# MyrtleSoftware/myrtlespeech

Measured on AMD Instinct MI355X. Metric: audio-sec/s (RTF), DS2 5xBiLSTM-1024 encoder forward + CTC greedy, 80-feature 10 s clips @ batch 32/GPU, higher is better.
Workload: dtype f16x3 (f32 split in fp16 hi+lo, 3 fp16 MFMA passes, f32 acc: LSTM, projections, conv1/2, FC1; FC2/CTC/decode f32)

## Files before the change

include/ms_hotpath.h:

```cpp
#ifndef MS_HOTPATH_H
#define MS_HOTPATH_H

#include <stddef.h>
#include <stdint.h>

#ifdef __cplusplus
extern "C" {
#endif

#define MS_ABI_VERSION 4

enum {
  MS_OK = 0,
  MS_ERR_INVALID = 1,
  MS_ERR_HIP = 2,
  MS_ERR_WORKSPACE = 3,
  MS_ERR_TIMEOUT = 4,
  MS_ERR_UNSUPPORTED = 5
};

enum { MS_CELL_LSTM = 0, MS_CELL_GRU = 1, MS_CELL_RNN_TANH = 2, MS_CELL_HARD_LSTM = 3 };

enum { MS_ACT_NONE = 0, MS_ACT_CLAMP = 1  };

int ms_abi_version(void);
const char* ms_last_error(void);


int ms_mask_time_(float* x, const int32_t* lens, int N, int inner, int T, void* stream);

size_t ms_maskconv_packed_bytes(int Cout, int Cin_g, int KF, int KT, int groups);

int ms_maskconv_pack(const float* w, void* packed, int Cout, int Cin_g, int KF, int KT, int groups, void* stream);

int ms_maskconv_forward(const float* x, const int32_t* lens, const void* packed_w, const float* bias, float* y,
                        int N, int Cin, int Fin, int Tin, int Cout, int Fout, int Tout, int KF, int KT, int SF,
                        int ST, int DF, int DT, int pad_f_l, int pad_t_l, int groups, int act, float act_lo,
                        float act_hi, void* stream);

size_t ms_maskconv_cl_packed_bytes(int Cout, int Cin, int KF, int KT);
int ms_maskconv_cl_pack(const float* w, void* packed, int Cout, int Cin, int KF, int KT, void* stream);
size_t ms_maskconv_cl_workspace_bytes(int N, int Cin, int Fin, int Tin);
int ms_maskconv_cl_forward(const float* x, const int32_t* lens, const void* packed_w, const float* bias, float* y,
                           int N, int Cin, int Fin, int Tin, int Cout, int Fout, int Tout, int KF, int KT, int SF,
                           int ST, int DF, int DT, int pad_f_l, int pad_t_l, int act, float act_lo, float act_hi,
                           void* workspace, size_t workspace_bytes, void* stream);

size_t ms_maskconv_fwin_packed_bytes(int Cout, int KF, int KT);
int ms_maskconv_fwin_pack(const float* w, void* packed, int Cout, int KF, int KT, void* stream);
size_t ms_maskconv_fwin_workspace_bytes(int N, int Tin, int KF, int SF, int Fout);
int ms_maskconv_fwin_forward(const float* x, const int32_t* lens, const void* packed_w, const float* bias, float* y, int N,
                             int Fin, int Tin, int Cout, int Fout, int Tout, int KF, int KT, int SF, int ST, int DT,
                             int pad_f_l, int pad_t_l, int act, float act_lo, float act_hi, void* workspace,
                             size_t workspace_bytes, void* stream);

int ms_maskconv_fwin_planes_supported(int N, int Tin, int Cout, int Fout, int Tout, int KF, int KT, int SF, int ST, int DT);
int ms_maskconv_cl_supported(int N, int Cin, int Fin, int Cout, int Fout, int Tout, int KT, int ST, int DT);
int ms_maskconv_fwin_planes_forward(const float* x, const int32_t* lens, const void* packed_w, const float* bias, void* planes,
                                    size_t planes_bytes, int N, int Fin, int Tin, int Cout, int Fout, int Tout, int KF, int KT,
                                    int SF, int ST, int DT, int pad_f_l, int pad_t_l, int act, float act_lo, float act_hi,
                                    void* workspace, size_t workspace_bytes, void* stream);
int ms_maskconv_cl_planes_forward(const int32_t* lens, const void* packed_w, const float* bias, float* y, int N, int Cin,
                                  int Fin, int Tin, int Cout, int Fout, int Tout, int KF, int KT, int SF, int ST, int DF,
                                  int DT, int pad_f_l, int pad_t_l, int act, float act_lo, float act_hi, void* planes,
                                  size_t planes_bytes, void* stream);

int ms_conv_set_variant(int variant);

size_t ms_maskconv1d_gemm_packed_bytes(int Cout, int Cin, int KT);
int ms_maskconv1d_gemm_pack(const float* w, void* packed, int Cout, int Cin, int KT, void* stream);
size_t ms_maskconv1d_gemm_workspace_bytes(int N, int Cin, int Tout, int Cout, int KT);
int ms_maskconv1d_gemm_forward(const float* x, const int32_t* lens, const void* packed, const float* bias, float* y, int N,
                               int Cin, int Tin, int Cout, int Tout, int KT, int ST, int DT, int pad_l, int act,
                               float act_lo, float act_hi, void* workspace, size_t workspace_bytes, void* stream);

int ms_nct_to_tnc(const float* x, float* y, int N, int CF, int T, void* stream);

int ms_clamp(const float* x, float* y, size_t n, float lo, float hi, void* stream);


int ms_linear_forward(const float* x, const float* w, const float* bias, float* y, int M, int K, int N, int act,
                      float act_lo, float act_hi, void* stream);

#define MS_LINEAR_FEW_ROWS 1
size_t ms_linear_splitk_workspace_bytes(int M, int K, int N, int flags);
int ms_linear_splitk_forward(const float* x, const float* w, const float* bias, float* y, int M, int K, int N, int act,
                             float act_lo, float act_hi, int flags, void* workspace, size_t workspace_bytes, void* stream);

size_t ms_linear_split_workspace_bytes(int M, int K, int N);
int ms_linear_split_forward(const float* x, const float* w, const float* bias, float* y, int M, int K, int N, int act,
                            float act_lo, float act_hi, void* workspace, size_t workspace_bytes, void* stream);

size_t ms_linear_split_packed_bytes(int K, int N);
int ms_linear_split_pack(const float* w, void* packed, int K, int N, void* stream);
int ms_linear_split_forward_packed(const float* x, const void* packed_w, const float* bias, float* y, int M, int K, int N, int act,
                                   float act_lo, float act_hi, void* workspace, size_t workspace_bytes, void* stream);


int ms_lookahead_forward(const float* x, const float* w, float* y, int N, int F, int T, int ctx, long xs_n,
                         long xs_f, long xs_t, long ys_n, long ys_f, long ys_t, int act, float act_lo,
                         float act_hi, void* stream);

int ms_lookahead_window_forward(const float* x, const float* w, float* y, int N, int F, int T_in, int T_out, int ctx,
                                long xs_n, long xs_f, long xs_t, long ys_n, long ys_f, long ys_t, int act, float act_lo,
                                float act_hi, void* stream);


int ms_rnn_padded_hidden(int cell, int H, int ndir);
size_t ms_rnn_packed_bytes(int cell, int In, int H, int ndir);
int ms_rnn_pack(int cell, int In, int H, int ndir, const float* const* w_ih_host, const float* const* w_hh_host,
                const float* const* b_ih_host, const float* const* b_hh_host, void* packed, void* stream);

size_t ms_rnn_workspace_bytes(int cell, int T, int N, int In, int H, int ndir);

int ms_rnn_layer_forward(int cell, const void* packed, const float* x, const int32_t* lens, int max_len,
                         const float* h0, const float* c0, float* out, float* hn, float* cn, int T, int N, int In,
                         int H, int ndir, void* workspace, size_t workspace_bytes, void* stream);

enum { MS_RNN_X_PLANES_IN_WS = 1, MS_RNN_OUT_PLANES_TO_WS = 2, MS_RNN_PACKED_ROWS = 4, MS_RNN_HX_PREINIT = 4096,
       MS_RNN_RECURRENCE_ONLY = 8192, MS_RNN_TIMING_SKIP_PROJECTION = 8192 ,
       MS_RNN_PROJECTION_ONLY = 16384 };
int ms_rnn_layer_chains_planes(int cell, int H, int ndir);
int ms_rnn_hx_preinit(int cell, int T, int N, int In, int H, int ndir, int max_len, int nregions, void* workspace,
                      size_t workspace_bytes, void* stream);
int ms_rnn_layer_packs_rows(int cell, int T, int N, int In, int H, int ndir);
int ms_rnn_layer_forward_ex(int cell, const void* packed, const float* x, const int32_t* lens, int max_len,
                            const float* h0, const float* c0, float* out, float* hn, float* cn, int T, int N, int In,
                            int H, int ndir, int flags, void* workspace, size_t workspace_bytes, void* stream);

int ms_rnn_layer_is_wide(int cell, int H, int ndir, int N);
int ms_rnn_stack_overlap_ok(int cell, int T, int N, int In, int H, int ndir, int nl);
int ms_rnn_stack_forward(int cell, const void* const* packed_host, const float* x, const int32_t* lens, int max_len,
                         const float* h0, const float* c0, float* out, float* hn, float* cn, int T, int N, int In, int H, int ndir,
                         int nl, int segments, void* workspace, size_t workspace_bytes, void* stream);

int ms_rnn_status(const void* workspace, void* stream);

size_t ms_rnn_debug_offset(int cell, int T, int N, int In, int H, int ndir);

int ms_gemm_set_variant(int variant);

enum {
  MS_PROF_PROJECTION = 0, MS_PROF_RECURRENCE = 1, MS_PROF_GEMM_K_LARGE = 2, MS_PROF_GEMM_K_SMALL = 3, MS_PROF_CONV = 4,
  MS_PROF_LAYOUT = 5, MS_PROF_LINEAR = 6, MS_PROF_GREEDY = 7, MS_PROF_OTHER = 8
};
#define MS_PROF_KINDS 9
int ms_prof_enable(int on);
int ms_prof_read(float* out_ms_host, int* out_n_host);

int ms_clock_probe(unsigned long long* out_dev, int samples, int spacing_us, void* stream);

int ms_barrier_chain_probe(unsigned long long* out_dev, int steps, int threads, void* stream);


size_t ms_ctc_loss_workspace_bytes(int T, int N, int V, int S_max);

int ms_ctc_status(const void* workspace, void* stream);

#define MS_CTC_LOG_PROBS_IN 2
int ms_ctc_loss_forward(const float* logits, const int32_t* in_lens, const int32_t* targets,
                        const int32_t* tgt_offsets, const int32_t* tgt_lens, float* nll, float* reduced, int T,
                        int N, int V, int S_max, int blank, int reduction, int zero_infinity, void* workspace,
                        size_t workspace_bytes, void* stream);

int ms_log_softmax_axis(const float* x, float* y, int outer, int axis, int inner, void* stream);
int ms_log_softmax_axis_backward(const float* y, const float* g, float* gx, int outer, int axis, int inner, void* stream);

size_t ms_ctc_loss_backward_workspace_bytes(int T, int N, int V, int S_max);
int ms_ctc_loss_backward(const float* logits, const int32_t* in_lens, const int32_t* targets, const int32_t* tgt_offsets,
                         const int32_t* tgt_lens, const float* grad_nll, float* grad_logits, int T, int N, int V,
                         int S_max, int blank, int zero_infinity, void* workspace, size_t workspace_bytes, void* stream);


int ms_ctc_greedy_decode(const float* x, const int32_t* lens, int32_t* out_idx, int32_t* out_len, int T, int N,
                         int V, int blank, void* stream);

size_t ms_ctc_greedy_stream_state_bytes(int N);
int ms_ctc_greedy_stream_begin(void* state, int N, void* stream);
int ms_ctc_greedy_stream_step(const float* x, int rows, int n, int V, int blank, const int32_t* total_lens,
                              const int32_t* chunk_lens, int32_t* labels, int32_t* label_frames, int cap, int32_t* fresh,
                              void* state, int N, void* stream);


#define MS_CTC_ALIGN_BP_LDS_BYTES 98304
size_t ms_ctc_align_workspace_bytes(int T, int N, int V, int S_max);
int ms_ctc_align(const float* x, const int32_t* in_lens, const int32_t* targets, const int32_t* tgt_offsets,
                 const int32_t* tgt_lens, float* score, int32_t* frame_state, int32_t* token_start, int32_t* token_end,
                 float* token_logp, int T, int N, int V, int L_max, int blank, int flags, void* workspace,
                 size_t workspace_bytes, void* stream);


size_t ms_ctc_beam_workspace_bytes(int T, int N, int V, int beam_width);

int ms_ctc_beam_decode(const float* probs, const int32_t* lens, int32_t* out_idx, int32_t* out_len, int T, int N,
                       int V, int blank, int beam_width, float prune_threshold, int separator, const float* word_factor,
                       int t_begin, int t_end, const float* lm_factor, int finish, int32_t* beam_len,
                       int32_t* beam_idx, int32_t* beam_plen, void* workspace, size_t workspace_bytes,
                       void* stream);

int ms_ctc_beam_decode_rows(const float* probs, const int32_t* lens, int32_t* out_idx, int32_t* out_len, int T, int N,
                            int V, int blank, int beam_width, float prune_threshold, int separator,
                            const float* word_factor, int t_begin, int t_end, int row0, int rows_held,
                            const float* lm_factor, int finish, int32_t* beam_len, int32_t* beam_idx, int32_t* beam_plen,
                            void* workspace, size_t workspace_bytes, void* stream);


#define MS_NGRAM_MAX_ORDER 5

int ms_ngram_lm_table_check(const void* blob_host, size_t bytes);

int ms_ngram_lm_score(const void* table, const void* header_host, size_t table_bytes, const int32_t* prefixes,
                      const int32_t* prefix_lens, float* out, int P, int L, int separator, void* stream);

size_t ms_ctc_beam_lm_workspace_bytes(int T, int N, int V, int beam_width, int order);
int ms_ctc_beam_decode_lm(const float* probs, const int32_t* lens, int32_t* out_idx, int32_t* out_len, int T, int N,
                          int V, int blank, int beam_width, float prune_threshold, int separator,
                          const float* word_factor, int t_begin, int t_end, int row0, int rows_held, const void* lm_table,
                          const void* lm_header_host, size_t lm_table_bytes, int finish, int32_t* beam_len,
                          int32_t* beam_idx, int32_t* beam_plen, void* workspace, size_t workspace_bytes, void* stream);

int ms_ctc_beam_decode_ex(const float* probs, const int32_t* lens, int32_t* out_idx, int32_t* out_len, int T, int N,
                          int V, int blank, int beam_width, float prune_threshold, int separator,
                          const float* word_factor, int t_begin, int t_end, int row0, int rows_held,
                          const float* lm_factor, int finish, int32_t* beam_len, int32_t* beam_idx, int32_t* beam_plen,
                          void* workspace, size_t workspace_bytes, void* stream, const void* lm_table,
                          const void* lm_header_host, size_t lm_table_bytes, int range_safe, float* beam_score,
                          int32_t* scale_log2);


size_t ms_mfcc_workspace_bytes(int N, int T, int n_fft, int n_mels, int n_mfcc);
int ms_mfcc_forward(const float* wave, const int32_t* wave_lens, const float* window, const float* dft,
                    const float* mel_fb, const float* dct, float* out, int N, int max_samples, int T, int n_fft,
                    int hop, int n_mels, int n_mfcc, float top_db, void* workspace, size_t workspace_bytes,
                    void* stream);

int ms_mfcc_legacy_forward(const float* wave, const int32_t* wave_lens, const double* twiddle, const double* fbank,
                           const double* dct, const double* lifter, float* out, int N, int max_samples, int T,
                           int frame_len, int frame_step, int nfft, int nfilt, int numcep, double preemph,
                           void* stream);

size_t ms_standardize_workspace_bytes(int N);
int ms_standardize_forward(const float* x, const int32_t* lens, float* y, int N, int inner, int T, void* workspace,
                           size_t workspace_bytes, void* stream);

int ms_context_frames_forward(const float* x, const int32_t* lens, float* y, int N, int F, int T, int n_context,
                              void* stream);

int ms_spec_augment_(float* x, const int32_t* f_bands, const int32_t* t_bands, int N, int C, int F, int T, int n_f,
                     int n_t, void* stream);


int ms_embedding_forward(const float* table, const int32_t* idx, float* out, int R, int D, int V1, void* stream);

int ms_rnnt_joint_forward(const float* enc_p, const int32_t* enc_row, const float* pred_p, const float* w_out,
                          const float* b_out, float* logp, int R, int J, int V1, void* stream);

int ms_rnnt_topk(const float* scores, int32_t* out_idx, float* out_val, int B, int C, int k, void* stream);

size_t ms_rnnt_decode_workspace_bytes(int T, int N, int V, int D, int H, int L, int J, int beam_width, int max_symbols,
                                      int greedy);
int ms_rnnt_decode(const float* enc_p, const int32_t* lens, const float* embedding, const float* const* w_ih,
                   const float* const* w_hh, const float* const* b_ih, const float* const* b_hh, const float* w_pred,
                   const float* w_out, const float* b_out, int32_t* out_idx, int32_t* out_len, float* out_score, int T,
                   int N, int V, int D, int H, int L, int J, int beam_width, int max_symbols, int greedy, void* workspace,
                   size_t workspace_bytes, void* stream);

size_t ms_rnnt_loss_lattice_bytes(int N, int T, int U1);
size_t ms_rnnt_loss_workspace_bytes(int N, int T, int U1, int V1);
int ms_rnnt_loss_forward(const float* logits, const int32_t* in_lens, const int32_t* targets, const int32_t* tgt_lens,
                         float* nll, float* lattice, int N, int T, int U1, int V1, int blank, void* workspace,
                         size_t workspace_bytes, void* stream);
int ms_rnnt_loss_backward(const float* logits, const int32_t* in_lens, const int32_t* targets, const int32_t* tgt_lens,
                          const float* nll, const float* lattice, const float* grad_nll, float* grad, int N, int T, int U1,
                          int V1, int blank, void* stream);

size_t ms_rnnt_score_lattice_bytes(int N, int T, int U1);
size_t ms_rnnt_score_workspace_bytes(int N, int T, int U1, int J, int V1);
int ms_rnnt_score(const float* enc_p, const float* pred_p, const float* w_out, const float* b_out, const int32_t* in_lens,
                  const int32_t* targets, const int32_t* tgt_lens, float* nll, float* lattice, int N, int T, int U1, int J,
                  int V1, int blank, void* workspace, size_t workspace_bytes, void* stream);

size_t ms_rnnt_joint_loss_lattice_bytes(int N, int T, int U1);
int ms_rnnt_joint_loss_forward(const float* enc_p, const float* pred_p, const float* w_out, const float* b_out,
                               const int32_t* in_lens, const int32_t* targets, const int32_t* tgt_lens, float* nll,
                               float* lattice, int N, int T, int U1, int J, int V1, int blank, void* workspace,
                               size_t workspace_bytes, void* stream);
size_t ms_rnnt_joint_loss_backward_workspace_min_bytes(int N, int T, int U1, int J, int V1);
size_t ms_rnnt_joint_loss_backward_workspace_bytes(int N, int T, int U1, int J, int V1);
int ms_rnnt_joint_loss_backward(const float* enc_p, const float* pred_p, const float* w_out, const float* b_out,
                                const int32_t* in_lens, const int32_t* targets, const int32_t* tgt_lens, const float* nll,
                                const float* lattice, const float* grad_nll, float* d_enc_p, float* d_pred_p, float* d_w_out,
                                float* d_b_out, int N, int T, int U1, int J, int V1, int blank, void* workspace,
                                size_t workspace_bytes, void* stream);
// ... 18 lines not shown
```

myrtlespeech_amd/_lib.py:

```python
import ctypes
import os
import re
from ctypes import POINTER, c_char_p, c_double, c_float, c_int, c_int32, c_long, c_size_t, c_void_p

import torch

_HERE = os.path.dirname(os.path.abspath(__file__))
LIB_PATH = os.environ.get("MS_HOTPATH_LIB") or os.path.join(_HERE, "libms_hotpath.so")
HEADER_PATH = os.path.join(os.path.dirname(_HERE), "include", "ms_hotpath.h")

MS_OK = 0
ABI_VERSION = 4
ERR_NAMES = {1: "MS_ERR_INVALID", 2: "MS_ERR_HIP", 3: "MS_ERR_WORKSPACE", 4: "MS_ERR_TIMEOUT", 5: "MS_ERR_UNSUPPORTED"}

CELL_LSTM, CELL_GRU, CELL_RNN_TANH, CELL_HARD_LSTM = 0, 1, 2, 3
ACT_NONE, ACT_CLAMP = 0, 1
LINEAR_FEW_ROWS = 1
PROF_KINDS = 9

_P = c_void_p
_PP = POINTER(c_void_p)

SIGNATURES = {
    "ms_abi_version": (c_int, []),
    "ms_last_error": (c_char_p, []),
    "ms_mask_time_": (c_int, [_P, _P, c_int, c_int, c_int, _P]),
    "ms_maskconv_packed_bytes": (c_size_t, [c_int, c_int, c_int, c_int, c_int]),
    "ms_maskconv_pack": (c_int, [_P, _P, c_int, c_int, c_int, c_int, c_int, _P]),
    "ms_maskconv_forward": (c_int, [_P, _P, _P, _P, _P] + [c_int] * 17 + [c_float, c_float, _P]),
    "ms_maskconv_cl_packed_bytes": (c_size_t, [c_int, c_int, c_int, c_int]),
    "ms_maskconv_cl_pack": (c_int, [_P, _P, c_int, c_int, c_int, c_int, _P]),
    "ms_maskconv_cl_workspace_bytes": (c_size_t, [c_int, c_int, c_int, c_int]),
    "ms_maskconv_cl_forward": (c_int, [_P, _P, _P, _P, _P] + [c_int] * 16 + [c_float, c_float, _P, c_size_t, _P]),
    "ms_maskconv_fwin_packed_bytes": (c_size_t, [c_int, c_int, c_int]),
    "ms_maskconv_fwin_pack": (c_int, [_P, _P, c_int, c_int, c_int, _P]),
    "ms_maskconv_fwin_workspace_bytes": (c_size_t, [c_int, c_int, c_int, c_int, c_int]),
    "ms_maskconv_fwin_forward": (c_int, [_P, _P, _P, _P, _P] + [c_int] * 14 + [c_float, c_float, _P, c_size_t, _P]),
    "ms_maskconv_fwin_planes_forward": (c_int, [_P, _P, _P, _P, _P, c_size_t] + [c_int] * 14 + [c_float, c_float, _P, c_size_t, _P]),
    "ms_maskconv_cl_planes_forward": (c_int, [_P, _P, _P, _P] + [c_int] * 16 + [c_float, c_float, _P, c_size_t, _P]),
    "ms_maskconv_fwin_planes_supported": (c_int, [c_int] * 10),
    "ms_maskconv_cl_supported": (c_int, [c_int] * 9),
    "ms_conv_set_variant": (c_int, [c_int]),
    "ms_maskconv1d_gemm_packed_bytes": (c_size_t, [c_int, c_int, c_int]),
    "ms_maskconv1d_gemm_pack": (c_int, [_P, _P, c_int, c_int, c_int, _P]),
    "ms_maskconv1d_gemm_workspace_bytes": (c_size_t, [c_int] * 5),
    "ms_maskconv1d_gemm_forward": (c_int, [_P, _P, _P, _P, _P] + [c_int] * 10 + [c_float, c_float, _P, c_size_t, _P]),
    "ms_nct_to_tnc": (c_int, [_P, _P, c_int, c_int, c_int, _P]),
    "ms_clamp": (c_int, [_P, _P, c_size_t, c_float, c_float, _P]),
    "ms_linear_forward": (c_int, [_P, _P, _P, _P, c_int, c_int, c_int, c_int, c_float, c_float, _P]),
    "ms_linear_splitk_workspace_bytes": (c_size_t, [c_int, c_int, c_int, c_int]),
    "ms_linear_splitk_forward": (c_int, [_P, _P, _P, _P, c_int, c_int, c_int, c_int, c_float, c_float, c_int, _P, c_size_t, _P]),
    "ms_linear_split_workspace_bytes": (c_size_t, [c_int, c_int, c_int]),
    "ms_linear_split_forward": (c_int, [_P, _P, _P, _P, c_int, c_int, c_int, c_int, c_float, c_float, _P, c_size_t, _P]),
    "ms_linear_split_packed_bytes": (c_size_t, [c_int, c_int]),
    "ms_linear_split_pack": (c_int, [_P, _P, c_int, c_int, _P]),
    "ms_linear_split_forward_packed": (c_int, [_P, _P, _P, _P, c_int, c_int, c_int, c_int, c_float, c_float, _P, c_size_t, _P]),
    "ms_lookahead_forward": (c_int, [_P, _P, _P, c_int, c_int, c_int, c_int] + [c_long] * 6 + [c_int, c_float, c_float, _P]),
    "ms_lookahead_window_forward": (c_int, [_P, _P, _P, c_int, c_int, c_int, c_int, c_int] + [c_long] * 6 + [c_int, c_float, c_float, _P]),
    "ms_rnn_packed_bytes": (c_size_t, [c_int, c_int, c_int, c_int]),
    "ms_ctc_status": (c_int, [_P, _P]),
    "ms_rnn_padded_hidden": (c_int, [c_int, c_int, c_int]),
    "ms_rnn_hx_preinit": (c_int, [c_int] * 8 + [_P, c_size_t, _P]),
    "ms_rnn_pack": (c_int, [c_int, c_int, c_int, c_int, _PP, _PP, _PP, _PP, _P, _P]),
    "ms_rnn_workspace_bytes": (c_size_t, [c_int] * 6),
    "ms_rnn_layer_forward": (c_int, [c_int, _P, _P, _P, c_int, _P, _P, _P, _P, _P] + [c_int] * 5 + [_P, c_size_t, _P]),
    "ms_rnn_layer_forward_ex": (c_int, [c_int, _P, _P, _P, c_int, _P, _P, _P, _P, _P] + [c_int] * 6 + [_P, c_size_t, _P]),
    "ms_rnn_layer_chains_planes": (c_int, [c_int, c_int, c_int]),
    "ms_rnn_layer_is_wide": (c_int, [c_int] * 4),
    "ms_rnn_stack_overlap_ok": (c_int, [c_int] * 7),
    "ms_rnn_stack_forward": (c_int, [c_int, _P, _P, _P, c_int, _P, _P, _P, _P, _P] + [c_int] * 7 + [_P, c_size_t, _P]),
    "ms_rnn_status": (c_int, [_P, _P]),
    "ms_rnn_debug_offset": (c_size_t, [c_int] * 6),
    "ms_rnn_layer_packs_rows": (c_int, [c_int] * 6),
    "ms_gemm_set_variant": (c_int, [c_int]),
    "ms_prof_enable": (c_int, [c_int]),
    "ms_prof_read": (c_int, [POINTER(c_float), POINTER(c_int)]),
    "ms_clock_probe": (c_int, [_P, c_int, c_int, _P]),
    "ms_barrier_chain_probe": (c_int, [_P, c_int, c_int, _P]),
    "ms_ctc_loss_workspace_bytes": (c_size_t, [c_int] * 4),
    "ms_ctc_loss_forward": (c_int, [_P] * 7 + [c_int] * 7 + [_P, c_size_t, _P]),
    "ms_log_softmax_axis": (c_int, [_P, _P, c_int, c_int, c_int, _P]),
    "ms_log_softmax_axis_backward": (c_int, [_P, _P, _P, c_int, c_int, c_int, _P]),
    "ms_ctc_loss_backward_workspace_bytes": (c_size_t, [c_int] * 4),
    "ms_ctc_loss_backward": (c_int, [_P] * 7 + [c_int] * 6 + [_P, c_size_t, _P]),
    "ms_ctc_greedy_decode": (c_int, [_P, _P, _P, _P, c_int, c_int, c_int, c_int, _P]),
    "ms_ctc_align_workspace_bytes": (c_size_t, [c_int] * 4),
    "ms_ctc_align": (c_int, [_P] * 10 + [c_int] * 6 + [_P, c_size_t, _P]),
    "ms_ctc_greedy_stream_state_bytes": (c_size_t, [c_int]),
    "ms_ctc_greedy_stream_begin": (c_int, [_P, c_int, _P]),
    "ms_ctc_greedy_stream_step": (c_int, [_P, c_int, c_int, c_int, c_int, _P, _P, _P, _P, c_int, _P, _P, c_int, _P]),
    "ms_embedding_forward": (c_int, [_P, _P, _P, c_int, c_int, c_int, _P]),
    "ms_rnnt_joint_forward": (c_int, [_P, _P, _P, _P, _P, _P, c_int, c_int, c_int, _P]),
    "ms_rnnt_topk": (c_int, [_P, _P, _P, c_int, c_int, c_int, _P]),
    "ms_ctc_beam_workspace_bytes": (c_size_t, [c_int] * 4),
    "ms_ctc_beam_decode": (c_int, [_P, _P, _P, _P, c_int, c_int, c_int, c_int, c_int, c_float, c_int, _P, c_int, c_int,
                                   _P, c_int, _P, _P, _P, _P, c_size_t, _P]),
    "ms_ctc_beam_decode_rows": (c_int, [_P, _P, _P, _P, c_int, c_int, c_int, c_int, c_int, c_float, c_int, _P, c_int, c_int,
                                        c_int, c_int, _P, c_int, _P, _P, _P, _P, c_size_t, _P]),
    "ms_ngram_lm_table_check": (c_int, [_P, c_size_t]),
    "ms_ngram_lm_score": (c_int, [_P, _P, c_size_t, _P, _P, _P, c_int, c_int, c_int, _P]),
    "ms_ctc_beam_lm_workspace_bytes": (c_size_t, [c_int] * 5),
    "ms_ctc_beam_decode_lm": (c_int, [_P, _P, _P, _P, c_int, c_int, c_int, c_int, c_int, c_float, c_int, _P, c_int, c_int,
                                      c_int, c_int, _P, _P, c_size_t, c_int, _P, _P, _P, _P, c_size_t, _P]),
    "ms_ctc_beam_decode_ex": (c_int, [_P, _P, _P, _P, c_int, c_int, c_int, c_int, c_int, c_float, c_int, _P, c_int, c_int,
                                      c_int, c_int, _P, c_int, _P, _P, _P, _P, c_size_t, _P, _P, _P, c_size_t, c_int, _P, _P]),
    "ms_rnnt_decode_workspace_bytes": (c_size_t, [c_int] * 10),
    "ms_rnnt_decode": (c_int, [_P, _P, _P, _PP, _PP, _PP, _PP, _P, _P, _P, _P, _P, _P] + [c_int] * 10 + [_P, c_size_t, _P]),
    "ms_rnnt_loss_lattice_bytes": (c_size_t, [c_int] * 3),
    "ms_rnnt_loss_workspace_bytes": (c_size_t, [c_int] * 4),
    "ms_rnnt_loss_forward": (c_int, [_P] * 6 + [c_int] * 5 + [_P, c_size_t, _P]),
    "ms_rnnt_loss_backward": (c_int, [_P] * 8 + [c_int] * 5 + [_P]),
    "ms_rnnt_score_lattice_bytes": (c_size_t, [c_int] * 3),
    "ms_rnnt_score_workspace_bytes": (c_size_t, [c_int] * 5),
    "ms_rnnt_score": (c_int, [_P] * 9 + [c_int] * 6 + [_P, c_size_t, _P]),
    "ms_rnnt_joint_loss_lattice_bytes": (c_size_t, [c_int] * 3),
    "ms_rnnt_joint_loss_forward": (c_int, [_P] * 9 + [c_int] * 6 + [_P, c_size_t, _P]),
    "ms_rnnt_joint_loss_backward_workspace_min_bytes": (c_size_t, [c_int] * 5),
    "ms_rnnt_joint_loss_backward_workspace_bytes": (c_size_t, [c_int] * 5),
    "ms_rnnt_joint_loss_backward": (c_int, [_P] * 14 + [c_int] * 6 + [_P, c_size_t, _P]),
    "ms_rnnt_align_workspace_bytes": (c_size_t, [c_int] * 4),
    "ms_rnnt_align": (c_int, [_P] * 9 + [c_int] * 6 + [_P, c_size_t, _P]),
    "ms_rnnt_align_joint_workspace_bytes": (c_size_t, [c_int] * 5),
    "ms_rnnt_align_joint": (c_int, [_P] * 12 + [c_int] * 6 + [_P, c_size_t, _P]),
    "ms_mfcc_workspace_bytes": (c_size_t, [c_int] * 5),
    "ms_mfcc_forward": (c_int, [_P] * 7 + [c_int] * 7 + [c_float, _P, c_size_t, _P]),
    "ms_mfcc_legacy_forward": (c_int, [_P] * 7 + [c_int] * 8 + [c_double, _P]),
    "ms_standardize_workspace_bytes": (c_size_t, [c_int]),
    "ms_standardize_forward": (c_int, [_P, _P, _P, c_int, c_int, c_int, _P, c_size_t, _P]),
    "ms_context_frames_forward": (c_int, [_P, _P, _P, c_int, c_int, c_int, c_int, _P]),
    "ms_spec_augment_": (c_int, [_P, _P, _P] + [c_int] * 6 + [_P]),
}

_lib = None


def header_symbols():
    with open(HEADER_PATH) as f:
        text = re.sub(r"/\*.*?\*/", "", f.read(), flags=re.S)
    return sorted(set(re.findall(r"\b(ms_[a-z0-9_]+)\s*\(", text)))


def load():
    global _lib
    if _lib is None:
        if not os.path.exists(LIB_PATH):
            raise RuntimeError(
                f"{LIB_PATH} not found: build it with `python -c 'import __graft_entry__ as g; g.build()'` "
                "(or `make -C myrtlespeech_amd/csrc`). There is no CPU fallback."
            )
        lib = ctypes.CDLL(LIB_PATH)
        for name, (res, args) in SIGNATURES.items():
            fn = getattr(lib, name)
            fn.restype = res
            fn.argtypes = args
        got = lib.ms_abi_version()
        if got != ABI_VERSION:
            raise RuntimeError(f"{LIB_PATH} reports MS_ABI_VERSION {got}, this binding needs {ABI_VERSION}: rebuild the "
                               "library (`make -C myrtlespeech_amd/csrc`)")
        _lib = lib
    return _lib


def require_gpu():
    if not torch.cuda.is_available():
        raise RuntimeError("myrtlespeech_amd: a HIP device (MI355X) is required; there is no CPU fallback")


def stream_ptr():
    return c_void_p(torch.cuda.current_stream().cuda_stream)


def ptr(t, strided=False):
    if t is None:
        return c_void_p(0)
    if not isinstance(t, torch.Tensor):
        raise TypeError(f"_lib.ptr: expected a torch.Tensor or None, got {type(t).__name__}")
    if not t.is_cuda:
        raise ValueError(f"_lib.ptr: a {t.device.type} tensor (shape {tuple(t.shape)}) cannot be a device-pointer argument; "
                         "move it to the GPU first (host buffers go through _lib.host_ptr)")
    if not strided and not t.is_contiguous():
        raise ValueError(f"_lib.ptr: tensor of shape {tuple(t.shape)} and strides {tuple(t.stride())} is not contiguous; the "
                         "kernels read dense storage (call .contiguous())")
    return c_void_p(t.data_ptr())


def host_ptr(t):
    if t is None:
        return c_void_p(0)
    if not isinstance(t, torch.Tensor) or t.is_cuda or not t.is_contiguous():
        raise ValueError("_lib.host_ptr: expected a contiguous CPU tensor")
    return c_void_p(t.data_ptr())


def check(rc, what):
    if rc != MS_OK:
        msg = load().ms_last_error().decode()
        raise RuntimeError(f"{what} failed with {ERR_NAMES.get(rc, rc)}: {msg}")


def f32c(t):
    if t.dtype != torch.float32:
        t = t.float()
    if not t.is_cuda:
        t = t.cuda()
    return t.contiguous()


_ASYNC_LENS = os.environ.get("MS_ASYNC_LENS") != "0"


_const_lens = {}


def _const_tensor(shape, dtype, value, make: bool):
    key = (tuple(shape), dtype, int(value))
    rec = _const_lens.get(key)
    if rec is not None:
        t, version = rec
        if version_of(t) == version:
            return t
        _const_lens[("stale", len(_const_lens)) + key] = rec
        del _const_lens[key]
    if not make or len(_const_lens) >= 4096:
        return None
    t = torch.full(tuple(shape), int(value), dtype=dtype, device="cuda")
    _const_lens[key] = (t, version_of(t))
    return t
# ... 108 lines not shown
```

myrtlespeech_amd/csrc/common.h:

```cpp
#pragma once
#include <hip/hip_runtime.h>
#include <stdint.h>
#include <stdio.h>
#include <atomic>
#include <string>

#include "../../include/ms_hotpath.h"

namespace ms {

void set_error(const std::string& s);

#define MS_REQUIRE(cond, msg)                                              \
  do {                                                                     \
    if (!(cond)) {                                                         \
      ms::set_error(std::string(__func__) + ": " + (msg));                 \
      return MS_ERR_INVALID;                                               \
    }                                                                      \
  } while (0)

#define MS_HIP(call)                                                                        \
  do {                                                                                      \
    hipError_t e_ = (call);                                                                 \
    if (e_ != hipSuccess) {                                                                 \
      ms::set_error(std::string(__func__) + ": " #call " -> " + hipGetErrorString(e_));     \
      return MS_ERR_HIP;                                                                    \
    }                                                                                       \
  } while (0)

#define MS_LAUNCH_CHECK() MS_HIP(hipGetLastError())

static inline size_t align_up(size_t v, size_t a) { return (v + a - 1) / a * a; }
static inline int cdiv(int a, int b) { return (a + b - 1) / b; }

typedef float f32x4 __attribute__((ext_vector_type(4)));
typedef float f32x16 __attribute__((ext_vector_type(16)));

__device__ __forceinline__ int mfma32_row(int reg, int lane) { return (reg & 3) + 8 * (reg >> 2) + 4 * (lane >> 5); }

int num_cus();

struct DeviceOnce {
  std::atomic<unsigned long long> done_mask{0};
  static unsigned long long bit() {
    int d = 0;
    if (hipGetDevice(&d) != hipSuccess) d = 0;
    return 1ull << (d & 63);
  }
  bool need() const { return !(done_mask.load(std::memory_order_acquire) & bit()); }
  void done() { done_mask.fetch_or(bit(), std::memory_order_release); }
};

struct ProfScope {
  hipEvent_t a = nullptr, b = nullptr;
  int kind;
  hipStream_t stream;
  bool on;
  ProfScope(int kind, hipStream_t st);
  ~ProfScope();
  ProfScope(const ProfScope&) = delete;
  ProfScope& operator=(const ProfScope&) = delete;
};

enum { PREC_F32 = 0, PREC_BF16X3 = 1, PREC_F16 = 2, PREC_F16X3 = 3 };
int precision_mode();
int split_mode();
enum { GEMM_K_WHOLE = 0, GEMM_K_FIRST = 1, GEMM_K_SECOND = 2 };
int weight_scale_launch(const float* w, size_t n, float* scale_word, int prec, hipStream_t stream);

constexpr bool prec_one_plane(int P) { return P == PREC_F16; }
constexpr bool prec_half_planes(int P) { return P == PREC_F16X3 || P == PREC_F16; }

typedef unsigned u32x4_ __attribute__((ext_vector_type(4)));
typedef __bf16 bf16x8_ __attribute__((ext_vector_type(8)));
typedef _Float16 f16x8_ __attribute__((ext_vector_type(8)));
template <bool HM>
__device__ __forceinline__ unsigned plane_bits(float x) {
  if constexpr (HM) return (unsigned)__builtin_bit_cast(unsigned short, (_Float16)__builtin_amdgcn_fmed3f(x, -65504.f, 65504.f));
  else return (unsigned)__builtin_bit_cast(unsigned short, (__bf16)x);
}
template <bool HM>
__device__ __forceinline__ unsigned plane_bits_bounded(float x) {
  if constexpr (HM) return (unsigned)__builtin_bit_cast(unsigned short, (_Float16)x);
  else return (unsigned)__builtin_bit_cast(unsigned short, (__bf16)x);
}
template <bool HM>
__device__ __forceinline__ float plane_val(unsigned bits) {
  if constexpr (HM) return (float)__builtin_bit_cast(_Float16, (unsigned short)bits);
  else return __uint_as_float(bits << 16);
}
template <bool HM>
__device__ __forceinline__ void plane_split(float x, unsigned& hi, unsigned& lo) {
  hi = plane_bits<HM>(x);
  lo = plane_bits<HM>(x - plane_val<HM>(hi));
}
template <bool HM>
__device__ __forceinline__ void plane_split_bounded(float x, unsigned& hi, unsigned& lo) {
  hi = plane_bits_bounded<HM>(x);
  lo = plane_bits_bounded<HM>(x - plane_val<HM>(hi));
}
template <bool HM>
__device__ __forceinline__ f32x16 mfma_32x32x16(u32x4_ a, u32x4_ b, f32x16 c) {
  if constexpr (HM) return __builtin_amdgcn_mfma_f32_32x32x16_f16(__builtin_bit_cast(f16x8_, a), __builtin_bit_cast(f16x8_, b), c, 0, 0, 0);
  else return __builtin_amdgcn_mfma_f32_32x32x16_bf16(__builtin_bit_cast(bf16x8_, a), __builtin_bit_cast(bf16x8_, b), c, 0, 0, 0);
}
template <bool HM>
__device__ __forceinline__ f32x4 mfma_16x16x32(u32x4_ a, u32x4_ b, f32x4 c) {
  if constexpr (HM) return __builtin_amdgcn_mfma_f32_16x16x32_f16(__builtin_bit_cast(f16x8_, a), __builtin_bit_cast(f16x8_, b), c, 0, 0, 0);
  else return __builtin_amdgcn_mfma_f32_16x16x32_bf16(__builtin_bit_cast(bf16x8_, a), __builtin_bit_cast(bf16x8_, b), c, 0, 0, 0);
}

}
```

myrtlespeech_amd/csrc/gemm_split.hip:

```cpp
#include <algorithm>
#include <cstdlib>

#include "common.h"

namespace ms {

typedef unsigned u32x4 __attribute__((ext_vector_type(4)));
typedef unsigned u32x2 __attribute__((ext_vector_type(2)));
typedef __bf16 bf16x8 __attribute__((ext_vector_type(8)));
typedef _Float16 f16x8 __attribute__((ext_vector_type(8)));

__device__ __forceinline__ unsigned bf16_hi_bits(float x) { return (unsigned)__builtin_bit_cast(unsigned short, (__bf16)x); }

__device__ __forceinline__ unsigned f16_bits(float x) { return (unsigned)__builtin_bit_cast(unsigned short, (_Float16)x); }

__global__ void to_f16_plane_kernel(const float* __restrict__ x, unsigned short* __restrict__ hi, size_t n4) {
  for (size_t i = (size_t)blockIdx.x * blockDim.x + threadIdx.x; i < n4; i += (size_t)gridDim.x * blockDim.x) {
    const f32x4 v = reinterpret_cast<const f32x4*>(x)[i];
    u32x2 ho = {f16_bits(v[0]) | (f16_bits(v[1]) << 16), f16_bits(v[2]) | (f16_bits(v[3]) << 16)};
    reinterpret_cast<u32x2*>(hi)[i] = ho;
  }
}

template <bool HM>
// ... 267 lines not shown
  }
  constexpr int GM = 4;
  const int per_group = GM * nbn;
  const int first_m = (bid / per_group) * GM;
  const int gm = min(GM, nbm - first_m);
  const int bm = first_m + (bid % per_group) % gm;
  const int bn = (bid % per_group) / gm;
  const int m0 = bm * S2_M, n0 = bn * S2_N;

  const int tid = threadIdx.x, lane = tid & 63, wave = tid >> 6;
  const int wm = wave >> 1, wn = wave & 1;
  const int l31 = lane & 31, half = lane >> 5;
  const int kg = tid & 3, r_in = tid >> 2;

  f32x16 acc[2][4];
#pragma unroll
  for (int i = 0; i < 2; ++i)
#pragma unroll
    for (int j = 0; j < 4; ++j)
#pragma unroll
      for (int r = 0; r < 16; ++r) acc[i][j][r] = 0.f;

  u32x4 rah[2], ral[2], rbh[2], rbl[2];
  auto load_regs = [&](int k0) {
#pragma unroll
    for (int i = 0; i < 2; ++i) {
      rah[i] = ld_granule(Ah, M, lda, m0 + r_in + 128 * i, k0 + kg * 8);
      rbh[i] = ld_granule(Wh, N, ldw, n0 + r_in + 128 * i, k0 + kg * 8);
      if (!F16) {
        ral[i] = ld_granule(Al, M, lda, m0 + r_in + 128 * i, k0 + kg * 8);
        rbl[i] = ld_granule(Wl, N, ldw, n0 + r_in + 128 * i, k0 + kg * 8);
      }
    }
  };
  auto store_regs = [&](char* buf) {
#pragma unroll
    for (int i = 0; i < 2; ++i) {
      const int off = kg * S2_PLANE + (r_in + 128 * i) * 16;
      *reinterpret_cast<u32x4*>(buf + off) = rah[i];
      *reinterpret_cast<u32x4*>(buf + 2 * S2_TILE + off) = rbh[i];
      if (!F16) {
        *reinterpret_cast<u32x4*>(buf + S2_TILE + off) = ral[i];
        *reinterpret_cast<u32x4*>(buf + 3 * S2_TILE + off) = rbl[i];
      }
    }
  };

  const int nk = K / SB_K;
  load_regs(0);
  store_regs(lds);
  if (nk > 1) load_regs(SB_K);
  __syncthreads();

  u32x4 ah[2], al[2], bh[4], bl[4];
  auto read_ops = [&](const char* cur, int s) {
    const int g = 2 * s + half;
#pragma unroll
    for (int i = 0; i < 2; ++i) {
      const int off = g * S2_PLANE + (wm * 64 + i * 32 + l31) * 16;
      ah[i] = *reinterpret_cast<const u32x4*>(cur + off);
      if (!F16) al[i] = *reinterpret_cast<const u32x4*>(cur + S2_TILE + off);
    }
#pragma unroll
    for (int j = 0; j < 4; ++j) {
      const int off = g * S2_PLANE + (wn * 128 + j * 32 + l31) * 16;
      bh[j] = *reinterpret_cast<const u32x4*>(cur + 2 * S2_TILE + off);
      if (!F16) bl[j] = *reinterpret_cast<const u32x4*>(cur + 3 * S2_TILE + off);
    }
  };
  auto mfma_ops = [&]() {
    if (F16) {
#pragma unroll
      for (int i = 0; i < 2; ++i)
#pragma unroll
        for (int j = 0; j < 4; ++j)
          acc[i][j] = __builtin_amdgcn_mfma_f32_32x32x16_f16(__builtin_bit_cast(f16x8, ah[i]), __builtin_bit_cast(f16x8, bh[j]),
                                                             acc[i][j], 0, 0, 0);
    } else {
#pragma unroll
      for (int i = 0; i < 2; ++i)
#pragma unroll
        for (int j = 0; j < 4; ++j)
          acc[i][j] = mfma_32x32x16<HM>(ah[i], bh[j], acc[i][j]);
#pragma unroll
      for (int i = 0; i < 2; ++i)
#pragma unroll
        for (int j = 0; j < 4; ++j)
          acc[i][j] = mfma_32x32x16<HM>(al[i], bh[j], acc[i][j]);
#pragma unroll
      for (int i = 0; i < 2; ++i)
#pragma unroll
        for (int j = 0; j < 4; ++j)
          acc[i][j] = mfma_32x32x16<HM>(ah[i], bl[j], acc[i][j]);
    }
  };
  {
    for (int kt = 0; kt < nk; ++kt) {
      const char* cur = lds + (kt & 1) * S2_BUF;
      read_ops(cur, 0);
      store_regs(lds + ((kt + 1) & 1) * S2_BUF);
      mfma_ops();
      __builtin_amdgcn_sched_group_barrier(0x100, F16 ? 6 : 12, 0);
#pragma unroll
      for (int i = 0; i < (F16 ? 4 : 8); ++i) {
        __builtin_amdgcn_sched_group_barrier(0x008, F16 ? 2 : 3, 0);
        __builtin_amdgcn_sched_group_barrier(0x200, 1, 0);
      }
      __builtin_amdgcn_sched_barrier(0);
      read_ops(cur, 1);
      load_regs(min(kt + 2, nk - 1) * SB_K);
      mfma_ops();
      __builtin_amdgcn_sched_group_barrier(0x100, F16 ? 6 : 12, 0);
#pragma unroll
      for (int i = 0; i < (F16 ? 4 : 8); ++i) {
        __builtin_amdgcn_sched_group_barrier(0x008, F16 ? 2 : 3, 0);
        __builtin_amdgcn_sched_group_barrier(0x020, 1, 0);
      }
      __builtin_amdgcn_sched_barrier(0);
      __syncthreads();
    }
  }

#pragma unroll
  for (int j = 0; j < 4; ++j) {
    const int n = n0 + wn * 128 + j * 32 + l31;
    const float bv = (bias != nullptr && n < N) ? bias[n] : 0.f;
#pragma unroll
    for (int i = 0; i < 2; ++i)
#pragma unroll
      for (int r = 0; r < 16; ++r) {
        const int m = m0 + wm * 64 + i * 32 + mfma32_row(r, lane);
        if (m < M && n < N) {
          float v = acc[i][j][r] + bv;
          if (act == MS_ACT_CLAMP) v = fminf(fmaxf(v, lo), hi);
          Y[(size_t)m * N + n] = v;
        }
      }
  }
}

constexpr int G4_PLANE = 256 * 64;
constexpr int G4_STAGE = 4 * G4_PLANE;
constexpr int G4_LDS = 2 * G4_STAGE;
typedef __attribute__((address_space(3))) void* lds_ptr_t;

__device__ __forceinline__ void lds_dma_16(__amdgpu_buffer_rsrc_t rsrc, char* dst, int voff, int soff) {
  __builtin_amdgcn_raw_ptr_buffer_load_lds(rsrc, (lds_ptr_t)dst, 16, voff, soff, 0, 0);
}

template <int P, int WN, int PER_STEP_ = 3, bool SPACED = false, int NJ = 4, int TM = 256>
__device__ __forceinline__ void gemm4_body(const unsigned short* __restrict__ Ah, const unsigned short* __restrict__ Al,
                                           const unsigned short* __restrict__ Wh, const unsigned short* __restrict__ Wl,
                                           const float* __restrict__ bias, float* __restrict__ Y, int M, int K, int N, int act,
                                           float lo, float hi, const int* __restrict__ m_eff, int lda, int ldw, int kmode) {
  constexpr bool F16 = prec_one_plane(P), HM = P == PREC_F16X3;
  extern __shared__ __attribute__((aligned(16))) char lds[];
  constexpr int TN = 32 * NJ * WN;
  static_assert(NJ == 4 || (NJ == 2 && WN == 2), "the narrow form is the 8-wave kernel");
  static_assert(TM == 256 || (TM == 128 && NJ == 2 && WN == 2), "128-row tiles: the four-wave 128 x 128 form");
  if (m_eff != nullptr) {
    M = __builtin_amdgcn_readfirstlane(*m_eff);
    if ((int)blockIdx.x >= ((N + TN - 1) / TN) * ((M + TM - 1) / TM)) return;
  }
  const int nbn = (N + TN - 1) / TN, nbm = (M + TM - 1) / TM;
  const int nwg = nbn * nbm;
  int bid = blockIdx.x;
  {
    const int q = nwg / 8, r = nwg % 8, xcd = bid % 8;
    bid = (xcd < r ? xcd * (q + 1) : r * (q + 1) + (xcd - r) * q) + bid / 8;
  }
  constexpr int GM = 4;
  const int per_group = GM * nbn;
  const int first_m = (bid / per_group) * GM;
  const int gm = min(GM, nbm - first_m);
  const int bm = first_m + (bid % per_group) % gm;
  const int bn = (bid % per_group) / gm;
  const int m0 = bm * TM, n0 = bn * TN;

  const int tid = threadIdx.x, lane = tid & 63;
  const int wave = __builtin_amdgcn_readfirstlane(tid >> 6);
  const int wm = WN == 2 ? wave >> 1 : wave, wn = WN == 2 ? wave & 1 : 0;
  const int l31 = lane & 31, half = lane >> 5;

  constexpr int NPA = NJ == 2 ? (F16 ? 2 : 4) : WN == 2 ? (F16 ? 4 : 8) : (F16 ? 4 : 8);
  constexpr int NPB = TM == 128 ? NPA : NJ == 2 ? (F16 ? 1 : 2) : WN == 2 ? 0 : (F16 ? 2 : 4);
  constexpr int NP = NPA + NPB;
  int PA, RA, PB = 2, RB = 0;
  if (TM == 128) {
    if (F16) { PA = 0; RA = wave * 32; PB = 2; RB = wave * 32; }
    else { PA = wave >> 1; RA = (wave & 1) * 64; PB = 2 + (wave >> 1); RB = (wave & 1) * 64; }
  } else if (NJ == 2) {
    if (F16) { PA = 0; RA = wave * 32; PB = 2; RB = wave * 16; }
    else { PA = wave >> 2; RA = (wave & 3) * 64; PB = 2 + (wave >> 2); RB = (wave & 3) * 32; }
  } else if (WN == 2) {
    const int g0 = wave * NPA;
    PA = F16 ? (g0 >> 4) * 2 : (g0 >> 4);
    RA = (g0 & 15) * 16;
  } else if (F16) {
    PA = 0; RA = wave * 64; PB = 2; RB = wave * 32;
  } else {
    PA = wave >> 1; RA = (wave & 1) * 128; PB = 2 + (wave >> 1); RB = (wave & 1) * 64;
  }
  auto plane_rsrc = [&](int pl) {
    const unsigned short* src = pl == 0 ? Ah : pl == 1 ? Al : pl == 2 ? Wh : Wl;
    return __builtin_amdgcn_make_buffer_rsrc(const_cast<unsigned short*>(src), 0, (unsigned)((size_t)(pl < 2 ? M : N) * (pl < 2 ? lda : ldw) * 2), 0x00020000);
  };
  const __amdgpu_buffer_rsrc_t rsrc_a = plane_rsrc(PA), rsrc_b = plane_rsrc(PB);
  int voff[NP];
  {
    const int kgs = (lane & 3) ^ ((lane >> 4) & 3);
#pragma unroll
    for (int p = 0; p < NP; ++p) {
      const int pl = p < NPA ? PA : PB;
      const int rows = pl < 2 ? M : N, row = (pl < 2 ? m0 : n0) + (p < NPA ? RA + p * 16 : RB + (p - NPA) * 16) + (lane >> 2);
      voff[p] = min(row, rows - 1) * ((pl < 2 ? lda : ldw) * 2) + kgs * 16;
    }
  }
  constexpr int RING = (F16 && WN == 2) ? 4 : 2;
  auto stage_off = [&](int stage) { return RING == 4 ? (stage & 1) * G4_STAGE + (stage >> 1) * G4_PLANE : stage * G4_STAGE; };
  auto dma_block = [&](int kb, int stage) {
    const int soff = __builtin_amdgcn_readfirstlane(kb * (SB_K * 2));
    char* dst_a = lds + stage_off(stage) + PA * G4_PLANE + RA * 64;
    char* dst_b = lds + stage_off(stage) + PB * G4_PLANE + RB * 64;
#pragma unroll
    for (int p = 0; p < NP; ++p) {
      if (p < NPA) lds_dma_16(rsrc_a, dst_a + p * 1024, voff[p], soff);
      else lds_dma_16(rsrc_b, dst_b + (p - NPA) * 1024, voff[p], soff);
    }
  };

  f32x16 acc[2][NJ];
#pragma unroll
  for (int i = 0; i < 2; ++i)
#pragma unroll
    for (int j = 0; j < NJ; ++j)
#pragma unroll
      for (int r = 0; r < 16; ++r) acc[i][j][r] = 0.f;
  if (kmode == GEMM_K_SECOND) {
#pragma unroll
    for (int i = 0; i < 2; ++i) {
      const int m = m0 + wm * 64 + i * 32 + l31;
      if (m >= M) continue;
#pragma unroll
      for (int j = 0; j < NJ; ++j)
#pragma unroll
        for (int g = 0; g < 4; ++g) {
          const int n = n0 + wn * (32 * NJ) + j * 32 + 8 * g + 4 * half;
          if (n + 3 < N) {
            const f32x4 v = *reinterpret_cast<const f32x4*>(Y + (size_t)m * N + n);
            acc[i][j][4 * g] = v[0]; acc[i][j][4 * g + 1] = v[1]; acc[i][j][4 * g + 2] = v[2]; acc[i][j][4 * g + 3] = v[3];
          }
        }
    }
  }

  const int sw = (l31 >> 2) & 3;
  const int foff0 = l31 * 64 + ((half ^ sw) * 16);
  const int foff1 = l31 * 64 + (((2 + half) ^ sw) * 16);
  const int a_base = wm * 64 * 64, b_base = 2 * G4_PLANE + wn * (32 * NJ) * 64;

  u32x4 fa[WN == 1 ? 1 : 2][6 + 6];
  auto read_frags = [&](int set, int stage, int h) {
    const char* st = lds + stage_off(stage) + (h ? foff1 : foff0);
#pragma unroll
    for (int i = 0; i < 2; ++i) {
      fa[set][i] = *reinterpret_cast<const u32x4*>(st + a_base + i * 32 * 64);
      if (!F16) fa[set][2 + i] = *reinterpret_cast<const u32x4*>(st + G4_PLANE + a_base + i * 32 * 64);
    }
#pragma unroll
    for (int j = 0; j < NJ; ++j) {
      fa[set][4 + j] = *reinterpret_cast<const u32x4*>(st + b_base + j * 32 * 64);
      if (!F16) fa[set][8 + j] = *reinterpret_cast<const u32x4*>(st + G4_PLANE + b_base + j * 32 * 64);
    }
  };
  auto mfma_set = [&](int set) {
    if (F16) {
#pragma unroll
      for (int i = 0; i < 2; ++i)
#pragma unroll
        for (int j = 0; j < NJ; ++j)
          acc[i][j] = __builtin_amdgcn_mfma_f32_32x32x16_f16(__builtin_bit_cast(f16x8, fa[set][4 + j]),
                                                             __builtin_bit_cast(f16x8, fa[set][i]), acc[i][j], 0, 0, 0);
    } else {
#pragma unroll
      for (int i = 0; i < 2; ++i)
#pragma unroll
        for (int j = 0; j < NJ; ++j)
          acc[i][j] = mfma_32x32x16<HM>(fa[set][4 + j], fa[set][i], acc[i][j]);
#pragma unroll
      for (int i = 0; i < 2; ++i)
#pragma unroll
        for (int j = 0; j < NJ; ++j)
          acc[i][j] = mfma_32x32x16<HM>(fa[set][4 + j], fa[set][2 + i], acc[i][j]);
#pragma unroll
      for (int i = 0; i < 2; ++i)
#pragma unroll
        for (int j = 0; j < NJ; ++j)
          acc[i][j] = mfma_32x32x16<HM>(fa[set][8 + j], fa[set][i], acc[i][j]);
    }
  };

  const int nk = K / SB_K;
  dma_block(0, 0);
  dma_block(min(1, nk - 1), 1);
  if (RING == 4) {
    dma_block(min(2, nk - 1), 2);
    dma_block(min(3, nk - 1), 3);
  }
  __builtin_amdgcn_s_waitcnt(0x0070);
  __builtin_amdgcn_s_barrier();
  if (WN == 1) {
    u32x4 xa[2][4], wb[2][2];
    auto rd_x = [&](int ring, int stage, int h) {
      const char* st = lds + stage * G4_STAGE + (h ? foff1 : foff0) + a_base;
#pragma unroll
      for (int i = 0; i < 2; ++i) {
        xa[ring][i] = *reinterpret_cast<const u32x4*>(st + i * 32 * 64);
        if (!F16) xa[ring][2 + i] = *reinterpret_cast<const u32x4*>(st + G4_PLANE + i * 32 * 64);
      }
    };
    auto rd_w = [&](int ring, int stage, int h, int j) {
      const char* st = lds + stage * G4_STAGE + (h ? foff1 : foff0) + b_base + j * 32 * 64;
      wb[ring][0] = *reinterpret_cast<const u32x4*>(st);
      if (!F16) wb[ring][1] = *reinterpret_cast<const u32x4*>(st + G4_PLANE);
    };
    auto mm = [&](int xr, int wr, int j, auto&& issue) {
      issue(0);
#pragma unroll
      for (int i = 0; i < 2; ++i) {
        if (F16) {
          acc[i][j] = __builtin_amdgcn_mfma_f32_32x32x16_f16(__builtin_bit_cast(f16x8, wb[wr][0]), __builtin_bit_cast(f16x8, xa[xr][i]), acc[i][j], 0, 0, 0);
        } else {
          acc[i][j] = mfma_32x32x16<HM>(wb[wr][0], xa[xr][i], acc[i][j]);
        }
      }
      if (!F16) {
        issue(1);
#pragma unroll
        for (int i = 0; i < 2; ++i)
          acc[i][j] = mfma_32x32x16<HM>(wb[wr][0], xa[xr][2 + i], acc[i][j]);
        issue(2);
#pragma unroll
        for (int i = 0; i < 2; ++i)
          acc[i][j] = mfma_32x32x16<HM>(wb[wr][1], xa[xr][i], acc[i][j]);
      }
    };
    rd_x(0, 0, 0);
    rd_w(0, 0, 0, 0);
    constexpr int PER_STEP = PER_STEP_, DMA_STEPS = (NP + PER_STEP - 1) / PER_STEP;
    for (int b = 0; b < nk; ++b) {
      const int cur = b & 1;
      const int soff_next = __builtin_amdgcn_readfirstlane(min(b + 1, nk - 1) * (SB_K * 2));
      char* dst_a = lds + (cur ^ 1) * G4_STAGE + PA * G4_PLANE + RA * 64;
      char* dst_b = lds + (cur ^ 1) * G4_STAGE + PB * G4_PLANE + RB * 64;
#pragma unroll
      for (int h = 0; h < 2; ++h)
#pragma unroll
        for (int j = 0; j < 4; ++j) {
          const int step = h * 4 + j;
          auto piece = [&](int p) {
            if (p < NPA) lds_dma_16(rsrc_a, dst_a + p * 1024, voff[p], soff_next);
            else lds_dma_16(rsrc_b, dst_b + (p - NPA) * 1024, voff[p], soff_next);
          };
          if (!SPACED && b > 0 && step < DMA_STEPS) {
#pragma unroll
            for (int p = step * PER_STEP; p < (step + 1) * PER_STEP && p < NP; ++p) piece(p);
          }
          auto issue = [&](int k) {
            if (SPACED && b > 0 && step < DMA_STEPS && k < PER_STEP && step * PER_STEP + k < NP) piece(step * PER_STEP + k);
          };
          if (step == 7) {
            __builtin_amdgcn_s_waitcnt(0x0070);
            __builtin_amdgcn_s_barrier();
            rd_x(0, cur ^ 1, 0);
            rd_w(0, cur ^ 1, 0, 0);
          } else {
            if (j == 3) rd_x(1, cur, 1);
            rd_w((step + 1) & 1, cur, (step + 1) >> 2, (step + 1) & 3);
          }
          mm(h, step & 1, j, issue);
        }
    }
  } else {
  read_frags(0, 0, 0);
  __builtin_amdgcn_s_waitcnt(0xc07f);
  __builtin_amdgcn_sched_barrier(0);

  constexpr int NR = NJ == 2 ? (F16 ? 4 : 8) : (F16 ? 6 : 12);
  constexpr int MPR = F16 ? 8 / 6 + 1 : 2;
  for (int b = 0; b < nk; ++b) {
    const int cur = b & (RING - 1), nxt = (b + 1) & (RING - 1);
    read_frags(1, cur, 1);
    mfma_set(0);
#pragma unroll
    for (int i = 0; i < NR; ++i) {
      __builtin_amdgcn_sched_group_barrier(0x100, 1, 0);
      __builtin_amdgcn_sched_group_barrier(0x008, MPR, 0);
    }
    __builtin_amdgcn_sched_barrier(0);
    if (RING == 4) __builtin_amdgcn_s_waitcnt(0x0070 | (2 * NP));
    else __builtin_amdgcn_s_waitcnt(0x0070);
    __builtin_amdgcn_s_barrier();
    __builtin_amdgcn_sched_barrier(0);
    dma_block(min(b + RING, nk - 1), cur);
    read_frags(0, nxt, 0);
    mfma_set(1);
#pragma unroll
    for (int i = 0; i < NR; ++i) {
      if (i < NP) __builtin_amdgcn_sched_group_barrier(0x020, 1, 0);
      __builtin_amdgcn_sched_group_barrier(0x100, 1, 0);
      __builtin_amdgcn_sched_group_barrier(0x008, MPR, 0);
    }
    __builtin_amdgcn_sched_barrier(0);
    __builtin_amdgcn_s_waitcnt(0xc07f);
    __builtin_amdgcn_sched_barrier(0);
  }
  }
  __builtin_amdgcn_s_waitcnt(0x0070);

  const bool n_vec = (N % 4) == 0;
#pragma unroll
  for (int i = 0; i < 2; ++i) {
    const int m = m0 + wm * 64 + i * 32 + l31;
    if (m >= M) continue;
#pragma unroll
    for (int j = 0; j < NJ; ++j)
#pragma unroll
      for (int g = 0; g < 4; ++g) {
        const int n = n0 + wn * (32 * NJ) + j * 32 + 8 * g + 4 * half;
        f32x4 v = {acc[i][j][4 * g], acc[i][j][4 * g + 1], acc[i][j][4 * g + 2], acc[i][j][4 * g + 3]};
        if (n_vec && n + 3 < N) {
          if (bias != nullptr && kmode != GEMM_K_FIRST) {
            const f32x4 bv = *reinterpret_cast<const f32x4*>(bias + n);
            v += bv;
          }
          if (act == MS_ACT_CLAMP && kmode != GEMM_K_FIRST) {
#pragma unroll
            for (int e = 0; e < 4; ++e) v[e] = fminf(fmaxf(v[e], lo), hi);
          }
          *reinterpret_cast<f32x4*>(Y + (size_t)m * N + n) = v;
        } else {
#pragma unroll
          for (int e = 0; e < 4; ++e)
            if (n + e < N) {
              float x = v[e] + (bias != nullptr ? bias[n + e] : 0.f);
              if (act == MS_ACT_CLAMP) x = fminf(fmaxf(x, lo), hi);
              Y[(size_t)m * N + n + e] = x;
            }
        }
      }
  }
}

template <int P>
__global__ __launch_bounds__(512, 2) void gemm_nt_bf16x3_kernel4(const unsigned short* __restrict__ Ah,
                                                                 const unsigned short* __restrict__ Al,
                                                                 const unsigned short* __restrict__ Wh,
                                                                 const unsigned short* __restrict__ Wl,
                                                                 const float* __restrict__ bias, float* __restrict__ Y,
                                                                 int M, int K, int N, int act, float lo, float hi,
                                                                 const int* __restrict__ m_eff, int lda, int ldw, int kmode) {
  gemm4_body<P, 2>(Ah, Al, Wh, Wl, bias, Y, M, K, N, act, lo, hi, m_eff, lda, ldw, kmode);
}

template <int P>
__global__ __launch_bounds__(512, 2) void gemm_nt_bf16x3_kernel4h(const unsigned short* __restrict__ Ah,
                                                                  const unsigned short* __restrict__ Al,
                                                                  const unsigned short* __restrict__ Wh,
                                                                  const unsigned short* __restrict__ Wl,
                                                                  const float* __restrict__ bias, float* __restrict__ Y,
                                                                  int M, int K, int N, int act, float lo, float hi,
                                                                  const int* __restrict__ m_eff, int lda, int ldw, int kmode) {
  gemm4_body<P, 2, 3, false, 2>(Ah, Al, Wh, Wl, bias, Y, M, K, N, act, lo, hi, m_eff, lda, ldw, kmode);
}

template <int P>
__global__ __launch_bounds__(256, 1) void gemm_nt_bf16x3_kernel4q(const unsigned short* __restrict__ Ah,
                                                                  const unsigned short* __restrict__ Al,
                                                                  const unsigned short* __restrict__ Wh,
                                                                  const unsigned short* __restrict__ Wl,
                                                                  const float* __restrict__ bias, float* __restrict__ Y,
                                                                  int M, int K, int N, int act, float lo, float hi,
                                                                  const int* __restrict__ m_eff, int lda, int ldw, int kmode) {
  gemm4_body<P, 2, 3, false, 2, 128>(Ah, Al, Wh, Wl, bias, Y, M, K, N, act, lo, hi, m_eff, lda, ldw, kmode);
}

template <int P, int PER_STEP = 3, bool SPACED = false>
__global__ __launch_bounds__(256, 2) void gemm_nt_bf16x3_kernel4n(
    const unsigned short* __restrict__ Ah, const unsigned short* __restrict__ Al, const unsigned short* __restrict__ Wh,
    const unsigned short* __restrict__ Wl, const float* __restrict__ bias, float* __restrict__ Y, int M, int K, int N, int act,
    float lo, float hi, const int* __restrict__ m_eff, int lda, int ldw, int kmode) {
  gemm4_body<P, 1, PER_STEP, SPACED>(Ah, Al, Wh, Wl, bias, Y, M, K, N, act, lo, hi, m_eff, lda, ldw, kmode);
}

static std::atomic<int> g_gemm_variant{0};

int split_planes_launch(const float* x, unsigned short* hi, unsigned short* lo, size_t elems, int prec, hipStream_t stream) {
  const size_t n4 = elems / 4;
  const int blocks = (int)std::min<size_t>((n4 + 255) / 256, 4096);
  if (prec == PREC_F16)
    hipLaunchKernelGGL(to_f16_plane_kernel, dim3(blocks), dim3(256), 0, stream, x, hi, n4);
  else if (prec == PREC_F16X3)
    hipLaunchKernelGGL(split_planes_kernel<true>, dim3(blocks), dim3(256), 0, stream, x, hi, lo, n4);
  else
    hipLaunchKernelGGL(split_planes_kernel<false>, dim3(blocks), dim3(256), 0, stream, x, hi, lo, n4);
  MS_LAUNCH_CHECK();
  return MS_OK;
}

int split_mode() {
  const int m = precision_mode();
  return m == PREC_F32 ? PREC_F16X3 : m;
}

bool gemm_rows_from_device_ok(int M, int K, int N) {
  static const bool small_tile = getenv("MS_GEMM_TILE128") && getenv("MS_GEMM_TILE128")[0] == '1';
  static const bool regstage = getenv("MS_GEMM_REGSTAGE") && getenv("MS_GEMM_REGSTAGE")[0] == '1';
  const long tiles256 = (long)cdiv(M, S2_M) * cdiv(N, S2_N);
  const bool starved = tiles256 * 4 < (long)num_cus() * 3 && (long)cdiv(M, SB_M) * cdiv(N, SB_N) > tiles256;
  return !small_tile && !regstage && !starved && (long)M * N >= 4L * 1024 * 1024 && K % 32 == 0 &&
         (size_t)std::max(M, N) * K * 2 < ((size_t)1 << 31) && g_gemm_variant.load(std::memory_order_relaxed) != 2;
}

int gemm_bf16x3_launch_rows(const unsigned short* ah, const unsigned short* al, const unsigned short* wh,
                            const unsigned short* wl, const float* bias, float* y, int M, int K, int N, int act, float lo,
                            float hi, int prec, hipStream_t stream, const int* m_eff);
int gemm_bf16x3_launch_ld(const unsigned short* ah, const unsigned short* al, const unsigned short* wh,
                          const unsigned short* wl, const float* bias, float* y, int M, int K, int N, int act, float lo,
                          float hi, int prec, hipStream_t stream, const int* m_eff, int lda, int ldw, int kmode);

int gemm_bf16x3_launch(const unsigned short* ah, const unsigned short* al, const unsigned short* wh,
                       const unsigned short* wl, const float* bias, float* y, int M, int K, int N, int act, float lo,
                       float hi, int prec, hipStream_t stream) {
  return gemm_bf16x3_launch_rows(ah, al, wh, wl, bias, y, M, K, N, act, lo, hi, prec, stream, nullptr);
}

#define MS_BY_PREC(K) (prec == PREC_F16 ? K<PREC_F16> : prec == PREC_F16X3 ? K<PREC_F16X3> : K<PREC_BF16X3>)

int gemm_bf16x3_launch_rows(const unsigned short* ah, const unsigned short* al, const unsigned short* wh,
                            const unsigned short* wl, const float* bias, float* y, int M, int K, int N, int act, float lo,
                            float hi, int prec, hipStream_t stream, const int* m_eff) {
  return gemm_bf16x3_launch_ld(ah, al, wh, wl, bias, y, M, K, N, act, lo, hi, prec, stream, m_eff, K, K, GEMM_K_WHOLE);
}

bool gemm_k_halves_ok(int M, int N) {
  static const bool small_tile = getenv("MS_GEMM_TILE128") && getenv("MS_GEMM_TILE128")[0] == '1';
  static const bool regstage = getenv("MS_GEMM_REGSTAGE") && getenv("MS_GEMM_REGSTAGE")[0] == '1';
  static const bool half_off = getenv("MS_GEMM_HALF_TILE") && getenv("MS_GEMM_HALF_TILE")[0] == '0';
  if (small_tile || regstage || half_off || N % 4 != 0 || g_gemm_variant.load(std::memory_order_relaxed) != 0) return false;
  const long tiles256 = (long)cdiv(M, S2_M) * cdiv(N, S2_N);
  const bool starved = tiles256 * 4 < (long)num_cus() * 3 && (long)cdiv(M, SB_M) * cdiv(N, SB_N) > tiles256;
  const bool t64 = (long)cdiv(M, T6) * cdiv(N, T6) <= 2L * num_cus() && (long)cdiv(M, S2_M) * cdiv(N, 128) * 4 <= (long)num_cus();
  if (t64) return false;
  return starved ? (long)M * N >= 1024L * 1024 : (long)M * N >= 4L * 1024 * 1024;
}

int gemm_bf16x3_launch_ld(const unsigned short* ah, const unsigned short* al, const unsigned short* wh,
                          const unsigned short* wl, const float* bias, float* y, int M, int K, int N, int act, float lo,
                          float hi, int prec, hipStream_t stream, const int* m_eff, int lda, int ldw, int kmode) {
  if (kmode != GEMM_K_WHOLE && !gemm_k_halves_ok(M, N)) {
    set_error("gemm_bf16x3_launch_ld: a contraction cut along K needs an output that runs on the LDS-DMA kernels");
    return MS_ERR_UNSUPPORTED;
  }
  static ms::DeviceOnce attr_once;
  if (attr_once.need()) {
    MS_HIP(hipFuncSetAttribute((const void*)gemm_nt_bf16x3_kernel<false>, hipFuncAttributeMaxDynamicSharedMemorySize, SPLIT_LDS));
    MS_HIP(hipFuncSetAttribute((const void*)gemm_nt_bf16x3_kernel<true>, hipFuncAttributeMaxDynamicSharedMemorySize, SPLIT_LDS));
#define MS_ATTR3(K, bytes)                                                                                         \
    MS_HIP(hipFuncSetAttribute((const void*)K<PREC_BF16X3>, hipFuncAttributeMaxDynamicSharedMemorySize, bytes));   \
    MS_HIP(hipFuncSetAttribute((const void*)K<PREC_F16>, hipFuncAttributeMaxDynamicSharedMemorySize, bytes));      \
    MS_HIP(hipFuncSetAttribute((const void*)K<PREC_F16X3>, hipFuncAttributeMaxDynamicSharedMemorySize, bytes));
    MS_ATTR3(gemm_nt_bf16x3_kernel2, SPLIT2_LDS)
    MS_ATTR3(gemm_nt_bf16x3_kernel4, G4_LDS)
    MS_ATTR3(gemm_nt_bf16x3_kernel4n, G4_LDS)
    MS_ATTR3(gemm_nt_bf16x3_kernel4h, G4_LDS)
    MS_ATTR3(gemm_nt_bf16x3_kernel4q, G4_LDS)
#undef MS_ATTR3
    MS_HIP(hipFuncSetAttribute((const void*)gemm_nt_bf16x3_kernel4n<PREC_BF16X3, 2>, hipFuncAttributeMaxDynamicSharedMemorySize, G4_LDS));
    MS_HIP(hipFuncSetAttribute((const void*)gemm_nt_bf16x3_kernel4n<PREC_BF16X3, 6>, hipFuncAttributeMaxDynamicSharedMemorySize, G4_LDS));
    MS_HIP(hipFuncSetAttribute((const void*)gemm_nt_bf16x3_kernel4n<PREC_BF16X3, 3, true>, hipFuncAttributeMaxDynamicSharedMemorySize, G4_LDS));
    MS_HIP(hipFuncSetAttribute((const void*)gemm_nt_bf16x3_kernel4n<PREC_BF16X3, 2, true>, hipFuncAttributeMaxDynamicSharedMemorySize, G4_LDS));
    attr_once.done();
  }
  static const bool small_tile = getenv("MS_GEMM_TILE128") && getenv("MS_GEMM_TILE128")[0] == '1';
  const bool f16 = prec == PREC_F16;
  const long tiles256 = (long)cdiv(M, S2_M) * cdiv(N, S2_N);
  const bool starved = tiles256 * 4 < (long)num_cus() * 3 && (long)cdiv(M, SB_M) * cdiv(N, SB_N) > tiles256;
  static const bool half_off = getenv("MS_GEMM_HALF_TILE") && getenv("MS_GEMM_HALF_TILE")[0] == '0';
  auto tile64 = [&]() {
    const char* e = getenv("MS_GEMM_TILE64");
    return !(e && e[0] == '0') && !small_tile && m_eff == nullptr && g_gemm_variant.load(std::memory_order_relaxed) == 0 &&
           (long)cdiv(M, T6) * cdiv(N, T6) <= 2L * num_cus();
  };
  auto launch_tile64 = [&]() {
    hipLaunchKernelGGL(MS_BY_PREC(gemm_nt_bf16x3_tile64_kernel), dim3(cdiv(M, T6) * cdiv(N, T6)), dim3(256), 0, stream, ah, al, wh, wl,
                       bias, y, M, K, N, act, lo, hi, lda, ldw);
  };
  if (tile64() && (long)cdiv(M, S2_M) * cdiv(N, 128) * 4 <= (long)num_cus()) {
    launch_tile64();
    MS_LAUNCH_CHECK();
    return MS_OK;
  }
  if (!half_off && !small_tile && starved && m_eff == nullptr && (long)M * N >= 1024L * 1024 &&
      g_gemm_variant.load(std::memory_order_relaxed) == 0 && std::max((size_t)M * lda, (size_t)N * ldw) * 2 < ((size_t)1 << 31)) {
    const char* qe = getenv("MS_GEMM_QUARTER_TILE");
    if (!(qe && qe[0] == '0') && (long)cdiv(M, S2_M) * cdiv(N, 128) * 2 <= (long)num_cus() && cdiv(M, 128) > cdiv(M, S2_M)) {
      hipLaunchKernelGGL(MS_BY_PREC(gemm_nt_bf16x3_kernel4q), dim3(cdiv(M, 128) * cdiv(N, 128)), dim3(256), G4_LDS, stream, ah, al, wh, wl,
                         bias, y, M, K, N, act, lo, hi, m_eff, lda, ldw, kmode);
      MS_LAUNCH_CHECK();
      return MS_OK;
    }
    hipLaunchKernelGGL(MS_BY_PREC(gemm_nt_bf16x3_kernel4h), dim3(cdiv(M, S2_M) * cdiv(N, 128)), dim3(512), G4_LDS, stream, ah, al, wh, wl,
                       bias, y, M, K, N, act, lo, hi, m_eff, lda, ldw, kmode);
    MS_LAUNCH_CHECK();
    return MS_OK;
  }
  if (f16 || (!small_tile && !starved && (long)M * N >= 4L * 1024 * 1024)) {
    const int nwg2 = cdiv(M, S2_M) * cdiv(N, S2_N);
    const int variant = g_gemm_variant.load(std::memory_order_relaxed);
    static const bool regstage = getenv("MS_GEMM_REGSTAGE") && getenv("MS_GEMM_REGSTAGE")[0] == '1';
    if (variant != 2 && !regstage && std::max((size_t)M * lda, (size_t)N * ldw) * 2 < ((size_t)1 << 31)) {
      if (variant >= 7 && variant <= 11) {
        auto k41 = MS_BY_PREC(gemm_nt_bf16x3_kernel4n);
        if (prec == PREC_BF16X3) {
          if (variant == 8) k41 = gemm_nt_bf16x3_kernel4n<PREC_BF16X3, 2>;
          if (variant == 9) k41 = gemm_nt_bf16x3_kernel4n<PREC_BF16X3, 6>;
          if (variant == 10) k41 = gemm_nt_bf16x3_kernel4n<PREC_BF16X3, 3, true>;
          if (variant == 11) k41 = gemm_nt_bf16x3_kernel4n<PREC_BF16X3, 2, true>;
        }
        hipLaunchKernelGGL(k41, dim3(cdiv(M, S2_M) * cdiv(N, 128)), dim3(256), G4_LDS, stream, ah, al, wh, wl, bias, y, M, K, N,
                           act, lo, hi, m_eff, lda, ldw, kmode);
        MS_LAUNCH_CHECK();
        return MS_OK;
      }
      hipLaunchKernelGGL(MS_BY_PREC(gemm_nt_bf16x3_kernel4), dim3(nwg2), dim3(512), G4_LDS, stream, ah, al, wh, wl, bias, y, M, K, N, act,
                         lo, hi, m_eff, lda, ldw, kmode);
      MS_LAUNCH_CHECK();
      return MS_OK;
    }
    if (m_eff != nullptr) {
      set_error("gemm_bf16x3_launch_rows: this shape does not run on the kernels that take the row count from the device");
      return MS_ERR_UNSUPPORTED;
    }
    hipLaunchKernelGGL(MS_BY_PREC(gemm_nt_bf16x3_kernel2), dim3(nwg2), dim3(512), SPLIT2_LDS, stream, ah, al, wh, wl, bias, y, M, K, N,
                       act, lo, hi, lda, ldw);
    MS_LAUNCH_CHECK();
    return MS_OK;
  }
  if (m_eff != nullptr) {
    set_error("gemm_bf16x3_launch_rows: this shape does not run on the kernels that take the row count from the device");
    return MS_ERR_UNSUPPORTED;
  }
  if (tile64()) {
    launch_tile64();
    MS_LAUNCH_CHECK();
    return MS_OK;
  }
  const int nwg = cdiv(M, SB_M) * cdiv(N, SB_N);
  if (prec == PREC_F16X3)
    hipLaunchKernelGGL(gemm_nt_bf16x3_kernel<true>, dim3(nwg), dim3(256), SPLIT_LDS, stream, ah, al, wh, wl, bias, y, M, K, N, act, lo, hi, lda, ldw);
  else
    hipLaunchKernelGGL(gemm_nt_bf16x3_kernel<false>, dim3(nwg), dim3(256), SPLIT_LDS, stream, ah, al, wh, wl, bias, y, M, K, N, act, lo, hi, lda, ldw);
  MS_LAUNCH_CHECK();
  return MS_OK;
}
#undef MS_BY_PREC

}

extern "C" int ms_gemm_set_variant(int v) {
  ms::g_gemm_variant.store(v, std::memory_order_relaxed);
  return MS_OK;
}

extern "C" size_t ms_linear_split_workspace_bytes(int M, int K, int N) {
  if (M <= 0 || K <= 0 || N <= 0) return 0;
  return ms::align_up((size_t)M * K * 4, 256) + ms::align_up((size_t)N * K * 4, 256);
}

extern "C" size_t ms_linear_split_packed_bytes(int K, int N) {
  if (K <= 0 || N <= 0) return 0;
  return ms::align_up((size_t)N * K * 4, 256);
}

extern "C" int ms_linear_split_pack(const float* w, void* packed, int K, int N, void* stream_) {
  MS_REQUIRE(w && packed, "null pointer");
  MS_REQUIRE(K > 0 && N > 0 && K % 32 == 0, "bad shape (K must be a multiple of 32)");
  MS_REQUIRE(((uintptr_t)w & 15) == 0, "w must be 16-byte aligned");
  unsigned short* wh = (unsigned short*)packed;
  const int prec = ms::split_mode();
  return ms::split_planes_launch(w, wh, wh + (size_t)N * K, (size_t)N * K, prec, (hipStream_t)stream_);
}

extern "C" int ms_linear_split_forward_packed(const float* x, const void* packed_w, const float* bias, float* y, int M, int K, int N,
                                              int act, float act_lo, float act_hi, void* workspace, size_t workspace_bytes,
                                              void* stream_) {
  ms::ProfScope prof_span(MS_PROF_LINEAR, (hipStream_t)stream_);
  MS_REQUIRE(x && packed_w && y && workspace, "null pointer");
  MS_REQUIRE(M > 0 && K > 0 && N > 0, "bad shape");
  MS_REQUIRE(K % 32 == 0, "K must be a multiple of 32 (use ms_linear_forward otherwise)");
  MS_REQUIRE(act == MS_ACT_NONE || act == MS_ACT_CLAMP, "bad act");
  MS_REQUIRE(((uintptr_t)x & 15) == 0, "x must be 16-byte aligned");
  if (workspace_bytes < ms::align_up((size_t)M * K * 4, 256)) {
    ms::set_error("ms_linear_split_forward_packed: workspace too small");
    return MS_ERR_WORKSPACE;
  }
  hipStream_t stream = (hipStream_t)stream_;
  unsigned short* xh = (unsigned short*)workspace;
  unsigned short* xl = xh + (size_t)M * K;
  const unsigned short* wh = (const unsigned short*)packed_w;
  const unsigned short* wl = wh + (size_t)N * K;
  const int prec = ms::split_mode();
  const char* skip = getenv("MS_TIMING_SKIP_SPLIT");
  int rc = (skip && skip[0] == '1') ? MS_OK : ms::split_planes_launch(x, xh, xl, (size_t)M * K, prec, stream);
  if (rc == MS_OK) rc = ms::gemm_bf16x3_launch(xh, xl, wh, wl, bias, y, M, K, N, act, act_lo, act_hi, prec, stream);
  return rc;
}

extern "C" int ms_linear_split_forward(const float* x, const float* w, const float* bias, float* y, int M, int K, int N,
                                       int act, float act_lo, float act_hi, void* workspace, size_t workspace_bytes,
                                       void* stream_) {
  ms::ProfScope prof_span(MS_PROF_LINEAR, (hipStream_t)stream_);
  MS_REQUIRE(x && w && y && workspace, "null pointer");
  MS_REQUIRE(M > 0 && K > 0 && N > 0, "bad shape");
  MS_REQUIRE(K % 32 == 0, "K must be a multiple of 32 (use ms_linear_forward otherwise)");
  MS_REQUIRE(act == MS_ACT_NONE || act == MS_ACT_CLAMP, "bad act");
  MS_REQUIRE((((uintptr_t)x | (uintptr_t)w) & 15) == 0, "x and w must be 16-byte aligned");
  if (workspace_bytes < ms_linear_split_workspace_bytes(M, K, N)) {
    ms::set_error("ms_linear_split_forward: workspace too small");
    return MS_ERR_WORKSPACE;
  }
  hipStream_t stream = (hipStream_t)stream_;
  unsigned short* xh = (unsigned short*)workspace;
  unsigned short* xl = xh + (size_t)M * K;
  unsigned short* wh = (unsigned short*)((char*)workspace + ms::align_up((size_t)M * K * 4, 256));
  unsigned short* wl = wh + (size_t)N * K;
  const int prec = ms::split_mode();
  int rc = ms::split_planes_launch(x, xh, xl, (size_t)M * K, prec, stream);
  if (rc == MS_OK) rc = ms::split_planes_launch(w, wh, wl, (size_t)N * K, prec, stream);
  if (rc == MS_OK) rc = ms::gemm_bf16x3_launch(xh, xl, wh, wl, bias, y, M, K, N, act, act_lo, act_hi, prec, stream);
  return rc;
}
```

myrtlespeech_amd/csrc/rnn.hip:

```cpp
#include <algorithm>
#include <cstring>
#include <mutex>
#include <vector>

#include "common.h"

namespace ms {
int split_planes_launch(const float* x, unsigned short* hi, unsigned short* lo, size_t elems, int prec, hipStream_t stream);
bool gemm_rows_from_device_ok(int M, int K, int N);
int gemm_bf16x3_launch_rows(const unsigned short* ah, const unsigned short* al, const unsigned short* wh,
                            const unsigned short* wl, const float* bias, float* y, int M, int K, int N, int act, float lo,
                            float hi, int prec, hipStream_t stream, const int* m_eff);
int gemm_bf16x3_launch(const unsigned short* ah, const unsigned short* al, const unsigned short* wh,
                       const unsigned short* wl, const float* bias, float* y, int M, int K, int N, int act, float lo,
                       float hi, int prec, hipStream_t stream);
int gemm_bf16x3_launch_ld(const unsigned short* ah, const unsigned short* al, const unsigned short* wh,
                          const unsigned short* wl, const float* bias, float* y, int M, int K, int N, int act, float lo,
                          float hi, int prec, hipStream_t stream, const int* m_eff, int lda, int ldw, int kmode);
bool gemm_k_halves_ok(int M, int N);
int linear_launch(const float* x, const float* w, const float* bias, float* y, int M, int K, int N, int act, float lo,
                  float hi, hipStream_t stream);
}

namespace {

using ms::f32x16;
using ms::f32x4;

constexpr int RED_STRIDE = 40;
constexpr int RED_FLOATS = 4 * 32 * RED_STRIDE;
constexpr size_t STATUS_BYTES = 256;
constexpr int HX_REGIONS = 8;
constexpr unsigned long long SPIN_LIMIT_TICKS = 200000000ull;

inline int gates_of(int cell) { return (cell == MS_CELL_LSTM || cell == MS_CELL_HARD_LSTM) ? 4 : (cell == MS_CELL_GRU ? 3 : 1); }

bool force_generic() {
  static int v = -1;
  if (v < 0) {
    const char* e = getenv("MS_RNN_FORCE_GENERIC");
    v = (e && e[0] == '1') ? 1 : 0;
  }
  return v == 1;
}

int persistent_blocks_per_cu(bool gru);

bool wide_lstm_h(int H) { return H == 1280 || H == 1536 || H == 2048; }
bool use_fast(int cell, int H, int ndir) {
  if (force_generic()) return false;
  if (!(cell == MS_CELL_LSTM || cell == MS_CELL_HARD_LSTM)) return false;
  const int cus = ms::num_cus();
  if (H > 1024) {
    if (!wide_lstm_h(H) || !(ms::precision_mode() == ms::PREC_BF16X3 || ms::precision_mode() == ms::PREC_F16X3)) return false;
    return cus > 0 && (H / 8) <= cus * std::min(1, persistent_blocks_per_cu(false));
  }
  if (H % 32 != 0) return false;
  return cus > 0 && ndir * (H / 8) <= cus * std::min(1, persistent_blocks_per_cu(false));
}

bool want_split() { return ms::precision_mode() != ms::PREC_F32; }
bool use_split(int cell, int H, int ndir) { return use_fast(cell, H, ndir) && want_split() && H % 64 == 0; }
bool two_stream_shape(int H) { return H == 256 || H == 512 || H == 768 || H == 1024 || wide_lstm_h(H); }
bool use_f32x2(int cell, int H, int ndir) {
  static const bool off = getenv("MS_LSTM_F32_ONE_STREAM") && getenv("MS_LSTM_F32_ONE_STREAM")[0] == '1';
  return !off && use_fast(cell, H, ndir) && !want_split() && two_stream_shape(H);
}
bool use_f16(int cell, int H, int ndir) {
  return ms::precision_mode() == ms::PREC_F16 && use_split(cell, H, ndir) && two_stream_shape(H);
}
int two_plane_mode() { return ms::precision_mode() == ms::PREC_F16X3 ? ms::PREC_F16X3 : ms::PREC_BF16X3; }
int layer_prec(int cell, int H, int ndir) { return use_f16(cell, H, ndir) ? ms::PREC_F16 : two_plane_mode(); }
bool use_split_gemm(int cell, int H, int ndir, int In) {
  if (In % 32 != 0 || !want_split() || force_generic()) return false;
  return use_split(cell, H, ndir) || !use_fast(cell, H, ndir);
}

constexpr int gru_units(int H) {
  return (H == 2560 || H == 1280) ? 10 : (H == 2048 || H == 1536 || H == 1024 || H == 768 || H == 512) ? 8 : 0;
}
bool use_gru_persistent(int cell, int H, int ndir) {
  static const bool off = getenv("MS_GRU_PERSISTENT") && getenv("MS_GRU_PERSISTENT")[0] == '0';
  if (off || force_generic() || !want_split() || cell != MS_CELL_GRU) return false;
  const int U = gru_units(H);
  if (U == 0) return false;
  const int cus = ms::num_cus();
  (void)ndir;
  return cus > 0 && (H / U) <= cus * std::min(1, persistent_blocks_per_cu(true));
}

int lstm_ring_shift() {
  static int v = -1;
  if (v < 0) {
    const char* e = getenv("MS_LSTM_RING");
    int slots = e ? atoi(e) : 2;
    v = 1;
    while ((1 << v) < slots && v < 7) ++v;
  }
  return v;
}
struct PackLayout {
  size_t wih, bias_x, whh, bhh, total;
};
PackLayout pack_layout(int cell, int In, int H, int ndir) {
  const size_t GH = (size_t)gates_of(cell) * H;
  PackLayout L;
  size_t o = 0;
  L.wih = o; o += ms::align_up(ndir * GH * In * sizeof(float), 256);
  L.bias_x = o; o += ms::align_up(ndir * GH * sizeof(float), 256);
  size_t whh_bytes = ndir * GH * H * sizeof(float);
  if (use_gru_persistent(cell, H, ndir)) whh_bytes = (size_t)ndir * (H / gru_units(H)) * 128 * H;
  L.whh = o; o += ms::align_up(whh_bytes, 256);
  L.bhh = o; o += ms::align_up(ndir * GH * sizeof(float), 256);
  L.total = o;
  return L;
}

struct WsLayout {
  size_t status, flags, xproj, xproj_bytes, hx, hx_bytes, state_h, state_c, dbg, row_off, xsplit, total;
  int xproj_slots;
  size_t xslot(int parity) const { return xproj + (size_t)(parity % xproj_slots) * xproj_bytes; }
};
bool overlap_shape(int cell, int H, int ndir) {
  return (cell == MS_CELL_LSTM || cell == MS_CELL_HARD_LSTM) && H == 1024 && ndir == 2 && ms::precision_mode() != ms::PREC_F32;
}
WsLayout ws_layout(int cell, int T, int N, int H, int ndir, int In) {
  const size_t GH = (size_t)gates_of(cell) * H;
  const int npad = ms::cdiv(N, 32) * 32;
  WsLayout L;
  size_t o = 0;
  o += STATUS_BYTES;
  L.status = o; o += STATUS_BYTES;
  L.flags = o; o += ms::align_up((size_t)ndir * std::max(H / 8, 1) * sizeof(unsigned), 256);
  L.xproj_slots = overlap_shape(cell, H, ndir) ? 2 : 1;
  L.xproj_bytes = ms::align_up((size_t)T * N * ndir * GH * sizeof(float), 256);
  L.xproj = o; o += L.xproj_bytes * L.xproj_slots;
  L.hx = o;
  L.hx_bytes = ms::align_up(((size_t)ndir * 2 * H * std::min(npad, 64) * sizeof(float)) << (lstm_ring_shift() - 1), 256);
  o += L.hx_bytes * HX_REGIONS;
  L.state_h = o; o += ms::align_up((size_t)2 * ndir * N * H * sizeof(float), 256);
  L.state_c = o; o += ms::align_up((size_t)ndir * N * H * sizeof(float), 256);
  L.dbg = o; o += ms::align_up((size_t)ndir * std::max(H / 8, 1) * 16 * sizeof(unsigned long long), 256);
  L.row_off = o; o += ms::align_up((size_t)(T + 1) * sizeof(int), 256);
  L.xsplit = o; o += ms::align_up((size_t)T * N * In * 4, 256);
  L.total = o;
  return L;
}


__global__ void pack_rows_fast_kernel(const float* __restrict__ w, float* __restrict__ dst, int H, int In) {
  const int row = blockIdx.x;
  const int j = row / 32, g = (row % 32) / 8, u = row % 8;
  const float* src = w + (size_t)(g * H + 8 * j + u) * In;
  float* d = dst + (size_t)row * In;
  for (int k = threadIdx.x; k < In; k += blockDim.x) d[k] = src[k];
}

template <int P>
__global__ void pack_rows_split_kernel(const float* __restrict__ w, unsigned short* __restrict__ hi,
                                       unsigned short* __restrict__ lo, int H, int In) {
  constexpr bool F16 = ms::prec_one_plane(P), HM = P == ms::PREC_F16X3;
  const int row = blockIdx.x;
  const int j = row / 32, g = (row % 32) / 8, u = row % 8;
  const float* src = w + (size_t)(g * H + 8 * j + u) * In;
  for (int k = threadIdx.x; k < In; k += blockDim.x) {
    const float x = src[k];
    if (F16) {
      hi[(size_t)row * In + k] = __builtin_bit_cast(unsigned short, (_Float16)x);
    } else {
      unsigned hb, lb;
      ms::plane_split<HM>(x, hb, lb);
      hi[(size_t)row * In + k] = (unsigned short)hb;
      lo[(size_t)row * In + k] = (unsigned short)lb;
    }
  }
}

__global__ void pack_bias_fast_kernel(const float* __restrict__ b_ih, const float* __restrict__ b_hh,
                                      float* __restrict__ dst, int H) {
  const int row = blockIdx.x * blockDim.x + threadIdx.x;
  if (row >= 4 * H) return;
  const int j = row / 32, g = (row % 32) / 8, u = row % 8;
  const int src = g * H + 8 * j + u;
  dst[row] = (b_ih ? b_ih[src] : 0.f) + (b_hh ? b_hh[src] : 0.f);
}

__global__ void pack_whh_fast_kernel(const float* __restrict__ w, float* __restrict__ dst, int H) {
  const size_t total = (size_t)4 * H * H;
  for (size_t i = (size_t)blockIdx.x * blockDim.x + threadIdx.x; i < total; i += (size_t)gridDim.x * blockDim.x) {
    const int e = i & 3;
    const int r = (i >> 2) & 31;
    const int kq = (i >> 7) % (H / 4);
    const int j = (i >> 7) / (H / 4);
    const int g = r >> 3, u = r & 7;
    dst[i] = w[(size_t)(g * H + 8 * j + u) * H + 4 * kq + e];
  }
}

template <int P>
__global__ void pack_whh_split_kernel(const float* __restrict__ w, unsigned short* __restrict__ dst, int H) {
  constexpr bool F16 = ms::prec_one_plane(P), HM = P == ms::PREC_F16X3;
  const size_t total = (size_t)4 * H * H;
  const int KG = H / 8;
  for (size_t i = (size_t)blockIdx.x * blockDim.x + threadIdx.x; i < total; i += (size_t)gridDim.x * blockDim.x) {
    const int e = i & 7;
    const int r = (i >> 3) & 31;
    const int kg = (i >> 8) % KG;
    const int j = (i >> 8) / KG;
    const int g = r >> 3, u = r & 7;
    const float x = w[(size_t)(g * H + 8 * j + u) * H + 8 * kg + e];
    const size_t base = (size_t)j * 2 * KG * 256 + ((size_t)kg * 32 + r) * 8 + e;
    if (F16) {
      dst[base] = __builtin_bit_cast(unsigned short, (_Float16)x);
      dst[base + (size_t)KG * 256] = 0;
    } else {
      unsigned hb, lb;
      ms::plane_split<HM>(x, hb, lb);
      dst[base] = (unsigned short)hb;
      dst[base + (size_t)KG * 256] = (unsigned short)lb;
    }
  }
}

__global__ void copy_or_zero_kernel(const float* __restrict__ src, float* __restrict__ dst, size_t n) {
  for (size_t i = (size_t)blockIdx.x * blockDim.x + threadIdx.x; i < n; i += (size_t)gridDim.x * blockDim.x)
    dst[i] = src ? src[i] : 0.f;
}

int blocks_for(size_t n) { return (int)std::min<size_t>((n + 255) / 256, 2048); }


__device__ __forceinline__ float sigmoidf_(float v) { return 1.0f / (1.0f + expf(-v)); }
__device__ __forceinline__ float fast_sigmoid(float v) {
  return __builtin_amdgcn_rcpf(1.0f + __builtin_amdgcn_exp2f(-1.44269504088896f * v));
}
__device__ __forceinline__ float fast_tanh(float v) {
  return 1.0f - 2.0f * __builtin_amdgcn_rcpf(1.0f + __builtin_amdgcn_exp2f(2.88539008177793f * v));
}
__device__ __forceinline__ float clamp01(float v) { return fminf(fmaxf(v, 0.f), 1.f); }
__device__ __forceinline__ float clamp11(float v) { return fminf(fmaxf(v, -1.f), 1.f); }

__device__ __forceinline__ float wave_sum(float v) {
#pragma unroll
  for (int o = 32; o > 0; o >>= 1) v += __shfl_xor(v, o, 64);
  return v;
}

struct StepP {
  const float* xproj;
  const float* whh;
  const float* bhh;
  const int32_t* lens;
  const float* h_prev;
  float* h_next;
  float* c_state;
  float* out;
  float* hn;
  float* cn;
  int s, steps, N, H, ndir;
};

template <int CELL>
__global__ __launch_bounds__(64) void rnn_step_generic_kernel(StepP p) {
  constexpr int G = (CELL == MS_CELL_LSTM || CELL == MS_CELL_HARD_LSTM) ? 4 : (CELL == MS_CELL_GRU ? 3 : 1);
  const int u = blockIdx.x, d = blockIdx.y, lane = threadIdx.x;
  const int t = d ? (p.steps - 1 - p.s) : p.s;
  const int H = p.H, N = p.N;
  const size_t GH = (size_t)G * H;
  const float* wbase = p.whh + (size_t)d * GH * H;
  for (int n = 0; n < N; ++n) {
    const float* hp = p.h_prev + ((size_t)d * N + n) * H;
    float part[G];
#pragma unroll
    for (int g = 0; g < G; ++g) part[g] = 0.f;
    for (int k = lane; k < H; k += 64) {
      const float hv = hp[k];
#pragma unroll
      for (int g = 0; g < G; ++g) part[g] += wbase[((size_t)g * H + u) * H + k] * hv;
    }
#pragma unroll
    for (int g = 0; g < G; ++g) part[g] = wave_sum(part[g]);
    if (lane == 0) {
      const bool active = p.lens ? (t < p.lens[n]) : true;
      const size_t sidx = ((size_t)d * N + n) * H + u;
      const float* xp = p.xproj + ((size_t)t * N + n) * (p.ndir * GH) + d * GH;
      const float* bh = p.bhh + d * GH;
      const float hold = hp[u];
      float hnew, cnew = 0.f;
// ... 35 lines not shown
  __shared__ f32x4 red[3][G][NT][64];
  const int tid = threadIdx.x, lane = tid & 63, wave = tid >> 6;
  const int x = lane & 15, kq = lane >> 4;
  const int u0 = blockIdx.x * 16, d = blockIdx.y, n0 = blockIdx.z * (16 * NT);
  const int H = p.H, N = p.N;
  const int t = d ? (p.steps - 1 - p.s) : p.s;
  const size_t GH = (size_t)G * H;
  const float* wbase = p.whh + (size_t)d * GH * H;
  const float* hbase = p.h_prev + (size_t)d * N * H;
  const int kbeg = wave * (H / 4), kend = kbeg + H / 4;

  f32x4 acc[G][NT];
  const float* arow[NT];
  const float* brow[G];
#pragma unroll
  for (int nt = 0; nt < NT; ++nt) arow[nt] = hbase + (size_t)min(n0 + nt * 16 + x, N - 1) * H + 4 * kq;
#pragma unroll
  for (int g = 0; g < G; ++g) {
    brow[g] = wbase + ((size_t)g * H + u0 + x) * H + 4 * kq;
#pragma unroll
    for (int nt = 0; nt < NT; ++nt) acc[g][nt] = f32x4{0.f, 0.f, 0.f, 0.f};
  }
  constexpr int D = 2;
  f32x4 a[D][2][NT], b[D][2][G];
  auto load_stage = [&](int st, int kb) {
#pragma unroll
    for (int hf = 0; hf < 2; ++hf) {
      if (kb + 16 * hf < kend) {
#pragma unroll
        for (int nt = 0; nt < NT; ++nt) a[st][hf][nt] = *reinterpret_cast<const f32x4*>(arow[nt] + kb + 16 * hf);
#pragma unroll
        for (int g = 0; g < G; ++g) b[st][hf][g] = *reinterpret_cast<const f32x4*>(brow[g] + kb + 16 * hf);
      }
    }
  };
#pragma unroll
  for (int st = 0; st < D; ++st)
    if (kbeg + 32 * st < kend) load_stage(st, kbeg + 32 * st);
  for (int kb0 = kbeg; kb0 < kend; kb0 += 32 * D) {
#pragma unroll
    for (int st = 0; st < D; ++st) {
      const int kb = kb0 + 32 * st;
      if (kb < kend) {
#pragma unroll
        for (int hf = 0; hf < 2; ++hf) {
          if (kb + 16 * hf < kend) {
#pragma unroll
            for (int e = 0; e < 4; ++e)
#pragma unroll
              for (int g = 0; g < G; ++g)
#pragma unroll
                for (int nt = 0; nt < NT; ++nt)
                  acc[g][nt] = __builtin_amdgcn_mfma_f32_16x16x4f32(a[st][hf][nt][e], b[st][hf][g][e], acc[g][nt], 0, 0, 0);
          }
        }
        if (kb + 32 * D < kend) load_stage(st, kb + 32 * D);
      }
    }
  }
  if (wave > 0) {
#pragma unroll
    for (int g = 0; g < G; ++g)
#pragma unroll
      for (int nt = 0; nt < NT; ++nt) red[wave - 1][g][nt][lane] = acc[g][nt];
  }
  __syncthreads();
  if (wave > 0) return;
#pragma unroll
  for (int g = 0; g < G; ++g)
#pragma unroll
    for (int nt = 0; nt < NT; ++nt)
#pragma unroll
      for (int w2 = 0; w2 < 3; ++w2) acc[g][nt] += red[w2][g][nt][lane];

  const int u = u0 + x;
  const float* bh = p.bhh + d * GH;
#pragma unroll
  for (int nt = 0; nt < NT; ++nt)
#pragma unroll
    for (int r = 0; r < 4; ++r) {
      const int n = n0 + nt * 16 + 4 * kq + r;
      if (n >= N) continue;
      const bool active = p.lens ? (t < p.lens[n]) : true;
      const size_t sidx = ((size_t)d * N + n) * H + u;
      const float* xp = p.xproj + ((size_t)t * N + n) * (p.ndir * GH) + d * GH;
      const float hold = hbase[(size_t)n * H + u];
      float hnew, cnew = 0.f;
      if (CELL == MS_CELL_LSTM || CELL == MS_CELL_HARD_LSTM) {
        const float gi = xp[u] + (acc[0][nt][r] + bh[u]);
        const float gf = xp[H + u] + (acc[1 % G][nt][r] + bh[H + u]);
        const float gg = xp[2 * H + u] + (acc[2 % G][nt][r] + bh[2 * H + u]);
        const float go = xp[3 * H + u] + (acc[3 % G][nt][r] + bh[3 * H + u]);
        const float cold = p.c_state[sidx];
        if (CELL == MS_CELL_LSTM) {
          cnew = sigmoidf_(gf) * cold + sigmoidf_(gi) * tanhf(gg);
          hnew = sigmoidf_(go) * tanhf(cnew);
        } else {
          cnew = clamp01(0.2f * gf + 0.5f) * cold + clamp01(0.2f * gi + 0.5f) * clamp11(gg);
          hnew = clamp01(0.2f * go + 0.5f) * clamp11(cnew);
        }
        const float cs = active ? cnew : cold;
        p.c_state[sidx] = cs;
        if (p.s == p.steps - 1) p.cn[sidx] = cs;
      } else if (CELL == MS_CELL_GRU) {
        const float rg = sigmoidf_(xp[u] + (acc[0][nt][r] + bh[u]));
        const float z = sigmoidf_(xp[H + u] + (acc[1 % G][nt][r] + bh[H + u]));
        const float nn = tanhf(xp[2 * H + u] + rg * (acc[2 % G][nt][r] + bh[2 * H + u]));
        hnew = (1.0f - z) * nn + z * hold;
      } else {
        hnew = tanhf(xp[u] + (acc[0][nt][r] + bh[u]));
      }
      const float hs = active ? hnew : hold;
      p.h_next[sidx] = hs;
      if (p.s == p.steps - 1) p.hn[sidx] = hs;
      p.out[((size_t)t * N + n) * (p.ndir * H) + d * H + u] = active ? hnew : 0.f;
    }
}

template <int CELL>
static void launch_step_mfma(const StepP& p, hipStream_t stream) {
  const int tiles = ms::cdiv(p.N, 16);
  if (tiles == 1)
    hipLaunchKernelGGL((rnn_step_mfma_kernel<CELL, 1>), dim3(p.H / 16, p.ndir, 1), dim3(256), 0, stream, p);
  else if (tiles == 2)
    hipLaunchKernelGGL((rnn_step_mfma_kernel<CELL, 2>), dim3(p.H / 16, p.ndir, 1), dim3(256), 0, stream, p);
  else
    hipLaunchKernelGGL((rnn_step_mfma_kernel<CELL, 4>), dim3(p.H / 16, p.ndir, ms::cdiv(p.N, 64)), dim3(256), 0, stream, p);
}


struct LstmP {
  const float* xproj;
  const float* whh;
  const int32_t* lens;
  const float* h0;
  const float* c0;
  float* out;
  float* hn;
  float* cn;
  float* hx;
  unsigned* flags;
  unsigned* status;
  unsigned long long* dbg;
  int steps, N, n_base, N_total, H, ndir, J, NPAD;
  int d_base;
  int grp_wgs;
  int poll_sleep;
  int xcd_map;
  int ring_shift;
  unsigned short* out_hi;
  unsigned short* out_lo;
  const int32_t* row_off;
  int s_begin, s_end;
};

__device__ __forceinline__ f32x4 load_sc1_b128(__amdgpu_buffer_rsrc_t rsrc, int byte_off) {
  auto v = __builtin_amdgcn_raw_buffer_load_b128(rsrc, byte_off, 0,  16);
  return __builtin_bit_cast(f32x4, v);
}

__device__ __forceinline__ void store_sc1_f32(float* p, float v) {
  __hip_atomic_store(p, v, __ATOMIC_RELAXED, __HIP_MEMORY_SCOPE_AGENT);
}

__device__ __forceinline__ void flag_timeout(unsigned* status) {
  __hip_atomic_store(status, 1u, __ATOMIC_RELAXED, __HIP_MEMORY_SCOPE_AGENT);
  __hip_atomic_store(status - STATUS_BYTES / sizeof(unsigned), 1u, __ATOMIC_RELAXED, __HIP_MEMORY_SCOPE_AGENT);
}

__device__ __forceinline__ bool wait_flags(const unsigned* flags, int count, unsigned epoch, unsigned* status, int lane) {
  const unsigned long long t0 = wall_clock64();
  unsigned spins = 0;
  for (;;) {
    unsigned v = epoch;
    if (lane < count) v = __hip_atomic_load(flags + lane, __ATOMIC_RELAXED, __HIP_MEMORY_SCOPE_AGENT);
    if (__all((int)(v - epoch) >= 0)) return true;
    if ((++spins & 63u) == 0) {
      const unsigned dead = __hip_atomic_load(status, __ATOMIC_RELAXED, __HIP_MEMORY_SCOPE_AGENT);
      if (dead != 0 || wall_clock64() - t0 > SPIN_LIMIT_TICKS) {
        if (lane == 0) flag_timeout(status);
        return false;
      }
    }
    __builtin_amdgcn_s_sleep(1);
  }
}

template <int NB, bool HARD, bool PIPE, bool STAMP = false>
__global__ __launch_bounds__(256, 1) void lstm_persistent_kernel(LstmP p) {
  extern __shared__ __attribute__((aligned(16))) float smem[];
  float* Ws = smem;
  float* red = smem + (size_t)p.H * 32;

  const int tid = threadIdx.x, lane = tid & 63, wave = __builtin_amdgcn_readfirstlane(tid >> 6);
  const int l31 = lane & 31, half = lane >> 5;
  const int d = blockIdx.x / p.J, j = blockIdx.x % p.J;
  const int H = p.H, N = p.N, KQ = H / 4;
  const int nl = tid >> 3, u = tid & 7;
  const int unit = 8 * j + u;

  {
    const f32x4* src = reinterpret_cast<const f32x4*>(p.whh + ((size_t)d * p.J + j) * H * 32);
    f32x4* dst = reinterpret_cast<f32x4*>(Ws);
    for (int i = tid; i < H * 8; i += 256) dst[i] = src[i];
  }

  float c[NB], h[NB];
  int len_n[NB];
  float* hx_d = p.hx + (size_t)d * 2 * KQ * p.NPAD * 4;
  const int hx_slot = ((unit >> 2) * p.NPAD) * 4 + (unit & 3);
#pragma unroll
  for (int b = 0; b < NB; ++b) {
    const int n = b * 32 + nl;
    const bool valid = n < N;
    const size_t sidx = ((size_t)d * p.N_total + p.n_base + n) * H + unit;
    h[b] = (valid && p.h0) ? p.h0[sidx] : 0.f;
    c[b] = (valid && p.c0) ? p.c0[sidx] : 0.f;
    len_n[b] = valid ? (p.lens ? p.lens[p.n_base + n] : p.steps) : 0;
    store_sc1_f32(hx_d + hx_slot + n * 4, h[b]);
  }
  asm volatile("s_waitcnt vmcnt(0)" ::: "memory");
  __syncthreads();
  unsigned* my_flag = p.flags + d * p.J + j;
  if (tid == 0) __hip_atomic_store(my_flag, 1u, __ATOMIC_RELAXED, __HIP_MEMORY_SCOPE_AGENT);

  const __amdgpu_buffer_rsrc_t hx_rsrc =
      __builtin_amdgcn_make_buffer_rsrc(hx_d, 0, 2 * KQ * p.NPAD * 16, 0x00020000);
  const unsigned* wave_flags = p.flags + d * p.J + wave * (p.J / 4);
  const int kq_base = wave * (KQ / 4);
  const int xcols = p.ndir * 4 * H;
  bool alive = true;
  unsigned long long st_sum[4] = {0, 0, 0, 0}, st_prev = 0;
  if (STAMP) st_prev = wall_clock64();

  for (int s = 0; s < p.steps; ++s) {
    const int t = d ? (p.steps - 1 - s) : s;
    const int par = s & 1;

    float xg[NB][4];
#pragma unroll
    for (int b = 0; b < NB; ++b) {
      const int n = b * 32 + nl;
      const float* xp = p.xproj + ((size_t)t * p.N_total + p.n_base + n) * xcols + d * 4 * H + j * 32 + u;
#pragma unroll
      for (int g = 0; g < 4; ++g) xg[b][g] = (n < N) ? xp[g * 8] : 0.f;
    }

    if (alive) alive = wait_flags(wave_flags, p.J / 4, (unsigned)(s + 1), p.status, lane);
    if (STAMP) { const unsigned long long now = wall_clock64(); st_sum[0] += now - st_prev; st_prev = now; }

    f32x16 acc[NB];
#pragma unroll
    for (int b = 0; b < NB; ++b)
#pragma unroll
      for (int r = 0; r < 16; ++r) acc[b][r] = 0.f;

    const int hx_par = par * KQ * p.NPAD * 16;
    const int iters = KQ / 8;
    if (PIPE) {
      f32x4 a0[8][NB], a1[8][NB];
      auto issue = [&](int it0, f32x4(&a)[8][NB]) {
#pragma unroll
        for (int i = 0; i < 8; ++i) {
          const int kq = kq_base + 2 * (it0 + i) + half;
#pragma unroll
          for (int b = 0; b < NB; ++b) a[i][b] = load_sc1_b128(hx_rsrc, hx_par + (kq * p.NPAD + b * 32 + l31) * 16);
        }
      };
      auto compute = [&](int it0, f32x4(&a)[8][NB]) {
#pragma unroll
        for (int i = 0; i < 8; ++i) {
          const int kq = kq_base + 2 * (it0 + i) + half;
          const f32x4 bw = *reinterpret_cast<const f32x4*>(Ws + (kq * 32 + l31) * 4);
#pragma unroll
          for (int b = 0; b < NB; ++b)
#pragma unroll
            for (int e = 0; e < 4; ++e)
              acc[b] = __builtin_amdgcn_mfma_f32_32x32x2f32(a[i][b][e], bw[e], acc[b], 0, 0, 0);
        }
      };
      issue(0, a0);
      for (int it0 = 0; it0 < iters; it0 += 16) {
        const bool more1 = it0 + 8 < iters;
        if (more1) issue(it0 + 8, a1);
        compute(it0, a0);
        if (it0 + 16 < iters) issue(it0 + 16, a0);
        if (more1) compute(it0 + 8, a1);
      }
    } else {
      for (int it = 0; it < iters; ++it) {
        const int kq = kq_base + 2 * it + half;
        const f32x4 bw = *reinterpret_cast<const f32x4*>(Ws + (kq * 32 + l31) * 4);
#pragma unroll
        for (int b = 0; b < NB; ++b) {
          const f32x4 a = load_sc1_b128(hx_rsrc, hx_par + (kq * p.NPAD + b * 32 + l31) * 16);
#pragma unroll
          for (int e = 0; e < 4; ++e) acc[b] = __builtin_amdgcn_mfma_f32_32x32x2f32(a[e], bw[e], acc[b], 0, 0, 0);
        }
      }
    }

    if (STAMP) { const unsigned long long now = wall_clock64(); st_sum[1] += now - st_prev; st_prev = now; }
    float hout[NB];
#pragma unroll
    for (int b = 0; b < NB; ++b) {
      if (b > 0) __syncthreads();
// ... 523 lines not shown
          const f16x8v xh = __builtin_bit_cast(f16x8v, ah[ks]);
          acc0 = __builtin_amdgcn_mfma_f32_16x16x32_f16(xh, __builtin_bit_cast(f16x8v, wh0[ks]), acc0, 0, 0, 0);
          acc1 = __builtin_amdgcn_mfma_f32_16x16x32_f16(xh, __builtin_bit_cast(f16x8v, wh1[ks]), acc1, 0, 0, 0);
        } else {
          const u32x4 bh0 = wh0[ks], bh1 = wh1[ks];
          const u32x4 bl0 = WL_LDS ? wlds[((wave * KS + ks) * 2 + 0) * 64 + lane] : wl0[ks];
          const u32x4 bl1 = WL_LDS ? wlds[((wave * KS + ks) * 2 + 1) * 64 + lane] : wl1[ks];
          const u32x4 xh = ah[ks], xl = al[ks];
          acc0 = ms::mfma_16x16x32<HM>(xh, bh0, acc0);
          acc1 = ms::mfma_16x16x32<HM>(xh, bh1, acc1);
          acc0 = ms::mfma_16x16x32<HM>(xl, bh0, acc0);
          acc1 = ms::mfma_16x16x32<HM>(xl, bh1, acc1);
          acc0 = ms::mfma_16x16x32<HM>(xh, bl0, acc0);
          acc1 = ms::mfma_16x16x32<HM>(xh, bl1, acc1);
        }
      }
      if (STAMP) st_sum[1] += spins;

      float* redb = red + sg * RED2;
#pragma unroll
      for (int i = 0; i < 4; ++i) {
        redb[(wave * 16 + 4 * q + i) * RED_STRIDE + c16] = acc0[i];
        redb[(wave * 16 + 4 * q + i) * RED_STRIDE + 16 + c16] = acc1[i];
      }
      __syncthreads();
      if (STAMP) { const unsigned long long now = wall_clock64(); st_sum[2] += now - st_prev; st_prev = now; }
      if (wave < 2) {
        float gsum[4];
#pragma unroll
        for (int g = 0; g < 4; ++g) {
          float v = xg[g];
#pragma unroll
          for (int w2 = 0; w2 < 4; ++w2) v += redb[(w2 * 16 + nl) * RED_STRIDE + g * 8 + u];
          gsum[g] = v;
        }
        float cnew, hnew;
        if (HARD) {
          cnew = clamp01(0.2f * gsum[1] + 0.5f) * c[sg] + clamp01(0.2f * gsum[0] + 0.5f) * clamp11(gsum[2]);
          hnew = clamp01(0.2f * gsum[3] + 0.5f) * clamp11(cnew);
        } else {
          cnew = fast_sigmoid(gsum[1]) * c[sg] + fast_sigmoid(gsum[0]) * fast_tanh(gsum[2]);
          hnew = fast_sigmoid(gsum[3]) * fast_tanh(cnew);
        }
        const bool active = t < len_n[sg];
        c[sg] = active ? cnew : c[sg];
        h[sg] = active ? hnew : h[sg];
        const int off = sg * STREAM + ec.wpar * KG * 256 + j * 256 + nl * 16;
        publish_split<P>(h[sg], wtag, hx_rsrc, off, PLANE + off, lane);
        if (n < N) {
          const size_t oidx = ((size_t)t * p.N_total + n_base + n) * (p.ndir * H) + d * H + unit;
          const float ov = active ? hnew : 0.f;
          if (p.out_hi) {
            if (F16) {
              p.out_hi[oidx] = __builtin_bit_cast(unsigned short, (_Float16)ov);
            } else {
              unsigned hb, lb;
              ms::plane_split_bounded<HM>(ov, hb, lb);
              p.out_hi[oidx] = (unsigned short)hb;
              p.out_lo[oidx] = (unsigned short)lb;
            }
          } else {
            p.out[oidx] = ov;
          }
        }
      }
      if (STAMP) { const unsigned long long now = wall_clock64(); st_sum[3] += now - st_prev; st_prev = now; }
    }
  }
  if (STAMP && (tid & 63) == 0) {
    for (int k = 0; k < 4; ++k) atomicAdd(&p.dbg[(size_t)blockIdx.x * 8 + (wave >= 2 ? 4 : 0) + k], st_sum[k]);
  }
  if (wave < 2) {
#pragma unroll
    for (int sg = 0; sg < 2; ++sg) {
      const int n = sg * 16 + nl;
      if (n < N) {
        const size_t sidx = ((size_t)d * p.N_total + n_base + n) * H + unit;
        p.hn[sidx] = h[sg];
        p.cn[sidx] = c[sg];
      }
    }
  }
}


constexpr int WIDE_RED_STRIDE = 72;
constexpr int WIDE_RED2 = 8 * 16 * WIDE_RED_STRIDE;

template <int KS, bool CELL, bool HARD, bool STAMP = false, bool PACKED = false, int P = ms::PREC_BF16X3>
__device__ __forceinline__ void wide2_wave(const LstmP& p, float* red, const int k0, const int32_t* __restrict__ row_off) {
  constexpr bool F16 = ms::prec_one_plane(P), HM = P == ms::PREC_F16X3;
  constexpr int H = 1024, KG = H / 8;

  const int tid = threadIdx.x, lane = tid & 63, wave = __builtin_amdgcn_readfirstlane(tid >> 6);
  const int c16 = lane & 15, q = lane >> 4;
  const int JJ = p.J / 2;
  int grp = blockIdx.x / (p.ndir * JJ);
  const int rem = blockIdx.x % (p.ndir * JJ);
  int d = rem / JJ, jj = rem % JJ;
  if (p.xcd_map) {
    const int xcd = blockIdx.x & 7;
    grp = xcd >> 2;
    d = (xcd >> 1) & 1;
    jj = (blockIdx.x >> 3) * 2 + (xcd & 1);
  }
  const int n_base = p.n_base + 32 * grp;
  const int N = min(32, p.N - 32 * grp);
  const int cb = (tid >> 7) & 1, nl = (tid >> 3) & 15, u = tid & 7;
  const int jb = 2 * jj + cb;
  const int unit = 8 * jb + u;

  u32x4 wh[2][2][KS], wl[2][2][F16 ? 1 : KS];
#pragma unroll
  for (int b = 0; b < 2; ++b) {
    const char* wsrc = reinterpret_cast<const char*>(p.whh) + ((size_t)d * p.J + 2 * jj + b) * 128 * H;
#pragma unroll
    for (int ks = 0; ks < KS; ++ks) {
      const int kg = 4 * (k0 + ks) + q;
      const char* wp = wsrc + (kg * 32 + c16) * 16;
      wh[b][0][ks] = *reinterpret_cast<const u32x4*>(wp);
      wh[b][1][ks] = *reinterpret_cast<const u32x4*>(wp + 256);
      if (!F16) {
        wl[b][0][ks] = *reinterpret_cast<const u32x4*>(wp + KG * 512);
        wl[b][1][ks] = *reinterpret_cast<const u32x4*>(wp + KG * 512 + 256);
      }
    }
  }

  const int rs = p.ring_shift;
  const int PLANE = (KG * 256) << rs;
  const int STREAM = 2 * PLANE;
  char* hx_d = reinterpret_cast<char*>(p.hx) + ((size_t)grp * p.ndir + d) * 2 * STREAM;
  const __amdgpu_buffer_rsrc_t hx_rsrc = __builtin_amdgcn_make_buffer_rsrc(hx_d, 0, 2 * STREAM, 0x00020000);

  float c[2] = {0.f, 0.f}, h[2] = {0.f, 0.f};
  int len_n[2] = {0, 0};
  if (CELL) {
#pragma unroll
    for (int sg = 0; sg < 2; ++sg) {
      const int n = sg * 16 + nl;
      const bool valid = n < N;
      const size_t sidx = ((size_t)d * p.N_total + n_base + n) * H + unit;
      h[sg] = (valid && p.h0) ? p.h0[sidx] : 0.f;
      c[sg] = (valid && p.c0) ? p.c0[sidx] : 0.f;
      len_n[sg] = valid ? (p.lens ? p.lens[n_base + n] : p.steps) : 0;
      const EpochClock ec0 = epoch_clock(d, p.s_begin, p.steps, rs);
      const int off = sg * STREAM + ec0.par * KG * 256 + jb * 256 + nl * 16;
      publish_split<P>(h[sg], ec0.em & 1u, hx_rsrc, off, PLANE + off, lane, valid);
    }
  }
  __syncthreads();

  const int xcols = p.ndir * 4 * H;
  const int lane_off = q * 256 + c16 * 16;
  const bool row_ok[2] = {c16 < N, 16 + c16 < N};
  const int loff[2] = {row_ok[0] ? lane_off : 0x40000000, row_ok[1] ? lane_off : 0x40000000};
  bool alive = true;
  unsigned long long st_sum[5] = {0, 0, 0, 0, 0}, st_prev = 0;
  if (STAMP) st_prev = wall_clock64();

  int roff_next = (PACKED && CELL) ? row_off[d ? p.steps - 1 - p.s_begin : p.s_begin] : 0;
  for (int s = p.s_begin; s < p.s_end; ++s) {
    const int t = d ? (p.steps - 1 - s) : s;
    const int roff = roff_next;
    if (PACKED && CELL) roff_next = row_off[s + 1 < p.steps ? (d ? t - 1 : t + 1) : t];
    const EpochClock ec = epoch_clock(d, s, p.steps, rs);
    const int par = ec.par;
    const unsigned em = ec.em;
    const unsigned wtag = ec.wtag;
#pragma unroll
    for (int sg = 0; sg < 2; ++sg) {
      float xg[4] = {0.f, 0.f, 0.f, 0.f};
      const int n = sg * 16 + nl;
      if (CELL && n < N) {
        const size_t row = PACKED ? (size_t)(roff + (t < len_n[sg] ? n_base + n : 0)) : (size_t)t * p.N_total + n_base + n;
        const float* xp = p.xproj + row * xcols + d * 4 * H + jb * 32 + u;
#pragma unroll
        for (int g = 0; g < 4; ++g) xg[g] = xp[g * 8];
      }

      const int base = sg * STREAM + par * KG * 256 + k0 * 1024;
      u32x4 ah[KS], al[F16 ? 1 : KS];
      const unsigned long long t_wait0 = wall_clock64();
      unsigned spins = 0;
#pragma unroll
      for (int ks = 0; ks < KS; ++ks) {
        ah[ks] = __builtin_amdgcn_raw_buffer_load_b128(hx_rsrc, loff[sg], base + ks * 1024,  16);
        if (!F16) al[ks] = __builtin_amdgcn_raw_buffer_load_b128(hx_rsrc, loff[sg], PLANE + base + ks * 1024,  16);
      }
      f32x4v acc[2][2];
#pragma unroll
      for (int b = 0; b < 2; ++b)
#pragma unroll
        for (int ct = 0; ct < 2; ++ct) acc[b][ct] = f32x4v{0.f, 0.f, 0.f, 0.f};
      auto mfma_step = [&](int ks) {
        if (F16) {
          const f16x8v xf = __builtin_bit_cast(f16x8v, ah[ks]);
#pragma unroll
          for (int b = 0; b < 2; ++b) {
            acc[b][0] = __builtin_amdgcn_mfma_f32_16x16x32_f16(xf, __builtin_bit_cast(f16x8v, wh[b][0][ks]), acc[b][0], 0, 0, 0);
            acc[b][1] = __builtin_amdgcn_mfma_f32_16x16x32_f16(xf, __builtin_bit_cast(f16x8v, wh[b][1][ks]), acc[b][1], 0, 0, 0);
          }
          return;
        }
        const u32x4 xh = ah[ks], xl = al[F16 ? 0 : ks];
#pragma unroll
        for (int b = 0; b < 2; ++b) {
          const u32x4 bh0 = wh[b][0][ks], bh1 = wh[b][1][ks], bl0 = wl[b][0][F16 ? 0 : ks], bl1 = wl[b][1][F16 ? 0 : ks];
          acc[b][0] = ms::mfma_16x16x32<HM>(xh, bh0, acc[b][0]);
          acc[b][1] = ms::mfma_16x16x32<HM>(xh, bh1, acc[b][1]);
          acc[b][0] = ms::mfma_16x16x32<HM>(xl, bh0, acc[b][0]);
          acc[b][1] = ms::mfma_16x16x32<HM>(xl, bh1, acc[b][1]);
          acc[b][0] = ms::mfma_16x16x32<HM>(xh, bl0, acc[b][0]);
          acc[b][1] = ms::mfma_16x16x32<HM>(xh, bl1, acc[b][1]);
        }
      };
      for (;;) {
        unsigned bad = 0;
#pragma unroll
        for (int ks = 0; ks < KS; ++ks)
#pragma unroll
          for (int e = 0; e < 4; ++e) bad |= (ah[ks][e] ^ em) | (F16 ? 0u : (al[F16 ? 0 : ks][e] ^ em));
        if (!alive || !__any(row_ok[sg] && (bad & 0x00010001u) != 0)) break;
        if ((++spins & 63u) == 0) {
          const unsigned dead = __hip_atomic_load(p.status, __ATOMIC_RELAXED, __HIP_MEMORY_SCOPE_AGENT);
          if (dead != 0 || wall_clock64() - t_wait0 > SPIN_LIMIT_TICKS) {
            if (lane == 0) flag_timeout(p.status);
            alive = false;
            break;
          }
        }
        for (int z = 0; z < p.poll_sleep; ++z) __builtin_amdgcn_s_sleep(1);
#pragma unroll
        for (int ks = 0; ks < KS; ++ks) {
          ah[ks] = __builtin_amdgcn_raw_buffer_load_b128(hx_rsrc, loff[sg], base + ks * 1024, (int)(0x80000000u | 16u));
          if (!F16) al[ks] = __builtin_amdgcn_raw_buffer_load_b128(hx_rsrc, loff[sg], PLANE + base + ks * 1024, (int)(0x80000000u | 16u));
        }
      }
      if (STAMP) { const unsigned long long now = wall_clock64(); st_sum[0] += now - st_prev; st_prev = now; st_sum[1] += spins; }
#pragma unroll
      for (int ks = 0; ks < KS; ++ks) mfma_step(ks);

      float* redb = red + sg * WIDE_RED2;
#pragma unroll
      for (int b = 0; b < 2; ++b)
#pragma unroll
        for (int ct = 0; ct < 2; ++ct)
#pragma unroll
          for (int i = 0; i < 4; ++i) redb[(wave * 16 + 4 * q + i) * WIDE_RED_STRIDE + b * 32 + ct * 16 + c16] = acc[b][ct][i];
      if (STAMP) {
        __builtin_amdgcn_s_waitcnt(0xc07f);
        const unsigned long long now = wall_clock64(); st_sum[2] += now - st_prev; st_prev = now;
      }
      __syncthreads();
      if (STAMP) { const unsigned long long now = wall_clock64(); st_sum[3] += now - st_prev; st_prev = now; }
      if (CELL) {
        float gsum[4];
#pragma unroll
        for (int g = 0; g < 4; ++g) {
          float v = xg[g];
#pragma unroll
          for (int w2 = 0; w2 < 8; ++w2) v += redb[(w2 * 16 + nl) * WIDE_RED_STRIDE + cb * 32 + g * 8 + u];
          gsum[g] = v;
        }
        float cnew, hnew;
        if (HARD) {
          cnew = clamp01(0.2f * gsum[1] + 0.5f) * c[sg] + clamp01(0.2f * gsum[0] + 0.5f) * clamp11(gsum[2]);
          hnew = clamp01(0.2f * gsum[3] + 0.5f) * clamp11(cnew);
        } else {
          cnew = fast_sigmoid(gsum[1]) * c[sg] + fast_sigmoid(gsum[0]) * fast_tanh(gsum[2]);
          hnew = fast_sigmoid(gsum[3]) * fast_tanh(cnew);
        }
        const bool active = t < len_n[sg];
        c[sg] = active ? cnew : c[sg];
        h[sg] = active ? hnew : h[sg];
        const int off = sg * STREAM + ec.wpar * KG * 256 + jb * 256 + nl * 16;
        publish_split<P>(h[sg], wtag, hx_rsrc, off, PLANE + off, lane, n < N);
        if (n < N) {
          const size_t oidx = ((size_t)t * p.N_total + n_base + n) * (p.ndir * H) + d * H + unit;
          const float ov = active ? hnew : 0.f;
          if (p.out_hi) {
            const size_t prow = active ? (size_t)(roff + n_base + n) : (size_t)p.steps * p.N_total - 1;
            const size_t pidx = PACKED ? (prow * (p.ndir * H) + d * H + unit) : oidx;
            if (F16) {
              p.out_hi[pidx] = __builtin_bit_cast(unsigned short, (_Float16)ov);
            } else {
              unsigned hb, lb;
              ms::plane_split_bounded<HM>(ov, hb, lb);
              p.out_hi[pidx] = (unsigned short)hb;
              p.out_lo[pidx] = (unsigned short)lb;
            }
          } else {
            p.out[oidx] = ov;
          }
        }
        if (STAMP) { const unsigned long long now = wall_clock64(); st_sum[4] += now - st_prev; st_prev = now; }
      }
    }
  }
  if (STAMP && lane == 0) {
    for (int k = 0; k < 5; ++k) atomicAdd(&p.dbg[(size_t)blockIdx.x * 16 + (CELL ? 0 : 8) + k], st_sum[k]);
  }
  if (CELL) {
#pragma unroll
    for (int sg = 0; sg < 2; ++sg) {
      const int n = sg * 16 + nl;
      if (n < N) {
        const size_t sidx = ((size_t)d * p.N_total + n_base + n) * H + unit;
        p.hn[sidx] = h[sg];
        p.cn[sidx] = c[sg];
      }
    }
  }
}

template <bool HARD, int KSC, bool STAMP = false, bool PACKED = false, int P = ms::PREC_BF16X3>
__global__ __launch_bounds__(512, 2) void lstm_persistent_wide2_kernel(LstmP p, const int32_t* __restrict__ row_off) {
  static_assert(KSC >= 1 && KSC <= 7, "both wave sets need at least one k-step");
  extern __shared__ __attribute__((aligned(16))) float smem[];
  const int wave = __builtin_amdgcn_readfirstlane(threadIdx.x >> 6);
  if (wave < 4) wide2_wave<KSC, true, HARD, STAMP, PACKED, P>(p, smem, wave * KSC, row_off);
  else wide2_wave<8 - KSC, false, HARD, STAMP, false, P>(p, smem, 4 * KSC + (wave - 4) * (8 - KSC), row_off);
}



__global__ void pack_whh_f32x2_kernel(const float* __restrict__ w, float* __restrict__ dst, int H) {
  const size_t total = (size_t)4 * H * H;
  const int G = H / 64;
  for (size_t i = (size_t)blockIdx.x * blockDim.x + threadIdx.x; i < total; i += (size_t)gridDim.x * blockDim.x) {
    const int e = i & 3, lane = (i >> 2) & 63, c = (i >> 8) & 1;
// ... 701 lines not shown
  if (attr_once.need()) {
    MS_HIP(hipFuncSetAttribute((const void*)lstm_persistent_wide2_kernel<false, 3, false, false, P>, hipFuncAttributeMaxDynamicSharedMemorySize, (int)lds));
    MS_HIP(hipFuncSetAttribute((const void*)lstm_persistent_wide2_kernel<true, 3, false, false, P>, hipFuncAttributeMaxDynamicSharedMemorySize, (int)lds));
    MS_HIP(hipFuncSetAttribute((const void*)lstm_persistent_wide2_kernel<false, 4, false, false, P>, hipFuncAttributeMaxDynamicSharedMemorySize, (int)lds));
    if (P == ms::PREC_F16) {
      MS_HIP(hipFuncSetAttribute((const void*)lstm_persistent_wide2_kernel<false, 2, false, false, ms::PREC_F16>, hipFuncAttributeMaxDynamicSharedMemorySize, (int)lds));
    } else {
      MS_HIP(hipFuncSetAttribute((const void*)lstm_persistent_wide2_kernel<true, 4, false, false, P>, hipFuncAttributeMaxDynamicSharedMemorySize, (int)lds));
      MS_HIP(hipFuncSetAttribute((const void*)lstm_persistent_wide2_kernel<false, 3, true, false, P>, hipFuncAttributeMaxDynamicSharedMemorySize, (int)lds));
      MS_HIP(hipFuncSetAttribute((const void*)lstm_persistent_wide2_kernel<false, 3, false, true, P>, hipFuncAttributeMaxDynamicSharedMemorySize, (int)lds));
      MS_HIP(hipFuncSetAttribute((const void*)lstm_persistent_wide2_kernel<true, 3, false, true, P>, hipFuncAttributeMaxDynamicSharedMemorySize, (int)lds));
    }
    attr_once.done();
  }
  const dim3 grid(groups * p.ndir * (p.J / 2));
  if constexpr (P == ms::PREC_F16) {
    static const int kf = getenv("MS_LSTM_WIDE_KSC_F16") ? atoi(getenv("MS_LSTM_WIDE_KSC_F16")) : 3;
    if (hard) hipLaunchKernelGGL((lstm_persistent_wide2_kernel<true, 3, false, false, P>), grid, dim3(512), lds, stream, p, p.row_off);
    else if (kf == 4) hipLaunchKernelGGL((lstm_persistent_wide2_kernel<false, 4, false, false, P>), grid, dim3(512), lds, stream, p, p.row_off);
    else if (kf == 2) hipLaunchKernelGGL((lstm_persistent_wide2_kernel<false, 2, false, false, P>), grid, dim3(512), lds, stream, p, p.row_off);
    else hipLaunchKernelGGL((lstm_persistent_wide2_kernel<false, 3, false, false, P>), grid, dim3(512), lds, stream, p, p.row_off);
    MS_LAUNCH_CHECK();
    return MS_OK;
  } else {
  static const bool stamps = getenv("MS_LSTM_STAMPS") && getenv("MS_LSTM_STAMPS")[0] == '1';
  if (p.row_off != nullptr) {
    if (hard) hipLaunchKernelGGL((lstm_persistent_wide2_kernel<true, 3, false, true, P>), grid, dim3(512), lds, stream, p, p.row_off);
    else hipLaunchKernelGGL((lstm_persistent_wide2_kernel<false, 3, false, true, P>), grid, dim3(512), lds, stream, p, p.row_off);
    MS_LAUNCH_CHECK();
    return MS_OK;
  }
  if (stamps && !hard) {
    hipLaunchKernelGGL((lstm_persistent_wide2_kernel<false, 3, true, false, P>), grid, dim3(512), lds, stream, p, p.row_off);
    MS_LAUNCH_CHECK();
    return MS_OK;
  }
  static const int ksc = getenv("MS_LSTM_WIDE_KSC") ? atoi(getenv("MS_LSTM_WIDE_KSC")) : 3;
  if (hard) {
    if (ksc == 4) hipLaunchKernelGGL((lstm_persistent_wide2_kernel<true, 4, false, false, P>), grid, dim3(512), lds, stream, p, p.row_off);
    else hipLaunchKernelGGL((lstm_persistent_wide2_kernel<true, 3, false, false, P>), grid, dim3(512), lds, stream, p, p.row_off);
  } else {
    if (ksc == 4) hipLaunchKernelGGL((lstm_persistent_wide2_kernel<false, 4, false, false, P>), grid, dim3(512), lds, stream, p, p.row_off);
    else hipLaunchKernelGGL((lstm_persistent_wide2_kernel<false, 3, false, false, P>), grid, dim3(512), lds, stream, p, p.row_off);
  }
  MS_LAUNCH_CHECK();
  return MS_OK;
  }
}
static int launch_wide2(const LstmP& p, bool hard, int groups, int prec, hipStream_t stream) {
  if (prec == ms::PREC_F16) return launch_wide2_p<ms::PREC_F16>(p, hard, groups, stream);
  if (prec == ms::PREC_F16X3) return launch_wide2_p<ms::PREC_F16X3>(p, hard, groups, stream);
  return launch_wide2_p<ms::PREC_BF16X3>(p, hard, groups, stream);
}

bool use_wide(int cell, int H, int ndir, int N) {
  static const int mode = getenv("MS_LSTM_WIDE") ? atoi(getenv("MS_LSTM_WIDE")) : -1;
  if (mode == 0) return false;
  if (H != 1024 || N > 64 || !use_split(cell, H, ndir) || ms::precision_mode() == ms::PREC_F32) return false;
  static std::atomic<int> ok[64];
  int dev = 0;
  if (hipGetDevice(&dev) != hipSuccess) return false;
  int v = ok[dev & 63].load(std::memory_order_relaxed);
  if (v == 0) {
    int nb = 0;
    const size_t lds = (size_t)2 * WIDE_RED2 * sizeof(float);
    const bool fits = hipFuncSetAttribute((const void*)lstm_persistent_wide2_kernel<false, 3, false, false, ms::PREC_F16X3>, hipFuncAttributeMaxDynamicSharedMemorySize, (int)lds) == hipSuccess &&
                      hipOccupancyMaxActiveBlocksPerMultiprocessor(&nb, (const void*)lstm_persistent_wide2_kernel<false, 3, false, false, ms::PREC_F16X3>, 512, lds) == hipSuccess &&
                      nb >= 1;
    v = fits ? 1 : 2;
    ok[dev & 63].store(v, std::memory_order_relaxed);
  }
  if (v != 1) return false;
  return ms::cdiv(N, 32) * ndir * (H / 16) <= ms::num_cus();
}

template <int G, bool HARD>
static int launch_f32x2(const LstmP& p, hipStream_t stream) {
  const size_t lds = (size_t)RED_FLOATS * sizeof(float);
  hipLaunchKernelGGL((lstm_persistent_f32x2_kernel<G, HARD>), dim3(p.ndir * p.J), dim3(256), lds, stream, p);
  MS_LAUNCH_CHECK();
  return MS_OK;
}

static int launch_f32x2_any(const LstmP& p, bool hard, hipStream_t stream) {
  switch (p.H) {
    case 256: return hard ? launch_f32x2<4, true>(p, stream) : launch_f32x2<4, false>(p, stream);
    case 512: return hard ? launch_f32x2<8, true>(p, stream) : launch_f32x2<8, false>(p, stream);
    case 768: return hard ? launch_f32x2<12, true>(p, stream) : launch_f32x2<12, false>(p, stream);
    default: return hard ? launch_f32x2<16, true>(p, stream) : launch_f32x2<16, false>(p, stream);
  }
}

template <int P>
static int launch_split2_prec(const LstmP& p, bool hard, bool stamps, hipStream_t stream) {
  switch (p.H) {
    case 256: return hard ? launch_split2<2, true, false, P>(p, stream) : launch_split2<2, false, false, P>(p, stream);
    case 512: return hard ? launch_split2<4, true, false, P>(p, stream) : launch_split2<4, false, false, P>(p, stream);
    case 768: return hard ? launch_split2<6, true, false, P>(p, stream) : launch_split2<6, false, false, P>(p, stream);
    default: break;
  }
  if constexpr (P != ms::PREC_F16) {
    switch (p.H) {
      case 1280: return hard ? launch_split2<10, true, false, P>(p, stream) : launch_split2<10, false, false, P>(p, stream);
      case 1536: return hard ? launch_split2<12, true, false, P>(p, stream) : launch_split2<12, false, false, P>(p, stream);
      case 2048: return hard ? launch_split2<16, true, false, P>(p, stream) : launch_split2<16, false, false, P>(p, stream);
      default: break;
    }
    if (stamps && !hard) return launch_split2<8, false, true, P>(p, stream);
  }
  return hard ? launch_split2<8, true, false, P>(p, stream) : launch_split2<8, false, false, P>(p, stream);
}
static int launch_split2_any(const LstmP& p, bool hard, bool stamps, int prec, hipStream_t stream) {
  if (prec == ms::PREC_F16) return launch_split2_prec<ms::PREC_F16>(p, hard, stamps, stream);
  if (prec == ms::PREC_F16X3) return launch_split2_prec<ms::PREC_F16X3>(p, hard, stamps, stream);
  return launch_split2_prec<ms::PREC_BF16X3>(p, hard, stamps, stream);
}

extern "C" int ms_rnn_layer_chains_planes(int cell, int H, int ndir) {
  static const bool off = getenv("MS_RNN_CHAIN_PLANES") && getenv("MS_RNN_CHAIN_PLANES")[0] == '0';
  if (off || cell < 0 || cell > MS_CELL_HARD_LSTM) return 0;
  if (use_gru_persistent(cell, H, ndir)) return use_split_gemm(cell, H, ndir, ndir * H) ? 1 : 0;
  return use_split(cell, H, ndir) && two_stream_shape(H) && use_split_gemm(cell, H, ndir, ndir * H) &&
         !(getenv("MS_LSTM_ONE_STREAM") && getenv("MS_LSTM_ONE_STREAM")[0] == '1') ? 1 : 0;
}

extern "C" int ms_rnn_layer_is_wide(int cell, int H, int ndir, int N) {
  if (cell < 0 || cell > MS_CELL_HARD_LSTM || H <= 0 || ndir < 1 || ndir > 2 || N <= 0) return 0;
  return use_fast(cell, H, ndir) && use_wide(cell, H, ndir, N) ? 1 : 0;
}

extern "C" int ms_rnn_layer_forward(int cell, const void* packed, const float* x, const int32_t* lens, int max_len,
                                    const float* h0, const float* c0, float* out, float* hn, float* cn, int T, int N,
                                    int In, int H, int ndir, void* workspace, size_t workspace_bytes, void* stream_) {
  return ms_rnn_layer_forward_ex(cell, packed, x, lens, max_len, h0, c0, out, hn, cn, T, N, In, H, ndir, 0, workspace,
                                 workspace_bytes, stream_);
}

static bool two_stream_pairs_groups(int cell, int H, int ndir) {
  static const bool off = getenv("MS_LSTM_PAIR_GROUPS") && getenv("MS_LSTM_PAIR_GROUPS")[0] == '0';
  static const bool one_stream = getenv("MS_LSTM_ONE_STREAM") && getenv("MS_LSTM_ONE_STREAM")[0] == '1';
  if (off || !use_fast(cell, H, ndir) || !use_split(cell, H, ndir) || !two_stream_shape(H)) return false;
  if (one_stream && !use_f16(cell, H, ndir) && H <= 1024) return false;
  return 2 * ndir * (H / 8) <= ms::num_cus();
}

static bool layer_packs_rows(int cell, int steps, int N, int In, int H, int ndir) {
  static const bool off = getenv("MS_RNN_PACKED") && getenv("MS_RNN_PACKED")[0] == '0';
  if (off || !(cell == MS_CELL_LSTM || cell == MS_CELL_HARD_LSTM)) return false;
  const int GH4 = 4 * H;
  return use_fast(cell, H, ndir) && use_wide(cell, H, ndir, std::min(N, 64)) && use_split_gemm(cell, H, ndir, In) && !use_f16(cell, H, ndir) &&
         ms::gemm_rows_from_device_ok(steps * N, 32, ndir * GH4) && (size_t)steps * N * std::max(In, ndir * H) * 2 < ((size_t)1 << 31);
}

extern "C" int ms_rnn_layer_packs_rows(int cell, int T, int N, int In, int H, int ndir) {
  if (cell < 0 || cell > MS_CELL_HARD_LSTM || T <= 0 || N <= 0 || In <= 0 || H <= 0 || (ndir != 1 && ndir != 2)) return 0;
  return layer_packs_rows(cell, T, N, In, H, ndir) ? 1 : 0;
}

extern "C" int ms_rnn_layer_forward_ex(int cell, const void* packed, const float* x, const int32_t* lens, int max_len,
                                       const float* h0, const float* c0, float* out, float* hn, float* cn, int T, int N,
                                       int In, int H, int ndir, int flags, void* workspace, size_t workspace_bytes,
                                       void* stream_) {
  MS_REQUIRE(cell >= 0 && cell <= MS_CELL_HARD_LSTM, "unknown cell");
  MS_REQUIRE(T > 0 && N > 0 && In > 0 && H > 0 && (ndir == 1 || ndir == 2), "bad shape");
  const bool x_in_ws = (flags & MS_RNN_X_PLANES_IN_WS) != 0, out_to_ws = (flags & MS_RNN_OUT_PLANES_TO_WS) != 0;
  MS_REQUIRE(!(x_in_ws || out_to_ws) || ms_rnn_layer_chains_planes(cell, H, ndir), "this layer kind does not chain planes");
  MS_REQUIRE(!x_in_ws || use_split_gemm(cell, H, ndir, In), "input planes need the split GEMM (In % 32 == 0)");
  MS_REQUIRE(packed && (x || x_in_ws) && (out || out_to_ws) && hn && workspace, "null pointer");
  const bool lstm_like = (cell == MS_CELL_LSTM || cell == MS_CELL_HARD_LSTM);
  MS_REQUIRE(!lstm_like || cn, "cn required for LSTM cells");
  MS_REQUIRE(max_len >= 1 && max_len <= T, "max_len must be in [1, T]");
  hipStream_t stream = (hipStream_t)stream_;
  const int G = gates_of(cell);
  const size_t GH = (size_t)G * H;
  const WsLayout W = ws_layout(cell, T, N, H, ndir, In);
  const size_t need = out_to_ws ? std::max(W.total, W.xsplit + ms::align_up((size_t)T * N * ndir * H * 4, 256)) : W.total;
  if (workspace_bytes < need) {
    ms::set_error("ms_rnn_layer_forward: workspace too small");
    return MS_ERR_WORKSPACE;
  }
  const PackLayout L = pack_layout(cell, In, H, ndir);
  const char* pk = (const char*)packed;
  char* ws = (char*)workspace;
  const int steps = max_len;
  const bool fast = use_fast(cell, H, ndir);
  const int hx_region = (flags >> 8) & 15;
  MS_REQUIRE(hx_region < HX_REGIONS, "exchange region out of range");
  const bool hx_preinit = (flags & MS_RNN_HX_PREINIT) != 0;
  MS_REQUIRE(!hx_preinit || hx_preinit_ok(cell, N, H, ndir), "MS_RNN_HX_PREINIT on a layer kind ms_rnn_hx_preinit does not serve");
  char* hx_ptr = ws + W.hx + (size_t)hx_region * W.hx_bytes;
  const bool packed_rows = (flags & MS_RNN_PACKED_ROWS) != 0 && lens != nullptr && layer_packs_rows(cell, steps, N, In, H, ndir);
  MS_REQUIRE(packed_rows || !(flags & MS_RNN_PACKED_ROWS) || lens == nullptr || !(x_in_ws || out_to_ws),
             "MS_RNN_PACKED_ROWS on a chained layer that cannot pack its rows (ask ms_rnn_layer_packs_rows for every layer of the stack)");
  int32_t* row_off = (int32_t*)(ws + W.row_off);
  if (packed_rows) {
    hipLaunchKernelGGL(row_offsets_kernel, dim3(1), dim3(256), 0, stream, lens, N, steps, row_off);
    MS_LAUNCH_CHECK();
  }

  const bool hx_path = use_split(cell, H, ndir) || use_f32x2(cell, H, ndir) || use_gru_persistent(cell, H, ndir);
  const bool projection_only = (flags & MS_RNN_PROJECTION_ONLY) != 0;
  MS_REQUIRE(!(projection_only && (flags & MS_RNN_RECURRENCE_ONLY)), "MS_RNN_PROJECTION_ONLY and MS_RNN_RECURRENCE_ONLY exclude each other");
  if (!hx_path && !projection_only) MS_HIP(hipMemsetAsync(ws + W.status, 0, W.xproj - W.status, stream));
  auto zero_base = [&](int n0) { return (unsigned*)(ws + (n0 == 0 ? W.status : W.flags)); };
  auto zero_words = [&](int n0) { return (int)((W.xproj - (n0 == 0 ? W.status : W.flags)) / sizeof(unsigned)); };
  if (steps < T && out && !projection_only)
    MS_HIP(hipMemsetAsync(out + (size_t)steps * N * ndir * H, 0, (size_t)(T - steps) * N * ndir * H * sizeof(float),
                          stream));

  float* xproj = (float*)(ws + W.xslot(0));
  int rc;
  if (flags & MS_RNN_RECURRENCE_ONLY) {
    rc = MS_OK;
  } else {
    ProfScope prof(MS_PROF_PROJECTION, stream);
    if (use_split_gemm(cell, H, ndir, In)) {
      unsigned short* xh = (unsigned short*)(ws + W.xsplit);
      unsigned short* xl = xh + (size_t)steps * N * In;
      const unsigned short* wh = (const unsigned short*)(pk + L.wih);
      const unsigned short* wl = wh + (size_t)ndir * GH * In;
      const int prec = layer_prec(cell, H, ndir);
      if (x_in_ws) {
        rc = MS_OK;
      } else if (packed_rows) {
        auto kern = prec == ms::PREC_F16X3 ? split_planes_packed_kernel<true> : split_planes_packed_kernel<false>;
        hipLaunchKernelGGL(kern, dim3(steps * N), dim3(256), 0, stream, x, xh, xl, lens, row_off, N, In);
        rc = hipGetLastError() == hipSuccess ? MS_OK : MS_ERR_HIP;
      } else {
        rc = ms::split_planes_launch(x, xh, xl, (size_t)steps * N * In, prec, stream);
      }
      if (rc == MS_OK) {
        ProfScope gemm_only(In >= 1024 ? MS_PROF_GEMM_K_LARGE : MS_PROF_GEMM_K_SMALL, stream);
        rc = ms::gemm_bf16x3_launch_rows(xh, xl, wh, wl, (const float*)(pk + L.bias_x), xproj, steps * N, In, (int)(ndir * GH),
                                         MS_ACT_NONE, 0.f, 0.f, prec, stream, packed_rows ? row_off + steps : nullptr);
      }
    } else {
      ProfScope gemm_only(In >= 1024 ? MS_PROF_GEMM_K_LARGE : MS_PROF_GEMM_K_SMALL, stream);
      rc = ms::linear_launch(x, (const float*)(pk + L.wih), (const float*)(pk + L.bias_x), xproj, steps * N, In,
                             (int)(ndir * GH), MS_ACT_NONE, 0.f, 0.f, stream);
    }
  }
  if (rc != MS_OK) return rc;
  if (projection_only) return MS_OK;

  if (fast) {
    PersistentTurn turn(stream);
    if (turn.rc != MS_OK) { ms::set_error("ms_rnn_layer_forward: cross-stream hand-over of the persistent launch failed"); return turn.rc; }
    ProfScope prof_rec(MS_PROF_RECURRENCE, stream);
    const bool f32x2 = use_f32x2(cell, H, ndir);
    const bool wide_rows = use_wide(cell, H, ndir, std::min(N, 64));
    const bool pair_groups = !wide_rows && two_stream_pairs_groups(cell, H, ndir);
    const int group = (wide_rows || pair_groups) ? 64 : ((use_split(cell, H, ndir) && two_stream_shape(H)) || f32x2) ? 32 : 64;
    for (int n0 = 0; n0 < N; n0 += group) {
      const int ng = std::min(group, N - n0);
      if (n0 > 0 && !hx_path) MS_HIP(hipMemsetAsync(ws + W.flags, 0, W.xproj - W.flags, stream));
      LstmP p;
      p.xproj = xproj;
      p.whh = (const float*)(pk + L.whh);
      p.lens = lens;
      p.h0 = h0; p.c0 = c0; p.out = out; p.hn = hn; p.cn = cn;
      p.out_hi = p.out_lo = nullptr;
      p.row_off = packed_rows ? row_off : nullptr;
      if (out_to_ws) {
        p.out_hi = (unsigned short*)(ws + W.xsplit);
        p.out_lo = p.out_hi + (size_t)steps * N * ndir * H;
      }
      p.hx = (float*)hx_ptr;
      p.flags = (unsigned*)(ws + W.flags);
      p.status = (unsigned*)(ws + W.status);
      p.steps = steps; p.N = ng; p.n_base = n0; p.N_total = N; p.H = H; p.ndir = ndir; p.J = H / 8;
      p.d_base = 0;
      p.grp_wgs = 0;
      p.s_begin = 0; p.s_end = steps;
      p.NPAD = ms::cdiv(ng, 32) * 32;
      {
        static const int ps = getenv("MS_LSTM_POLL_SLEEP") ? atoi(getenv("MS_LSTM_POLL_SLEEP")) : 1;
        p.poll_sleep = ps > 0 ? ps : 1;
      }
      const bool hard = (cell == MS_CELL_HARD_LSTM);
      p.dbg = (unsigned long long*)(ws + W.dbg);
      const bool pipe = (H % 256 == 0);
      static const bool stamps = getenv("MS_LSTM_STAMPS") && getenv("MS_LSTM_STAMPS")[0] == '1';
      if (wide_rows) {
        const int groups = ms::cdiv(ng, 32);
        const int rs = 1;
        const size_t words_per_dir = (size_t)32 * H << rs;
        p.ring_shift = rs;
        p.N = ng;
        {
          static const bool on = getenv("MS_LSTM_WIDE_XCD") && getenv("MS_LSTM_WIDE_XCD")[0] == '1';
          p.xcd_map = (on && groups == 2 && ndir == 2 && p.J == 128) ? 1 : 0;
        }
        if (!hx_preinit || n0 > 0) {
          hipLaunchKernelGGL(hx_init_kernel, dim3(blocks_for(words_per_dir * ndir * groups)), dim3(256), 0, stream,
                             (unsigned*)hx_ptr, words_per_dir, (size_t)8 * H, ndir * groups, steps, rs, zero_base(n0), zero_words(n0), ndir);
          MS_LAUNCH_CHECK();
        }
        if (stamps) MS_HIP(hipMemsetAsync(ws + W.dbg, 0, W.row_off - W.dbg, stream));
        rc = launch_wide2(p, cell == MS_CELL_HARD_LSTM, groups, layer_prec(cell, H, ndir), stream);
        if (rc != MS_OK) return rc;
        continue;
      }
      if (use_split(cell, H, ndir)) {
        const bool hard_ = (cell == MS_CELL_HARD_LSTM);
        if (stamps) MS_HIP(hipMemsetAsync(ws + W.dbg, 0, W.row_off - W.dbg, stream));
        static const bool one_stream = getenv("MS_LSTM_ONE_STREAM") && getenv("MS_LSTM_ONE_STREAM")[0] == '1';
        const bool two_stream = (p.NPAD == 32 || pair_groups) && two_stream_shape(H) && (!one_stream || use_f16(cell, H, ndir) || H > 1024);
        const int groups = (two_stream && pair_groups) ? ms::cdiv(ng, 32) : 1;
        p.grp_wgs = groups > 1 ? ndir * p.J : 0;
        {
          const int rs = two_stream ? lstm_ring_shift() : 1;
          const size_t slab_words = two_stream ? (size_t)8 * H : (size_t)H * p.NPAD / 2;
          const size_t words_per_dir = two_stream ? ((size_t)32 * H << rs) : (size_t)2 * H * p.NPAD;
          p.ring_shift = rs;
          MS_REQUIRE(words_per_dir * ndir * groups * sizeof(unsigned) <= W.hx_bytes, "exchange region smaller than the launch's batch groups");
          if (!(hx_preinit && two_stream) || groups > 1) {
            hipLaunchKernelGGL(hx_init_kernel, dim3(blocks_for(words_per_dir * ndir * groups)), dim3(256), 0, stream,
                               (unsigned*)hx_ptr, words_per_dir, slab_words, ndir * groups, steps, rs, zero_base(n0), zero_words(n0), ndir);
            MS_LAUNCH_CHECK();
          }
        }
        if (two_stream) {
          rc = launch_split2_any(p, hard_, stamps, layer_prec(cell, H, ndir), stream);
        } else if (p.NPAD == 32 && H == 1024) {
          if (stamps && !hard_) rc = launch_split<1, 4, false, true>(p, stream);
          else rc = hard_ ? launch_split<1, 4, true>(p, stream) : launch_split<1, 4, false>(p, stream);
        } else if (p.NPAD == 32) {
          rc = hard_ ? launch_split<1, 0, true>(p, stream) : launch_split<1, 0, false>(p, stream);
        } else {
          rc = hard_ ? launch_split<2, 0, true>(p, stream) : launch_split<2, 0, false>(p, stream);
        }
        if (rc != MS_OK) return rc;
        continue;
      }
      if (f32x2) {
        hipLaunchKernelGGL(hx_init_kernel, dim3(blocks_for((size_t)64 * H * ndir)), dim3(256), 0, stream,
                           (unsigned*)hx_ptr, (size_t)64 * H, (size_t)16 * H, ndir, steps, 1, zero_base(n0), zero_words(n0), ndir);
        MS_LAUNCH_CHECK();
        rc = launch_f32x2_any(p, hard, stream);
        if (rc != MS_OK) return rc;
        continue;
      }
      if (stamps && pipe && p.NPAD == 32 && !(cell == MS_CELL_HARD_LSTM)) {
        MS_HIP(hipMemsetAsync(ws + W.dbg, 0, W.row_off - W.dbg, stream));
        rc = launch_persistent<1, false, true, true>(p, stream);
        if (rc != MS_OK) return rc;
        continue;
      }
      if (p.NPAD == 32) {
        if (pipe) rc = hard ? launch_persistent<1, true, true>(p, stream) : launch_persistent<1, false, true>(p, stream);
        else rc = hard ? launch_persistent<1, true, false>(p, stream) : launch_persistent<1, false, false>(p, stream);
      } else {
        if (pipe) rc = hard ? launch_persistent<2, true, true>(p, stream) : launch_persistent<2, false, true>(p, stream);
        else rc = hard ? launch_persistent<2, true, false>(p, stream) : launch_persistent<2, false, false>(p, stream);
      }
      if (rc != MS_OK) return rc;
    }
    return MS_OK;
  }

  if (use_gru_persistent(cell, H, ndir)) {
    PersistentTurn turn(stream);
    if (turn.rc != MS_OK) { ms::set_error("ms_rnn_layer_forward: cross-stream hand-over of the persistent launch failed"); return turn.rc; }
    ProfScope prof_rec(MS_PROF_RECURRENCE, stream);
    static const bool pair_off = getenv("MS_LSTM_PAIR_GROUPS") && getenv("MS_LSTM_PAIR_GROUPS")[0] == '0';
    const bool pair_groups = !pair_off && 2 * ndir * (H / gru_units(H)) <= ms::num_cus();
    const int rows_per_launch = pair_groups ? 64 : 32;
    for (int n0 = 0; n0 < N; n0 += rows_per_launch) {
      const int rs = lstm_ring_shift();
      const int ng = std::min(rows_per_launch, N - n0), groups = ms::cdiv(ng, 32);
      MS_REQUIRE(((size_t)32 * H << rs) * ndir * groups * sizeof(unsigned) <= W.hx_bytes, "exchange region smaller than the launch's batch groups");
      if (!hx_preinit || groups > 1) {
        hipLaunchKernelGGL(hx_init_kernel, dim3(blocks_for(((size_t)32 * H << rs) * ndir * groups)), dim3(256), 0, stream,
                           (unsigned*)hx_ptr, (size_t)32 * H << rs, (size_t)8 * H, ndir * groups, steps, rs, zero_base(n0), zero_words(n0), ndir);
        MS_LAUNCH_CHECK();
      }
      GruP g;
      g.xproj = xproj;
      g.whh = (const unsigned short*)(pk + L.whh);
      g.bhh = (const float*)(pk + L.bhh);
      g.lens = lens;
      g.h0 = h0; g.out = out; g.hn = hn;
      g.out_hi = g.out_lo = nullptr;
      if (out_to_ws) {
        g.out_hi = (unsigned short*)(ws + W.xsplit);
        g.out_lo = g.out_hi + (size_t)steps * N * ndir * H;
      }
      g.hx = (float*)hx_ptr;
      g.status = (unsigned*)(ws + W.status);
      g.steps = steps; g.N = ng; g.n_base = n0; g.N_total = N; g.ndir = ndir; g.J = H / gru_units(H);
      g.grp_wgs = groups > 1 ? ndir * g.J : 0;
      g.ring_shift = rs;
      {
        static const int ps = getenv("MS_LSTM_POLL_SLEEP") ? atoi(getenv("MS_LSTM_POLL_SLEEP")) : 1;
        g.poll_sleep = ps > 0 ? ps : 1;
      }
      const size_t lds = (size_t)RED_FLOATS * sizeof(float);
      const int launches = ndir * g.J > ms::num_cus() ? ndir : 1, dirs = (ndir / launches) * groups;
      for (int l = 0; l < launches; ++l) {
        g.d_base = l;
        switch (H) {
#define MS_GRU_CASE(HH, KS_, U_) \
          case HH:                                                                                                         \
            if (two_plane_mode() == ms::PREC_F16X3) hipLaunchKernelGGL((gru_persistent_kernel<KS_, U_, true>), dim3(dirs * g.J), dim3(256), lds, stream, g); \
            else hipLaunchKernelGGL((gru_persistent_kernel<KS_, U_, false>), dim3(dirs * g.J), dim3(256), lds, stream, g);  \
            break;
          MS_GRU_CASE(2560, 20, 10) MS_GRU_CASE(1280, 10, 10) MS_GRU_CASE(2048, 16, 8) MS_GRU_CASE(1536, 12, 8)
          MS_GRU_CASE(1024, 8, 8) MS_GRU_CASE(768, 6, 8) MS_GRU_CASE(512, 4, 8)
#undef MS_GRU_CASE
          default: ms::set_error("persistent GRU: unsupported hidden size"); return MS_ERR_UNSUPPORTED;
        }
        MS_LAUNCH_CHECK();
      }
    }
    return MS_OK;
  }

  ProfScope prof_rec(MS_PROF_RECURRENCE, stream);
  float* sh = (float*)(ws + W.state_h);
  float* sc = (float*)(ws + W.state_c);
  const size_t st = (size_t)ndir * N * H;
  hipLaunchKernelGGL(copy_or_zero_kernel, dim3(blocks_for(st)), dim3(256), 0, stream, h0, sh, st);
  if (lstm_like) hipLaunchKernelGGL(copy_or_zero_kernel, dim3(blocks_for(st)), dim3(256), 0, stream, c0, sc, st);
  MS_LAUNCH_CHECK();
  StepP p;
  p.xproj = xproj; p.whh = (const float*)(pk + L.whh); p.bhh = (const float*)(pk + L.bhh); p.lens = lens;
  p.c_state = sc; p.out = out; p.hn = hn; p.cn = cn; p.steps = steps; p.N = N; p.H = H; p.ndir = ndir;
  for (int s = 0; s < steps; ++s) {
    p.s = s;
    p.h_prev = sh + (size_t)(s & 1) * st;
    p.h_next = sh + (size_t)((s + 1) & 1) * st;
    if (!force_generic() && H % 64 == 0) {
      switch (cell) {
        case MS_CELL_LSTM: launch_step_mfma<MS_CELL_LSTM>(p, stream); break;
        case MS_CELL_GRU: launch_step_mfma<MS_CELL_GRU>(p, stream); break;
        case MS_CELL_RNN_TANH: launch_step_mfma<MS_CELL_RNN_TANH>(p, stream); break;
        default: launch_step_mfma<MS_CELL_HARD_LSTM>(p, stream); break;
      }
      continue;
    }
    dim3 grid(H, ndir);
    switch (cell) {
      case MS_CELL_LSTM: hipLaunchKernelGGL(rnn_step_generic_kernel<MS_CELL_LSTM>, grid, dim3(64), 0, stream, p); break;
      case MS_CELL_GRU: hipLaunchKernelGGL(rnn_step_generic_kernel<MS_CELL_GRU>, grid, dim3(64), 0, stream, p); break;
      case MS_CELL_RNN_TANH: hipLaunchKernelGGL(rnn_step_generic_kernel<MS_CELL_RNN_TANH>, grid, dim3(64), 0, stream, p); break;
      default: hipLaunchKernelGGL(rnn_step_generic_kernel<MS_CELL_HARD_LSTM>, grid, dim3(64), 0, stream, p); break;
    }
  }
  MS_LAUNCH_CHECK();
  return MS_OK;
}

namespace {
struct OverlapCtx {
  std::mutex mu;
  hipStream_t side = nullptr;
  hipStream_t urgent = nullptr;
  std::vector<hipEvent_t> ev;
};
OverlapCtx g_overlap[64];

int overlap_segment_steps(int steps, int N, int NG, int want) {
  want = std::max(2, want);
  const long rows = (long)steps * N;
  long j = std::max(1L, (rows + (long)want * 512) / ((long)want * 1024));
  for (; j >= 1; --j) {
    const int L = (int)((1024 * j) / N);
    if (L >= 1 && L < steps && ms::gemm_k_halves_ok(L * N, NG)) return L;
  }
  return 0;
}
}

extern "C" int ms_rnn_stack_overlap_ok(int cell, int T, int N, int In, int H, int ndir, int nl) {
  static const bool off = getenv("MS_RNN_OVERLAP") && getenv("MS_RNN_OVERLAP")[0] == '0';
  if (off || cell < 0 || cell > MS_CELL_HARD_LSTM || T <= 0 || N <= 0 || In <= 0 || nl < 2 || nl > HX_REGIONS) return 0;
  if (!overlap_shape(cell, H, ndir) || !use_fast(cell, H, ndir) || !use_wide(cell, H, ndir, N) || N > 32) return 0;
  if (!use_split_gemm(cell, H, ndir, In) || !use_split_gemm(cell, H, ndir, ndir * H)) return 0;
  if (!ms_rnn_layer_chains_planes(cell, H, ndir) || !hx_preinit_ok(cell, N, H, ndir)) return 0;
  return overlap_segment_steps(T, N, ndir * 4 * H, 8) > 0 ? 1 : 0;
}

extern "C" int ms_rnn_stack_forward(int cell, const void* const* packed_host, const float* x, const int32_t* lens, int max_len,
                                    const float* h0, const float* c0, float* out, float* hn, float* cn, int T, int N, int In, int H,
                                    int ndir, int nl, int segments, void* workspace, size_t workspace_bytes, void* stream_) {
  MS_REQUIRE(max_len >= 1 && max_len <= T, "max_len must be in [1, T]");
  MS_REQUIRE(ms_rnn_stack_overlap_ok(cell, max_len, N, In, H, ndir, nl), "this stack does not run on the overlapped schedule (ask ms_rnn_stack_overlap_ok)");
  MS_REQUIRE(packed_host && x && out && hn && cn && workspace, "null pointer");
  hipStream_t stream = (hipStream_t)stream_;
  const int steps = max_len;
  const size_t GH = (size_t)4 * H;
  const int NG = (int)(ndir * GH);
  int SL = overlap_segment_steps(steps, N, NG, segments);
  if (SL <= 0) SL = overlap_segment_steps(steps, N, NG, 8);
  MS_REQUIRE(SL > 0, "no time segmentation of this stack qualifies (ask ms_rnn_stack_overlap_ok with T = max_len)");
  const int S = std::max(1, steps / SL);
  const WsLayout W = ws_layout(cell, T, N, H, ndir, std::max(In, ndir * H));
  if (workspace_bytes < W.total) {
    ms::set_error("ms_rnn_stack_forward: workspace too small");
    return MS_ERR_WORKSPACE;
  }
  int dev = 0;
  MS_HIP(hipGetDevice(&dev));
  OverlapCtx& oc = g_overlap[dev & 63];
  std::lock_guard<std::mutex> lock(oc.mu);
  if (oc.side == nullptr) MS_HIP(hipStreamCreateWithFlags(&oc.side, hipStreamNonBlocking));
  if (oc.urgent == nullptr) {
    int lo_pri = 0, hi_pri = 0;
    MS_HIP(hipDeviceGetStreamPriorityRange(&lo_pri, &hi_pri));
    MS_HIP(hipStreamCreateWithPriority(&oc.urgent, hipStreamNonBlocking, hi_pri));
  }
  while ((int)oc.ev.size() < 4 * S) {
    hipEvent_t e;
    MS_HIP(hipEventCreateWithFlags(&e, hipEventDisableTiming));
    oc.ev.push_back(e);
  }
  char* ws = (char*)workspace;
  const bool hard = cell == MS_CELL_HARD_LSTM;
  const int prec = layer_prec(cell, H, ndir);
  int rc = ms_rnn_hx_preinit(cell, T, N, std::max(In, ndir * H), H, ndir, max_len, nl, workspace, workspace_bytes, stream_);
  if (rc != MS_OK) return rc;
  if (steps < T) MS_HIP(hipMemsetAsync(out + (size_t)steps * N * ndir * H, 0, (size_t)(T - steps) * N * ndir * H * sizeof(float), stream));
  unsigned short* xh = (unsigned short*)(ws + W.xsplit);
  {
    const PackLayout L0 = pack_layout(cell, In, H, ndir);
    const char* pk = (const char*)packed_host[0];
    ProfScope prof(MS_PROF_PROJECTION, stream);
    unsigned short* xl = xh + (size_t)steps * N * In;
    rc = ms::split_planes_launch(x, xh, xl, (size_t)steps * N * In, prec, stream);
    if (rc != MS_OK) return rc;
    ProfScope gemm_only(In >= 1024 ? MS_PROF_GEMM_K_LARGE : MS_PROF_GEMM_K_SMALL, stream);
    const unsigned short* wh = (const unsigned short*)(pk + L0.wih);
    rc = ms::gemm_bf16x3_launch_rows(xh, xl, wh, wh + (size_t)ndir * GH * In, (const float*)(pk + L0.bias_x), (float*)(ws + W.xslot(0)),
                                     steps * N, In, NG, MS_ACT_NONE, 0.f, 0.f, prec, stream, nullptr);
    if (rc != MS_OK) return rc;
  }
  const int Kc = ndir * H;
  unsigned short* ph = xh;
  unsigned short* pl = ph + (size_t)steps * N * Kc;
  const size_t st = (size_t)ndir * N * H;
  struct Batch { int a0, a1, b0, b1; hipEvent_t ev; bool waited; };
  std::vector<Batch> made_prev, made;
  static const int urgent_segments = getenv("MS_RNN_OVERLAP_URGENT") ? atoi(getenv("MS_RNN_OVERLAP_URGENT")) : 0;
  for (int l = 0; l < nl; ++l) {
    const int in_l = l == 0 ? In : Kc;
    const PackLayout L = pack_layout(cell, in_l, H, ndir);
    const char* pk = (const char*)packed_host[l];
    const bool last_layer = l + 1 == nl;
    hipEvent_t* evl = oc.ev.data() + (size_t)(l & 1) * 2 * S;
    LstmP p;
    p.xproj = (const float*)(ws + W.xslot(l & 1));
    p.whh = (const float*)(pk + L.whh);
    p.lens = lens;
    p.out = last_layer ? out : nullptr;
    p.hn = hn + l * st; p.cn = cn + l * st;
    p.out_hi = last_layer ? nullptr : ph;
    p.out_lo = last_layer ? nullptr : pl;
    p.row_off = nullptr;
    p.grp_wgs = 0;
    p.hx = (float*)(ws + W.hx + (size_t)l * W.hx_bytes);
    p.flags = (unsigned*)(ws + W.flags);
    p.status = (unsigned*)(ws + W.status);
    p.steps = steps; p.N = N; p.n_base = 0; p.N_total = N; p.H = H; p.ndir = ndir; p.J = H / 8;
    p.d_base = 0; p.NPAD = 32; p.xcd_map = 0; p.ring_shift = 1;
    p.dbg = (unsigned long long*)(ws + W.dbg);
    {
      static const int ps = getenv("MS_LSTM_POLL_SLEEP") ? atoi(getenv("MS_LSTM_POLL_SLEEP")) : 1;
      p.poll_sleep = ps > 0 ? ps : 1;
    }
    const PackLayout Ln = pack_layout(cell, Kc, H, ndir);
    const char* pkn = last_layer ? nullptr : (const char*)packed_host[l + 1];
    float* xnext = (float*)(ws + W.xslot((l + 1) & 1));
    made_prev.swap(made);
    made.clear();
    int done_lo = 0, done_hi = 0;
    int part_hi = 0;
    hipEvent_t first_half_ev = nullptr;
    {
    ProfScope prof_rec(MS_PROF_RECURRENCE, stream);
    for (int k = 0; k < S; ++k) {
      const int s0 = k * SL, s1 = k + 1 == S ? steps : (k + 1) * SL;
      static const bool wait_all = !(getenv("MS_RNN_OVERLAP_WAIT_ALL") && getenv("MS_RNN_OVERLAP_WAIT_ALL")[0] == '0');
      for (Batch& m : made_prev) {
        auto hits = [&](int q0, int q1) { return (q0 < m.a1 && m.a0 < q1) || (q0 < m.b1 && m.b0 < q1); };
        if (!m.waited && (wait_all || hits(s0, s1) || hits(steps - s1, steps - s0))) {
          MS_HIP(hipStreamWaitEvent(stream, m.ev, 0));
          m.waited = true;
        }
      }
      p.s_begin = s0; p.s_end = s1;
      p.h0 = s0 == 0 ? (h0 ? h0 + l * st : nullptr) : p.hn;
      p.c0 = s0 == 0 ? (c0 ? c0 + l * st : nullptr) : p.cn;
      {
        PersistentTurn turn(stream);
        if (turn.rc != MS_OK) { ms::set_error("ms_rnn_stack_forward: cross-stream hand-over of the persistent launch failed"); return turn.rc; }
        rc = launch_wide2(p, hard, 1, prec, stream);
        if (rc != MS_OK) return rc;
      }
      if (last_layer) continue;
      hipStream_t ss = (k + urgent_segments >= S && steps - s1 < s1 && part_hi >= steps - s1) ? oc.urgent : oc.side;
      hipEvent_t seg_done = evl[2 * k], pieces_done = evl[2 * k + 1];
      MS_HIP(hipEventRecord(seg_done, stream));
      MS_HIP(hipStreamWaitEvent(ss, seg_done, 0));
      Batch made_now{0, 0, 0, 0, pieces_done, false};
      {
        ProfScope prof(MS_PROF_PROJECTION, ss);
        const unsigned short* wh = (const unsigned short*)(pkn + Ln.wih);
        const unsigned short* wl = wh + (size_t)ndir * GH * Kc;
        const float* bias = (const float*)(pkn + Ln.bias_x);
        auto piece = [&](int t0, int t1, int kmode) -> int {
          if (t1 <= t0) return (int)MS_OK;
          if (kmode == ms::GEMM_K_SECOND && ss != oc.side && first_half_ev != nullptr)
            MS_HIP(hipStreamWaitEvent(ss, first_half_ev, 0));
          const size_t r0 = (size_t)t0 * N;
          const int koff = kmode == ms::GEMM_K_SECOND ? H : 0;
          return ms::gemm_bf16x3_launch_ld(ph + r0 * Kc + koff, pl + r0 * Kc + koff, wh + koff, wl + koff, bias, xnext + r0 * NG,
                                           (t1 - t0) * N, kmode == ms::GEMM_K_WHOLE ? Kc : H, NG, MS_ACT_NONE, 0.f, 0.f, prec, ss,
                                           nullptr, Kc, Kc, kmode);
        };
        auto cut_ok = [&](int t0, int t1) { return t1 > t0 && ms::gemm_k_halves_ok((t1 - t0) * N, NG); };
        auto complete = [&](int t0, int t1) {
          int rc2 = MS_OK;
          const int mid = std::min(std::max(part_hi, t0), t1);
          if (mid > t0 && cut_ok(t0, mid)) {
            rc2 = piece(t0, mid, ms::GEMM_K_SECOND);
            if (rc2 == MS_OK) rc2 = piece(mid, t1, ms::GEMM_K_WHOLE);
          } else {
            rc2 = piece(t0, t1, ms::GEMM_K_WHOLE);
          }
          return rc2;
        };
        const int f_k = s1, b_k = steps - s1;
        bool first_half_piece = false;
        if (b_k >= f_k) {
          if (cut_ok(part_hi, f_k)) {
            rc = piece(part_hi, f_k, ms::GEMM_K_FIRST);
            part_hi = f_k;
            first_half_piece = true;
          }
        } else {
          if (part_hi < b_k && cut_ok(part_hi, b_k)) {
            rc = piece(part_hi, b_k, ms::GEMM_K_FIRST);
            part_hi = b_k;
            first_half_piece = true;
          }
          if (rc == MS_OK) {
            if (done_hi <= done_lo) {
              rc = complete(b_k, f_k);
              made_now.a0 = b_k; made_now.a1 = f_k;
            } else {
              rc = complete(b_k, done_lo);
              if (rc == MS_OK) rc = complete(done_hi, f_k);
              made_now.a0 = b_k; made_now.a1 = done_lo; made_now.b0 = done_hi; made_now.b1 = f_k;
            }
          }
          done_lo = b_k; done_hi = f_k;
        }
        if (rc != MS_OK) return rc;
        if (first_half_piece) first_half_ev = pieces_done;
      }
      MS_HIP(hipEventRecord(pieces_done, ss));
      if (made_now.a1 > made_now.a0 || made_now.b1 > made_now.b0) made.push_back(made_now);
    }
    }
  }
  return MS_OK;
}

extern "C" size_t ms_rnn_debug_offset(int cell, int T, int N, int In, int H, int ndir) {
  return ws_layout(cell, T, N, H, ndir, In).dbg;
}

extern "C" int ms_rnn_status(const void* workspace, void* stream) {
  MS_REQUIRE(workspace, "null pointer");
  MS_HIP(hipStreamSynchronize((hipStream_t)stream));
  unsigned st = 0;
  MS_HIP(hipMemcpy(&st, workspace, sizeof(st), hipMemcpyDeviceToHost));
  if (st != 0) {
    MS_HIP(hipMemset(const_cast<void*>(workspace), 0, sizeof(st)));
    ms::set_error("ms_rnn_status: persistent LSTM kernel timed out waiting for a peer workgroup");
    return MS_ERR_TIMEOUT;
  }
  return MS_OK;
}
```

Baseline: 28670.

## Store LSTM input-projection gates in a tiled 32x8 layout for recurrence reads

The input-projection GEMM can now write its output in a tiled layout of 32-row by 8-column blocks, and the LSTM recurrence kernel reads gate inputs with tiled addressing. The goal is better locality and coalescing for the per-step gate loads in the recurrent kernel, which read scattered columns across each row. It is on by default, gated by MS_RNN_XG_TILED, and applies to H=1024 LSTM layers. It adds padded workspace rows, a dry-run check of which GEMM kernel will be used, and a forced-kernel fallback in the stack path.

```diff
diff --git a/include/ms_hotpath.h b/include/ms_hotpath.h
--- a/include/ms_hotpath.h
+++ b/include/ms_hotpath.h
@@ -134,11 +134,17 @@
                          const float* h0, const float* c0, float* out, float* hn, float* cn, int T, int N, int In, int H, int ndir,
                          int nl, int segments, void* workspace, size_t workspace_bytes, void* stream);
 
+int ms_rnn_set_xg_layout(int tiled);
+int ms_rnn_layer_xg_tiled(int cell, int T, int N, int In, int H, int ndir, int packed_rows);
+
 int ms_rnn_status(const void* workspace, void* stream);
 
 size_t ms_rnn_debug_offset(int cell, int T, int N, int In, int H, int ndir);
 
 int ms_gemm_set_variant(int variant);
+int ms_gemm_split_out_test(const float* x, const float* w, const float* bias, float* y, int M, int K, int N, int prec, int kernel,
+                           int kmode, int layout, int row0, const int32_t* m_eff, void* workspace, size_t workspace_bytes,
+                           void* stream);
 
 enum {
   MS_PROF_PROJECTION = 0, MS_PROF_RECURRENCE = 1, MS_PROF_GEMM_K_LARGE = 2, MS_PROF_GEMM_K_SMALL = 3, MS_PROF_CONV = 4,
diff --git a/myrtlespeech_amd/_lib.py b/myrtlespeech_amd/_lib.py
--- a/myrtlespeech_amd/_lib.py
+++ b/myrtlespeech_amd/_lib.py
@@ -69,10 +69,13 @@
     "ms_rnn_layer_is_wide": (c_int, [c_int] * 4),
     "ms_rnn_stack_overlap_ok": (c_int, [c_int] * 7),
     "ms_rnn_stack_forward": (c_int, [c_int, _P, _P, _P, c_int, _P, _P, _P, _P, _P] + [c_int] * 7 + [_P, c_size_t, _P]),
+    "ms_rnn_set_xg_layout": (c_int, [c_int]),
+    "ms_rnn_layer_xg_tiled": (c_int, [c_int] * 7),
     "ms_rnn_status": (c_int, [_P, _P]),
     "ms_rnn_debug_offset": (c_size_t, [c_int] * 6),
     "ms_rnn_layer_packs_rows": (c_int, [c_int] * 6),
     "ms_gemm_set_variant": (c_int, [c_int]),
+    "ms_gemm_split_out_test": (c_int, [_P, _P, _P, _P] + [c_int] * 8 + [_P, _P, c_size_t, _P]),
     "ms_prof_enable": (c_int, [c_int]),
     "ms_prof_read": (c_int, [POINTER(c_float), POINTER(c_int)]),
     "ms_clock_probe": (c_int, [_P, c_int, c_int, _P]),
diff --git a/myrtlespeech_amd/csrc/common.h b/myrtlespeech_amd/csrc/common.h
--- a/myrtlespeech_amd/csrc/common.h
+++ b/myrtlespeech_amd/csrc/common.h
@@ -66,6 +66,11 @@
 int precision_mode();
 int split_mode();
 enum { GEMM_K_WHOLE = 0, GEMM_K_FIRST = 1, GEMM_K_SECOND = 2 };
+enum { XG_ROW_MAJOR = 0, XG_TILED = 1 };
+__host__ __device__ __forceinline__ size_t xg_tiled_index(size_t m, int n, int NG) {
+  return ((m >> 5) * (size_t)(NG >> 3) + (size_t)(n >> 3)) * 256 + (m & 31) * 8 + (n & 7);
+}
+static inline size_t xg_tiled_rows(size_t M) { return (M + 31) / 32 * 32; }
 int weight_scale_launch(const float* w, size_t n, float* scale_word, int prec, hipStream_t stream);
 
 constexpr bool prec_one_plane(int P) { return P == PREC_F16; }
diff --git a/myrtlespeech_amd/csrc/gemm_split.hip b/myrtlespeech_amd/csrc/gemm_split.hip
--- a/myrtlespeech_amd/csrc/gemm_split.hip
+++ b/myrtlespeech_amd/csrc/gemm_split.hip
@@ -443,7 +443,8 @@
 __device__ __forceinline__ void gemm4_body(const unsigned short* __restrict__ Ah, const unsigned short* __restrict__ Al,
                                            const unsigned short* __restrict__ Wh, const unsigned short* __restrict__ Wl,
                                            const float* __restrict__ bias, float* __restrict__ Y, int M, int K, int N, int act,
-                                           float lo, float hi, const int* __restrict__ m_eff, int lda, int ldw, int kmode) {
+                                           float lo, float hi, const int* __restrict__ m_eff, int lda, int ldw, int kmode,
+                                           int ylayout, int row0) {
   constexpr bool F16 = prec_one_plane(P), HM = P == PREC_F16X3;
   extern __shared__ __attribute__((aligned(16))) char lds[];
   constexpr int TN = 32 * NJ * WN;
@@ -527,6 +528,9 @@
     for (int j = 0; j < NJ; ++j)
 #pragma unroll
       for (int r = 0; r < 16; ++r) acc[i][j][r] = 0.f;
+  auto yidx = [&](int m, int n) -> size_t {
+    return ylayout == XG_TILED ? xg_tiled_index((size_t)(row0 + m), n, N) : (size_t)m * N + n;
+  };
   if (kmode == GEMM_K_SECOND) {
 #pragma unroll
     for (int i = 0; i < 2; ++i) {
@@ -538,7 +542,7 @@
         for (int g = 0; g < 4; ++g) {
           const int n = n0 + wn * (32 * NJ) + j * 32 + 8 * g + 4 * half;
           if (n + 3 < N) {
-            const f32x4 v = *reinterpret_cast<const f32x4*>(Y + (size_t)m * N + n);
+            const f32x4 v = *reinterpret_cast<const f32x4*>(Y + yidx(m, n));
             acc[i][j][4 * g] = v[0]; acc[i][j][4 * g + 1] = v[1]; acc[i][j][4 * g + 2] = v[2]; acc[i][j][4 * g + 3] = v[3];
           }
         }
@@ -729,7 +733,7 @@
 #pragma unroll
             for (int e = 0; e < 4; ++e) v[e] = fminf(fmaxf(v[e], lo), hi);
           }
-          *reinterpret_cast<f32x4*>(Y + (size_t)m * N + n) = v;
+          *reinterpret_cast<f32x4*>(Y + yidx(m, n)) = v;
         } else {
 #pragma unroll
           for (int e = 0; e < 4; ++e)
@@ -750,8 +754,9 @@
                                                                  const unsigned short* __restrict__ Wl,
                                                                  const float* __restrict__ bias, float* __restrict__ Y,
                                                                  int M, int K, int N, int act, float lo, float hi,
-                                                                 const int* __restrict__ m_eff, int lda, int ldw, int kmode) {
-  gemm4_body<P, 2>(Ah, Al, Wh, Wl, bias, Y, M, K, N, act, lo, hi, m_eff, lda, ldw, kmode);
+                                                                 const int* __restrict__ m_eff, int lda, int ldw, int kmode,
+    int ylayout, int row0) {
+  gemm4_body<P, 2>(Ah, Al, Wh, Wl, bias, Y, M, K, N, act, lo, hi, m_eff, lda, ldw, kmode, ylayout, row0);
 }
 
 template <int P>
@@ -761,8 +766,9 @@
                                                                   const unsigned short* __restrict__ Wl,
                                                                   const float* __restrict__ bias, float* __restrict__ Y,
                                                                   int M, int K, int N, int act, float lo, float hi,
-                                                                  const int* __restrict__ m_eff, int lda, int ldw, int kmode) {
-  gemm4_body<P, 2, 3, false, 2>(Ah, Al, Wh, Wl, bias, Y, M, K, N, act, lo, hi, m_eff, lda, ldw, kmode);
+                                                                  const int* __restrict__ m_eff, int lda, int ldw, int kmode,
+    int ylayout, int row0) {
+  gemm4_body<P, 2, 3, false, 2>(Ah, Al, Wh, Wl, bias, Y, M, K, N, act, lo, hi, m_eff, lda, ldw, kmode, ylayout, row0);
 }
 
 template <int P>
@@ -772,16 +778,18 @@
                                                                   const unsigned short* __restrict__ Wl,
                                                                   const float* __restrict__ bias, float* __restrict__ Y,
                                                                   int M, int K, int N, int act, float lo, float hi,
-                                                                  const int* __restrict__ m_eff, int lda, int ldw, int kmode) {
-  gemm4_body<P, 2, 3, false, 2, 128>(Ah, Al, Wh, Wl, bias, Y, M, K, N, act, lo, hi, m_eff, lda, ldw, kmode);
+                                                                  const int* __restrict__ m_eff, int lda, int ldw, int kmode,
+    int ylayout, int row0) {
+  gemm4_body<P, 2, 3, false, 2, 128>(Ah, Al, Wh, Wl, bias, Y, M, K, N, act, lo, hi, m_eff, lda, ldw, kmode, ylayout, row0);
 }
 
 template <int P, int PER_STEP = 3, bool SPACED = false>
 __global__ __launch_bounds__(256, 2) void gemm_nt_bf16x3_kernel4n(
     const unsigned short* __restrict__ Ah, const unsigned short* __restrict__ Al, const unsigned short* __restrict__ Wh,
     const unsigned short* __restrict__ Wl, const float* __restrict__ bias, float* __restrict__ Y, int M, int K, int N, int act,
-    float lo, float hi, const int* __restrict__ m_eff, int lda, int ldw, int kmode) {
-  gemm4_body<P, 1, PER_STEP, SPACED>(Ah, Al, Wh, Wl, bias, Y, M, K, N, act, lo, hi, m_eff, lda, ldw, kmode);
+    float lo, float hi, const int* __restrict__ m_eff, int lda, int ldw, int kmode,
+    int ylayout, int row0) {
+  gemm4_body<P, 1, PER_STEP, SPACED>(Ah, Al, Wh, Wl, bias, Y, M, K, N, act, lo, hi, m_eff, lda, ldw, kmode, ylayout, row0);
 }
 
 static std::atomic<int> g_gemm_variant{0};
@@ -846,15 +854,22 @@
   return starved ? (long)M * N >= 1024L * 1024 : (long)M * N >= 4L * 1024 * 1024;
 }
 
-int gemm_bf16x3_launch_ld(const unsigned short* ah, const unsigned short* al, const unsigned short* wh,
-                          const unsigned short* wl, const float* bias, float* y, int M, int K, int N, int act, float lo,
-                          float hi, int prec, hipStream_t stream, const int* m_eff, int lda, int ldw, int kmode) {
+static int gemm_launch_impl(const unsigned short* ah, const unsigned short* al, const unsigned short* wh,
+                            const unsigned short* wl, const float* bias, float* y, int M, int K, int N, int act, float lo,
+                            float hi, int prec, hipStream_t stream, const int* m_eff, int lda, int ldw, int kmode, int ylayout,
+                            int row0, bool dry, int force = 0) {
   if (kmode != GEMM_K_WHOLE && !gemm_k_halves_ok(M, N)) {
-    set_error("gemm_bf16x3_launch_ld: a contraction cut along K needs an output that runs on the LDS-DMA kernels");
+    if (!dry) set_error("gemm_bf16x3_launch_ld: a contraction cut along K needs an output that runs on the LDS-DMA kernels");
     return MS_ERR_UNSUPPORTED;
   }
+  const bool tiled = ylayout == XG_TILED;
+  auto refuse_tiled = [&]() {
+    if (!dry) set_error("gemm_bf16x3_launch_out: the tiled output layout needs N % 8 == 0 and an output that runs on the LDS-DMA kernels");
+    return MS_ERR_UNSUPPORTED;
+  };
+  if ((tiled || dry) && (N % 8 != 0 || row0 < 0)) return refuse_tiled();
   static ms::DeviceOnce attr_once;
-  if (attr_once.need()) {
+  if (!dry && attr_once.need()) {
     MS_HIP(hipFuncSetAttribute((const void*)gemm_nt_bf16x3_kernel<false>, hipFuncAttributeMaxDynamicSharedMemorySize, SPLIT_LDS));
     MS_HIP(hipFuncSetAttribute((const void*)gemm_nt_bf16x3_kernel<true>, hipFuncAttributeMaxDynamicSharedMemorySize, SPLIT_LDS));
 #define MS_ATTR3(K, bytes)                                                                                         \
@@ -873,6 +888,20 @@
     MS_HIP(hipFuncSetAttribute((const void*)gemm_nt_bf16x3_kernel4n<PREC_BF16X3, 2, true>, hipFuncAttributeMaxDynamicSharedMemorySize, G4_LDS));
     attr_once.done();
   }
+  if (force != 0) {
+    if (std::max((size_t)M * lda, (size_t)N * ldw) * 2 >= ((size_t)1 << 31)) return refuse_tiled();
+    if (force == 4)
+      hipLaunchKernelGGL(MS_BY_PREC(gemm_nt_bf16x3_kernel4), dim3(cdiv(M, S2_M) * cdiv(N, S2_N)), dim3(512), G4_LDS, stream, ah, al, wh, wl,
+                         bias, y, M, K, N, act, lo, hi, m_eff, lda, ldw, kmode, ylayout, row0);
+    else if (force == 5)
+      hipLaunchKernelGGL(MS_BY_PREC(gemm_nt_bf16x3_kernel4h), dim3(cdiv(M, S2_M) * cdiv(N, 128)), dim3(512), G4_LDS, stream, ah, al, wh, wl,
+                         bias, y, M, K, N, act, lo, hi, m_eff, lda, ldw, kmode, ylayout, row0);
+    else
+      hipLaunchKernelGGL(MS_BY_PREC(gemm_nt_bf16x3_kernel4q), dim3(cdiv(M, 128) * cdiv(N, 128)), dim3(256), G4_LDS, stream, ah, al, wh, wl,
+                         bias, y, M, K, N, act, lo, hi, m_eff, lda, ldw, kmode, ylayout, row0);
+    MS_LAUNCH_CHECK();
+    return MS_OK;
+  }
   static const bool small_tile = getenv("MS_GEMM_TILE128") && getenv("MS_GEMM_TILE128")[0] == '1';
   const bool f16 = prec == PREC_F16;
   const long tiles256 = (long)cdiv(M, S2_M) * cdiv(N, S2_N);
@@ -888,6 +917,7 @@
                        bias, y, M, K, N, act, lo, hi, lda, ldw);
   };
   if (tile64() && (long)cdiv(M, S2_M) * cdiv(N, 128) * 4 <= (long)num_cus()) {
+    if (tiled || dry) return refuse_tiled();
     launch_tile64();
     MS_LAUNCH_CHECK();
     return MS_OK;
@@ -896,13 +926,15 @@
       g_gemm_variant.load(std::memory_order_relaxed) == 0 && std::max((size_t)M * lda, (size_t)N * ldw) * 2 < ((size_t)1 << 31)) {
     const char* qe = getenv("MS_GEMM_QUARTER_TILE");
     if (!(qe && qe[0] == '0') && (long)cdiv(M, S2_M) * cdiv(N, 128) * 2 <= (long)num_cus() && cdiv(M, 128) > cdiv(M, S2_M)) {
+      if (dry) return MS_OK;
       hipLaunchKernelGGL(MS_BY_PREC(gemm_nt_bf16x3_kernel4q), dim3(cdiv(M, 128) * cdiv(N, 128)), dim3(256), G4_LDS, stream, ah, al, wh, wl,
-                         bias, y, M, K, N, act, lo, hi, m_eff, lda, ldw, kmode);
+                         bias, y, M, K, N, act, lo, hi, m_eff, lda, ldw, kmode, ylayout, row0);
       MS_LAUNCH_CHECK();
       return MS_OK;
     }
+    if (dry) return MS_OK;
     hipLaunchKernelGGL(MS_BY_PREC(gemm_nt_bf16x3_kernel4h), dim3(cdiv(M, S2_M) * cdiv(N, 128)), dim3(512), G4_LDS, stream, ah, al, wh, wl,
-                       bias, y, M, K, N, act, lo, hi, m_eff, lda, ldw, kmode);
+                       bias, y, M, K, N, act, lo, hi, m_eff, lda, ldw, kmode, ylayout, row0);
     MS_LAUNCH_CHECK();
     return MS_OK;
   }
@@ -911,6 +943,7 @@
     const int variant = g_gemm_variant.load(std::memory_order_relaxed);
     static const bool regstage = getenv("MS_GEMM_REGSTAGE") && getenv("MS_GEMM_REGSTAGE")[0] == '1';
     if (variant != 2 && !regstage && std::max((size_t)M * lda, (size_t)N * ldw) * 2 < ((size_t)1 << 31)) {
+      if (dry) return MS_OK;
       if (variant >= 7 && variant <= 11) {
         auto k41 = MS_BY_PREC(gemm_nt_bf16x3_kernel4n);
         if (prec == PREC_BF16X3) {
@@ -920,15 +953,16 @@
           if (variant == 11) k41 = gemm_nt_bf16x3_kernel4n<PREC_BF16X3, 2, true>;
         }
         hipLaunchKernelGGL(k41, dim3(cdiv(M, S2_M) * cdiv(N, 128)), dim3(256), G4_LDS, stream, ah, al, wh, wl, bias, y, M, K, N,
-                           act, lo, hi, m_eff, lda, ldw, kmode);
+                           act, lo, hi, m_eff, lda, ldw, kmode, ylayout, row0);
         MS_LAUNCH_CHECK();
         return MS_OK;
       }
       hipLaunchKernelGGL(MS_BY_PREC(gemm_nt_bf16x3_kernel4), dim3(nwg2), dim3(512), G4_LDS, stream, ah, al, wh, wl, bias, y, M, K, N, act,
-                         lo, hi, m_eff, lda, ldw, kmode);
+                         lo, hi, m_eff, lda, ldw, kmode, ylayout, row0);
       MS_LAUNCH_CHECK();
       return MS_OK;
     }
+    if (tiled || dry) return refuse_tiled();
     if (m_eff != nullptr) {
       set_error("gemm_bf16x3_launch_rows: this shape does not run on the kernels that take the row count from the device");
       return MS_ERR_UNSUPPORTED;
@@ -938,6 +972,7 @@
     MS_LAUNCH_CHECK();
     return MS_OK;
   }
+  if (tiled || dry) return refuse_tiled();
   if (m_eff != nullptr) {
     set_error("gemm_bf16x3_launch_rows: this shape does not run on the kernels that take the row count from the device");
     return MS_ERR_UNSUPPORTED;
@@ -957,11 +992,63 @@
 }
 #undef MS_BY_PREC
 
+int gemm_bf16x3_launch_ld(const unsigned short* ah, const unsigned short* al, const unsigned short* wh,
+                          const unsigned short* wl, const float* bias, float* y, int M, int K, int N, int act, float lo,
+                          float hi, int prec, hipStream_t stream, const int* m_eff, int lda, int ldw, int kmode) {
+  return gemm_launch_impl(ah, al, wh, wl, bias, y, M, K, N, act, lo, hi, prec, stream, m_eff, lda, ldw, kmode, XG_ROW_MAJOR, 0, false);
+}
+
+bool gemm_tiled_out_ok(int M, int K, int N, int prec, bool rows_from_device, int lda, int ldw, int kmode);
+int gemm_bf16x3_launch_out(const unsigned short* ah, const unsigned short* al, const unsigned short* wh,
+                           const unsigned short* wl, const float* bias, float* y, int M, int K, int N, int act, float lo,
+                           float hi, int prec, hipStream_t stream, const int* m_eff, int lda, int ldw, int kmode, int ylayout,
+                           int row0, bool any_size) {
+  const int force = (ylayout == XG_TILED && any_size && !gemm_tiled_out_ok(M, K, N, prec, m_eff != nullptr, lda, ldw, kmode)) ? 6 : 0;
+  return gemm_launch_impl(ah, al, wh, wl, bias, y, M, K, N, act, lo, hi, prec, stream, m_eff, lda, ldw, kmode, ylayout, row0, false, force);
+}
+
+bool gemm_tiled_out_ok(int M, int K, int N, int prec, bool rows_from_device, int lda, int ldw, int kmode) {
+  static const int word = 0;
+  return gemm_launch_impl(nullptr, nullptr, nullptr, nullptr, nullptr, nullptr, M, K, N, MS_ACT_NONE, 0.f, 0.f, prec, nullptr,
+                          rows_from_device ? &word : nullptr, lda, ldw, kmode, XG_TILED, 0, true) == MS_OK;
+}
+
 }
 
 extern "C" int ms_gemm_set_variant(int v) {
   ms::g_gemm_variant.store(v, std::memory_order_relaxed);
   return MS_OK;
+}
+
+extern "C" int ms_gemm_split_out_test(const float* x, const float* w, const float* bias, float* y, int M, int K, int N, int prec,
+                                      int kernel, int kmode, int layout, int row0, const int32_t* m_eff, void* workspace,
+                                      size_t workspace_bytes, void* stream_) {
+  MS_REQUIRE(x && w && y && workspace, "null pointer");
+  MS_REQUIRE(M > 0 && K > 0 && N > 0 && K % 32 == 0, "bad shape (K must be a multiple of 32)");
+  MS_REQUIRE(prec == ms::PREC_BF16X3 || prec == ms::PREC_F16 || prec == ms::PREC_F16X3, "bad prec");
+  MS_REQUIRE(kernel == 0 || (kernel >= 4 && kernel <= 6), "bad kernel");
+  MS_REQUIRE(kmode == ms::GEMM_K_WHOLE || ((kmode == ms::GEMM_K_FIRST || kmode == ms::GEMM_K_SECOND) && K % 64 == 0), "bad kmode");
+  MS_REQUIRE(layout == ms::XG_ROW_MAJOR || layout == ms::XG_TILED, "bad layout");
+  MS_REQUIRE((((uintptr_t)x | (uintptr_t)w | (uintptr_t)y) & 15) == 0, "x, w and y must be 16-byte aligned");
+  if (workspace_bytes < ms_linear_split_workspace_bytes(M, K, N)) {
+    ms::set_error("ms_gemm_split_out_test: workspace too small");
+    return MS_ERR_WORKSPACE;
+  }
+  hipStream_t stream = (hipStream_t)stream_;
+  unsigned short* xh = (unsigned short*)workspace;
+  unsigned short* xl = xh + (size_t)M * K;
+  unsigned short* wh = (unsigned short*)((char*)workspace + ms::align_up((size_t)M * K * 4, 256));
+  unsigned short* wl = wh + (size_t)N * K;
+  const char* skip = getenv("MS_TIMING_SKIP_SPLIT");
+  int rc = MS_OK;
+  if (!(skip && skip[0] == '1')) {
+    rc = ms::split_planes_launch(x, xh, xl, (size_t)M * K, prec, stream);
+    if (rc == MS_OK) rc = ms::split_planes_launch(w, wh, wl, (size_t)N * K, prec, stream);
+  }
+  if (rc != MS_OK) return rc;
+  const int koff = kmode == ms::GEMM_K_SECOND ? K / 2 : 0, kc = kmode == ms::GEMM_K_WHOLE ? K : K / 2;
+  return ms::gemm_launch_impl(xh + koff, xl + koff, wh + koff, wl + koff, bias, y, M, kc, N, MS_ACT_NONE, 0.f, 0.f, prec, stream, m_eff,
+                              K, K, kmode, layout, row0, false, kernel);
 }
 
 extern "C" size_t ms_linear_split_workspace_bytes(int M, int K, int N) {
diff --git a/myrtlespeech_amd/csrc/rnn.hip b/myrtlespeech_amd/csrc/rnn.hip
--- a/myrtlespeech_amd/csrc/rnn.hip
+++ b/myrtlespeech_amd/csrc/rnn.hip
@@ -18,6 +18,11 @@
                           const unsigned short* wl, const float* bias, float* y, int M, int K, int N, int act, float lo,
                           float hi, int prec, hipStream_t stream, const int* m_eff, int lda, int ldw, int kmode);
 bool gemm_k_halves_ok(int M, int N);
+int gemm_bf16x3_launch_out(const unsigned short* ah, const unsigned short* al, const unsigned short* wh,
+                           const unsigned short* wl, const float* bias, float* y, int M, int K, int N, int act, float lo,
+                           float hi, int prec, hipStream_t stream, const int* m_eff, int lda, int ldw, int kmode, int ylayout,
+                           int row0, bool any_size);
+bool gemm_tiled_out_ok(int M, int K, int N, int prec, bool rows_from_device, int lda, int ldw, int kmode);
 int linear_launch(const float* x, const float* w, const float* bias, float* y, int M, int K, int N, int act, float lo,
                   float hi, hipStream_t stream);
 }
@@ -133,7 +138,8 @@
   L.status = o; o += STATUS_BYTES;
   L.flags = o; o += ms::align_up((size_t)ndir * std::max(H / 8, 1) * sizeof(unsigned), 256);
   L.xproj_slots = overlap_shape(cell, H, ndir) ? 2 : 1;
-  L.xproj_bytes = ms::align_up((size_t)T * N * ndir * GH * sizeof(float), 256);
+  const size_t xrows = ((cell == MS_CELL_LSTM || cell == MS_CELL_HARD_LSTM) && H == 1024) ? ms::xg_tiled_rows((size_t)T * N) : (size_t)T * N;
+  L.xproj_bytes = ms::align_up(xrows * ndir * GH * sizeof(float), 256);
   L.xproj = o; o += L.xproj_bytes * L.xproj_slots;
   L.hx = o;
   L.hx_bytes = ms::align_up(((size_t)ndir * 2 * H * std::min(npad, 64) * sizeof(float)) << (lstm_ring_shift() - 1), 256);
@@ -475,6 +481,7 @@
   unsigned short* out_lo;
   const int32_t* row_off;
   int s_begin, s_end;
+  int xg_tiled = 0;
 };
 
 __device__ __forceinline__ f32x4 load_sc1_b128(__amdgpu_buffer_rsrc_t rsrc, int byte_off) {
@@ -1304,6 +1311,8 @@
   __syncthreads();
 
   const int xcols = p.ndir * 4 * H;
+  const bool xg_tiled = p.xg_tiled != 0;
+  const int xg_col = (d * 4 * H + jb * 32) * 32 + u;
   const int lane_off = q * 256 + c16 * 16;
   const bool row_ok[2] = {c16 < N, 16 + c16 < N};
   const int loff[2] = {row_ok[0] ? lane_off : 0x40000000, row_ok[1] ? lane_off : 0x40000000};
@@ -1326,9 +1335,15 @@
       const int n = sg * 16 + nl;
       if (CELL && n < N) {
         const size_t row = PACKED ? (size_t)(roff + (t < len_n[sg] ? n_base + n : 0)) : (size_t)t * p.N_total + n_base + n;
-        const float* xp = p.xproj + row * xcols + d * 4 * H + jb * 32 + u;
-#pragma unroll
-        for (int g = 0; g < 4; ++g) xg[g] = xp[g * 8];
+        if (xg_tiled) {
+          const float* xp = p.xproj + (row >> 5) * (unsigned)(xcols * 32) + (((unsigned)row & 31u) << 3) + xg_col;
+#pragma unroll
+          for (int g = 0; g < 4; ++g) xg[g] = xp[g * 256];
+        } else {
+          const float* xp = p.xproj + row * xcols + d * 4 * H + jb * 32 + u;
+#pragma unroll
+          for (int g = 0; g < 4; ++g) xg[g] = xp[g * 8];
+        }
       }
 
       const int base = sg * STREAM + par * KG * 256 + k0 * 1024;
@@ -2336,6 +2351,35 @@
          ms::gemm_rows_from_device_ok(steps * N, 32, ndir * GH4) && (size_t)steps * N * std::max(In, ndir * H) * 2 < ((size_t)1 << 31);
 }
 
+static std::atomic<int> g_xg_tiled{-1};
+static bool xg_tiled_on() {
+  int v = g_xg_tiled.load(std::memory_order_relaxed);
+  if (v < 0) {
+    const char* e = getenv("MS_RNN_XG_TILED");
+    v = (e && e[0] == '0') ? 0 : 1;
+    g_xg_tiled.store(v, std::memory_order_relaxed);
+  }
+  return v != 0;
+}
+static bool xg_tiled_shape(int cell, int H, int ndir, int N) {
+  return (cell == MS_CELL_LSTM || cell == MS_CELL_HARD_LSTM) && use_fast(cell, H, ndir) && use_wide(cell, H, ndir, std::min(N, 64));
+}
+static bool xg_tiled_layer(int cell, int steps, int N, int In, int H, int ndir, bool packed_rows) {
+  if (!xg_tiled_on() || !xg_tiled_shape(cell, H, ndir, N) || !use_split_gemm(cell, H, ndir, In)) return false;
+  return ms::gemm_tiled_out_ok(steps * N, In, ndir * 4 * H, layer_prec(cell, H, ndir), packed_rows, In, In, ms::GEMM_K_WHOLE);
+}
+static bool xg_tiled_stack() { return xg_tiled_on(); }
+
+extern "C" int ms_rnn_set_xg_layout(int tiled) {
+  g_xg_tiled.store(tiled ? 1 : 0, std::memory_order_relaxed);
+  return MS_OK;
+}
+
+extern "C" int ms_rnn_layer_xg_tiled(int cell, int T, int N, int In, int H, int ndir, int packed_rows) {
+  if (cell < 0 || cell > MS_CELL_HARD_LSTM || T <= 0 || N <= 0 || In <= 0 || H <= 0 || (ndir != 1 && ndir != 2)) return 0;
+  return xg_tiled_layer(cell, T, N, In, H, ndir, packed_rows != 0 && layer_packs_rows(cell, T, N, In, H, ndir)) ? 1 : 0;
+}
+
 extern "C" int ms_rnn_layer_packs_rows(int cell, int T, int N, int In, int H, int ndir) {
   if (cell < 0 || cell > MS_CELL_HARD_LSTM || T <= 0 || N <= 0 || In <= 0 || H <= 0 || (ndir != 1 && ndir != 2)) return 0;
   return layer_packs_rows(cell, T, N, In, H, ndir) ? 1 : 0;
@@ -2393,6 +2437,7 @@
                           stream));
 
   float* xproj = (float*)(ws + W.xslot(0));
+  const bool xg_tiled = xg_tiled_layer(cell, steps, N, In, H, ndir, packed_rows);
   int rc;
   if (flags & MS_RNN_RECURRENCE_ONLY) {
     rc = MS_OK;
@@ -2415,8 +2460,9 @@
       }
       if (rc == MS_OK) {
         ProfScope gemm_only(In >= 1024 ? MS_PROF_GEMM_K_LARGE : MS_PROF_GEMM_K_SMALL, stream);
-        rc = ms::gemm_bf16x3_launch_rows(xh, xl, wh, wl, (const float*)(pk + L.bias_x), xproj, steps * N, In, (int)(ndir * GH),
-                                         MS_ACT_NONE, 0.f, 0.f, prec, stream, packed_rows ? row_off + steps : nullptr);
+        rc = ms::gemm_bf16x3_launch_out(xh, xl, wh, wl, (const float*)(pk + L.bias_x), xproj, steps * N, In, (int)(ndir * GH),
+                                        MS_ACT_NONE, 0.f, 0.f, prec, stream, packed_rows ? row_off + steps : nullptr, In, In,
+                                        ms::GEMM_K_WHOLE, xg_tiled ? ms::XG_TILED : ms::XG_ROW_MAJOR, 0, false);
       }
     } else {
       ProfScope gemm_only(In >= 1024 ? MS_PROF_GEMM_K_LARGE : MS_PROF_GEMM_K_SMALL, stream);
@@ -2471,6 +2517,7 @@
         const size_t words_per_dir = (size_t)32 * H << rs;
         p.ring_shift = rs;
         p.N = ng;
+        p.xg_tiled = xg_tiled ? 1 : 0;
         {
           static const bool on = getenv("MS_LSTM_WIDE_XCD") && getenv("MS_LSTM_WIDE_XCD")[0] == '1';
           p.xcd_map = (on && groups == 2 && ndir == 2 && p.J == 128) ? 1 : 0;
@@ -2702,6 +2749,8 @@
   char* ws = (char*)workspace;
   const bool hard = cell == MS_CELL_HARD_LSTM;
   const int prec = layer_prec(cell, H, ndir);
+  const bool xg_tiled = xg_tiled_stack();
+  const int xg_layout = xg_tiled ? ms::XG_TILED : ms::XG_ROW_MAJOR;
   int rc = ms_rnn_hx_preinit(cell, T, N, std::max(In, ndir * H), H, ndir, max_len, nl, workspace, workspace_bytes, stream_);
   if (rc != MS_OK) return rc;
   if (steps < T) MS_HIP(hipMemsetAsync(out + (size_t)steps * N * ndir * H, 0, (size_t)(T - steps) * N * ndir * H * sizeof(float), stream));
@@ -2715,8 +2764,8 @@
     if (rc != MS_OK) return rc;
     ProfScope gemm_only(In >= 1024 ? MS_PROF_GEMM_K_LARGE : MS_PROF_GEMM_K_SMALL, stream);
     const unsigned short* wh = (const unsigned short*)(pk + L0.wih);
-    rc = ms::gemm_bf16x3_launch_rows(xh, xl, wh, wh + (size_t)ndir * GH * In, (const float*)(pk + L0.bias_x), (float*)(ws + W.xslot(0)),
-                                     steps * N, In, NG, MS_ACT_NONE, 0.f, 0.f, prec, stream, nullptr);
+    rc = ms::gemm_bf16x3_launch_out(xh, xl, wh, wh + (size_t)ndir * GH * In, (const float*)(pk + L0.bias_x), (float*)(ws + W.xslot(0)),
+                                    steps * N, In, NG, MS_ACT_NONE, 0.f, 0.f, prec, stream, nullptr, In, In, ms::GEMM_K_WHOLE, xg_layout, 0, true);
     if (rc != MS_OK) return rc;
   }
   const int Kc = ndir * H;
@@ -2747,6 +2796,7 @@
     p.status = (unsigned*)(ws + W.status);
     p.steps = steps; p.N = N; p.n_base = 0; p.N_total = N; p.H = H; p.ndir = ndir; p.J = H / 8;
     p.d_base = 0; p.NPAD = 32; p.xcd_map = 0; p.ring_shift = 1;
+    p.xg_tiled = xg_tiled ? 1 : 0;
     p.dbg = (unsigned long long*)(ws + W.dbg);
     {
       static const int ps = getenv("MS_LSTM_POLL_SLEEP") ? atoi(getenv("MS_LSTM_POLL_SLEEP")) : 1;
@@ -2798,9 +2848,9 @@
             MS_HIP(hipStreamWaitEvent(ss, first_half_ev, 0));
           const size_t r0 = (size_t)t0 * N;
           const int koff = kmode == ms::GEMM_K_SECOND ? H : 0;
-          return ms::gemm_bf16x3_launch_ld(ph + r0 * Kc + koff, pl + r0 * Kc + koff, wh + koff, wl + koff, bias, xnext + r0 * NG,
-                                           (t1 - t0) * N, kmode == ms::GEMM_K_WHOLE ? Kc : H, NG, MS_ACT_NONE, 0.f, 0.f, prec, ss,
-                                           nullptr, Kc, Kc, kmode);
+          return ms::gemm_bf16x3_launch_out(ph + r0 * Kc + koff, pl + r0 * Kc + koff, wh + koff, wl + koff, bias,
+                                            xg_tiled ? xnext : xnext + r0 * NG, (t1 - t0) * N, kmode == ms::GEMM_K_WHOLE ? Kc : H, NG,
+                                            MS_ACT_NONE, 0.f, 0.f, prec, ss, nullptr, Kc, Kc, kmode, xg_layout, xg_tiled ? (int)r0 : 0, true);
         };
         auto cut_ok = [&](int t0, int t1) { return t1 > t0 && ms::gemm_k_halves_ok((t1 - t0) * N, NG); };
         auto complete = [&](int t0, int t1) {
```

After: 28810, median of 4. About the same (+0.5%).
